# dougsouza/pytorch-sync-batchnorm-example

Measured on AMD Instinct MI355X. Metric: images/sec (whole node) resnet50 SyncBN, higher is better.
Workload: dtype bf16; 1 GPU; model=resnet50, global_batch=512, per_gpu_batch=512, image=3x224x224, memory_format=channels_last, parallelism=dp1, impl=msbn, hip_graph=False, conv_autotune=False, fused_bn_act=True

## Files before the change

msbn/models/resnet.py:

```python

from typing import List, Type, Union

import torch
import torch.nn as nn

from msbn.nn import BatchNorm2d, SyncBatchNorm
from msbn.nn.fused import SyncBatchNormAct2d, bn_act_maxpool


def conv3x3(cin, cout, stride=1):
    return nn.Conv2d(cin, cout, 3, stride=stride, padding=1, bias=False)


def conv1x1(cin, cout, stride=1):
    return nn.Conv2d(cin, cout, 1, stride=stride, bias=False)


def _norm(planes, fused):
    return SyncBatchNorm(planes) if fused else BatchNorm2d(planes)


def _split(x):
    return x if isinstance(x, tuple) else (x, x)


def _last_bn(bn, x, identity, fork):
    if not fork:
        return bn(x, residual=identity)
    if isinstance(bn, SyncBatchNormAct2d):
        return bn(x, residual=identity, fork=True)
    y = bn(x, residual=identity)
    return y, y


class BasicBlock(nn.Module):
    expansion = 1

    def __init__(self, cin, planes, stride=1, downsample=None, fused=False,
                 fork=False):
        super().__init__()
        self.fused = fused
        self.fork = fork and fused
        self.conv1 = conv3x3(cin, planes, stride)
        self.conv2 = conv3x3(planes, planes)
        self.downsample = downsample
        if fused:
            self.bn1 = SyncBatchNormAct2d(planes, relu=True)
            self.bn2 = SyncBatchNormAct2d(planes, relu=True)
        else:
            self.bn1 = BatchNorm2d(planes)
            self.bn2 = BatchNorm2d(planes)
            self.relu = nn.ReLU(inplace=True)

    def forward(self, x):
        x, skip = _split(x)
        identity = (self.downsample(skip) if self.downsample is not None
                    else skip)
        if self.fused:
            out = self.bn1(self.conv1(x))
            return _last_bn(self.bn2, self.conv2(out), identity,
                            getattr(self, "fork", False))
        out = self.relu(self.bn1(self.conv1(x)))
        out = self.bn2(self.conv2(out))
        return self.relu(out + identity)


class Bottleneck(nn.Module):
    expansion = 4

    def __init__(self, cin, planes, stride=1, downsample=None, fused=False,
                 fork=False):
        super().__init__()
        self.fused = fused
        self.fork = fork and fused
        self.conv1 = conv1x1(cin, planes)
        self.conv2 = conv3x3(planes, planes, stride)
        self.conv3 = conv1x1(planes, planes * self.expansion)
        self.downsample = downsample
        if fused:
            self.bn1 = SyncBatchNormAct2d(planes, relu=True)
            self.bn2 = SyncBatchNormAct2d(planes, relu=True)
            self.bn3 = SyncBatchNormAct2d(planes * self.expansion, relu=True)
        else:
            self.bn1 = BatchNorm2d(planes)
            self.bn2 = BatchNorm2d(planes)
            self.bn3 = BatchNorm2d(planes * self.expansion)
            self.relu = nn.ReLU(inplace=True)

    def forward(self, x):
        x, skip = _split(x)
        identity = (self.downsample(skip) if self.downsample is not None
                    else skip)
        if self.fused:
            out = self.bn1(self.conv1(x))
            out = self.bn2(self.conv2(out))
            return _last_bn(self.bn3, self.conv3(out), identity,
                            getattr(self, "fork", False))
        out = self.relu(self.bn1(self.conv1(x)))
        out = self.relu(self.bn2(self.conv2(out)))
        out = self.bn3(self.conv3(out))
        return self.relu(out + identity)


class ResNet(nn.Module):
    def __init__(
        self,
        block: Type[Union[BasicBlock, Bottleneck]],
        layers: List[int],
        num_classes: int = 1000,
        in_chans: int = 3,
        fused: bool = False,
        fork_grads: bool = True,
    ):
        super().__init__()
        self.fused = fused
        self.fork_grads = fork_grads and fused
        self.stem_pool = fused
        self.inplanes = 64
        self.conv1 = nn.Conv2d(in_chans, 64, 7, stride=2, padding=3, bias=False)
        if fused:
            self.bn1 = SyncBatchNormAct2d(64, relu=True)
        else:
            self.bn1 = BatchNorm2d(64)
        self.relu = nn.ReLU(inplace=True)
        self.maxpool = nn.MaxPool2d(3, stride=2, padding=1)
        self.layer1 = self._make_layer(block, 64, layers[0])
        self.layer2 = self._make_layer(block, 128, layers[1], stride=2)
        self.layer3 = self._make_layer(block, 256, layers[2], stride=2)
        self.layer4 = self._make_layer(block, 512, layers[3], stride=2,
                                       fork_last=False)
        self.avgpool = nn.AdaptiveAvgPool2d(1)
        self.fc = nn.Linear(512 * block.expansion, num_classes)
        for m in self.modules():
            if isinstance(m, nn.Conv2d):
                nn.init.kaiming_normal_(m.weight, mode="fan_out",
                                        nonlinearity="relu")

    def _make_layer(self, block, planes, blocks, stride=1, fork_last=True):
        fork = [self.fork_grads] * (blocks - 1) + [self.fork_grads
                                                   and fork_last]
        downsample = None
        if stride != 1 or self.inplanes != planes * block.expansion:
            downsample = nn.Sequential(
                conv1x1(self.inplanes, planes * block.expansion, stride),
                _norm(planes * block.expansion, self.fused),
            )
        layers = [block(self.inplanes, planes, stride, downsample,
                        fused=self.fused, fork=fork[0])]
        self.inplanes = planes * block.expansion
        for i in range(1, blocks):
            layers.append(block(self.inplanes, planes, fused=self.fused,
                                fork=fork[i]))
        return nn.Sequential(*layers)

    def _stem(self, x):
        x = self.conv1(x)
        if self.fused:
            if (getattr(self, "stem_pool", True)
                    and isinstance(self.bn1, SyncBatchNormAct2d)):
                return bn_act_maxpool(self.bn1, self.maxpool, x,
                                      fork=getattr(self, "fork_grads", False))
            return self.maxpool(self.bn1(x))
        return self.maxpool(self.relu(self.bn1(x)))

    def forward_features(self, x):
        x = self._stem(x)
        c2 = self.layer1(x)
        c3 = self.layer2(c2)
        c4 = self.layer3(c3)
        c5 = self.layer4(c4)
        return _split(c2)[0], _split(c3)[0], _split(c4)[0], _split(c5)[0]

    def forward(self, x):
        _, _, _, c5 = self.forward_features(x)
        out = self.avgpool(c5).flatten(1)
        return self.fc(out)


def resnet18(num_classes: int = 1000, fused: bool = False,
             fork_grads: bool = True) -> ResNet:
    return ResNet(BasicBlock, [2, 2, 2, 2], num_classes, fused=fused,
                  fork_grads=fork_grads)


def resnet50(num_classes: int = 1000, fused: bool = False,
             fork_grads: bool = True) -> ResNet:
    return ResNet(Bottleneck, [3, 4, 6, 3], num_classes, fused=fused,
                  fork_grads=fork_grads)
```

msbn/nn/fused.py:

```python

from typing import Optional

import torch
import torch.distributed as dist

from msbn import ops
from msbn.nn.batchnorm import (SyncBatchNorm, _check_negative_slope,
                               _momentum_factor, _running_stats_forward)
from msbn.nn.functions import (_combined_view, _contig, _force_sync,
                               _match_layout, compute_sync_stats)


class SyncBatchNormActFunction(torch.autograd.Function):
    @staticmethod
    def forward(
        ctx,
        input: torch.Tensor,
        residual: Optional[torch.Tensor],
        weight: Optional[torch.Tensor],
        bias: Optional[torch.Tensor],
        running_mean: Optional[torch.Tensor],
        running_var: Optional[torch.Tensor],
        eps: float,
        momentum: float,
        process_group,
        world_size: int,
        relu: bool,
        negative_slope: float = 0.0,
        fork: bool = False,
    ):
        ctx.fork = fork
        y = SyncBatchNormActFunction._forward(
            ctx, input, residual, weight, bias, running_mean, running_var,
            eps, momentum, process_group, world_size, relu, negative_slope,
        )
        if not fork:
            return y
        ctx.set_materialize_grads(False)
        return y, y.detach()

    @staticmethod
    def _forward(ctx, input, residual, weight, bias, running_mean,
                 running_var, eps, momentum, process_group, world_size, relu,
                 negative_slope):
        ctx.negative_slope = negative_slope
        input = _contig(input)
        if residual is not None:
            residual = _match_layout(residual, input)
        if weight is not None:
            weight = weight.contiguous()
        if bias is not None:
            bias = bias.contiguous()

        use_sync = world_size > 1 or (
            process_group is not None and _force_sync()
        )
        if (
            not use_sync
            and input.numel() > 0
            and (residual is None or residual.is_contiguous())
            and ops.bn_fused_local_eligible(
                input, weight, bias, running_mean, running_var
            )
        ):
            y, mean, invstd, count_sum, coefs = ops.batch_norm_fwd_fused_local(
                input, residual, weight, bias, eps, momentum,
                running_mean, running_var, relu, negative_slope,
            )
            ctx.save_for_backward(input, residual, weight, bias, mean,
                                  invstd, count_sum, coefs)
            ctx.has_coefs = True
            ctx.local_fused = True
            ctx.relu = relu
            ctx.process_group = process_group
            ctx.world_size = world_size
            return y
        ctx.local_fused = False

        mean, invstd, count_sum, coefs = compute_sync_stats(
            input, eps, momentum, running_mean, running_var,
            process_group, world_size, weight, bias, want_coefs=True,
        )
        if coefs is None:
            ctx.save_for_backward(input, residual, weight, bias, mean, invstd,
                                  count_sum)
            ctx.has_coefs = False
        else:
            ctx.save_for_backward(input, residual, weight, bias, mean, invstd,
                                  count_sum, coefs)
            ctx.has_coefs = True
        ctx.relu = relu
        ctx.process_group = process_group
        ctx.world_size = world_size
        ctx.use_sync = use_sync
        if input.numel() == 0:
            return torch.empty_like(input)
        return ops.batch_norm_elemt_act(
            input, residual, weight, bias, mean, invstd, relu, coefs,
            negative_slope,
        )

    @staticmethod
    def backward(ctx, grad_output, grad_skip=None):
        if grad_output is None:
            grad_output, grad_skip = grad_skip, None
        if grad_output is None:
            return (None,) * 13
        if ctx.has_coefs:
            (input, residual, weight, bias, mean, invstd, count_sum,
             coefs) = ctx.saved_tensors
        else:
            input, residual, weight, bias, mean, invstd, count_sum = (
                ctx.saved_tensors
            )
            coefs = None
        fold = (
            grad_skip is not None and input.is_cuda and input.numel() > 0
            and not getattr(ctx, "local_fused", False)
        )
        if fold and ctx.relu and ctx.negative_slope != 0.0 and not (
            residual is not None and ctx.needs_input_grad[1]
        ):
            fold = False
        if grad_skip is not None and not fold:
            grad_output = grad_output + grad_skip
            grad_skip = None
        grad_output = _match_layout(grad_output, input)
        if fold:
            grad_skip = _match_layout(grad_skip, input)
        relu = ctx.relu
        slope = ctx.negative_slope
        process_group = ctx.process_group
        world_size = ctx.world_size
        need_input_g = ctx.needs_input_grad[0]
        need_res_g = residual is not None and ctx.needs_input_grad[1]
        need_weight_g = weight is not None and ctx.needs_input_grad[2]
        need_bias_g = bias is not None and ctx.needs_input_grad[3]

        C = int(input.shape[1])

        if getattr(ctx, "local_fused", False) and input.numel() > 0:
            grad_input, grad_weight, grad_bias, grad_res = (
                ops.batch_norm_bwd_fused_local(
                    grad_output, input, residual, mean, invstd, weight,
                    coefs, relu, need_res_g, need_weight_g, need_bias_g,
                    slope,
                )
            )
            return (
                grad_input if need_input_g else None,
                grad_res if need_res_g else None,
                grad_weight if need_weight_g else None,
                grad_bias if need_bias_g else None,
                None, None, None, None, None, None, None, None, None,
            )

        use_gm = fold or (
            relu and residual is not None and need_res_g and input.is_cuda
            and input.numel() > 0
        )
        use_sync = getattr(ctx, "use_sync", world_size > 1)
        if input.numel() == 0:
            if use_sync and (need_input_g or need_res_g):
                combined = torch.zeros(2 * C, dtype=torch.float32,
                                       device=grad_output.device)
                from msbn.utils import debug as _dbg
                if _dbg.enabled():
                    _dbg.verify_collective("syncbn.bwd.all_reduce", combined,
                                           process_group)
                dist.all_reduce(combined, dist.ReduceOp.SUM,
                                group=process_group)
            zg = torch.empty_like(grad_output)
            return (
                zg if need_input_g else None,
                torch.empty_like(grad_output) if need_res_g else None,
                torch.zeros_like(weight) if need_weight_g else None,
                torch.zeros_like(bias) if need_bias_g else None,
                None, None, None, None, None, None, None, None, None,
            )
        gm = torch.empty_like(grad_output) if use_gm else None
        sum_dy, sum_dy_xmu, grad_weight, grad_bias = (
            ops.batch_norm_backward_reduce_act(
                grad_output, input, residual, mean, invstd, weight, bias,
                relu, need_input_g, need_weight_g, need_bias_g, coefs, gm,
                slope, grad_skip,
            )
        )
        grad_input = grad_res = None
        if need_input_g or need_res_g:
            if use_sync:
                combined, copied = _combined_view(sum_dy, sum_dy_xmu, C)
                from msbn.utils import debug as _dbg
                if _dbg.enabled():
                    _dbg.verify_collective("syncbn.bwd.all_reduce",
                                           combined, process_group)
                dist.all_reduce(combined, dist.ReduceOp.SUM, group=process_group)
                from msbn.utils.logging import comm_log
                comm_log.record("all_reduce", combined.numel() * 4,
                                f"syncbn bwd C={C}")
                if copied:
                    sum_dy, sum_dy_xmu = combined[:C], combined[C:]
            if use_gm:
                grad_input, _ = ops.batch_norm_backward_elemt_act(
                    gm, input, None, mean, invstd, weight, bias,
                    sum_dy, sum_dy_xmu, count_sum, False, False, coefs,
                )
                grad_res = gm if need_res_g else None
            else:
                grad_input, grad_res = ops.batch_norm_backward_elemt_act(
                    grad_output, input, residual, mean, invstd, weight, bias,
                    sum_dy, sum_dy_xmu, count_sum, relu, need_res_g, coefs,
                    slope,
                )
        return (
            grad_input if need_input_g else None,
            grad_res,
            grad_weight if need_weight_g else None,
            grad_bias if need_bias_g else None,
            None, None, None, None, None, None, None, None, None,
        )


class SyncBatchNormActPoolFunction(torch.autograd.Function):

    @staticmethod
    def forward(
        ctx,
        input: torch.Tensor,
        weight: Optional[torch.Tensor],
        bias: Optional[torch.Tensor],
        running_mean: Optional[torch.Tensor],
        running_var: Optional[torch.Tensor],
        eps: float,
        momentum: float,
        process_group,
        world_size: int,
        relu: bool,
        negative_slope: float = 0.0,
        fork: bool = False,
    ):
        if weight is not None:
            weight = weight.contiguous()
        if bias is not None:
            bias = bias.contiguous()
        use_sync = world_size > 1 or (
            process_group is not None and _force_sync()
        )
        mean, invstd, count_sum, coefs = compute_sync_stats(
            input, eps, momentum, running_mean, running_var,
            process_group, world_size, weight, bias, want_coefs=True,
        )
        pooled, codes = ops.batch_norm_elemt_act_pool(
            input, weight, bias, mean, invstd, relu, coefs, negative_slope
        )
        ctx.has_coefs = coefs is not None
        saved = (input, codes, weight, bias, mean, invstd, count_sum)
        ctx.save_for_backward(*(saved + ((coefs,) if ctx.has_coefs else ())))
        ctx.relu = relu
        ctx.negative_slope = negative_slope
        ctx.process_group = process_group
        ctx.use_sync = use_sync
        if not fork:
            return pooled
        ctx.set_materialize_grads(False)
        return pooled, pooled.detach()

    @staticmethod
    def backward(ctx, grad_output, grad_skip=None):
        if grad_output is None:
            grad_output, grad_skip = grad_skip, None
        if grad_output is None:
            return (None,) * 12
        saved = ctx.saved_tensors
        input, codes, weight, bias, mean, invstd, count_sum = saved[:7]
        coefs = saved[7] if ctx.has_coefs else None
        grad_output = _match_layout(grad_output, codes)
        if grad_skip is not None:
            grad_skip = _match_layout(grad_skip, codes)
        relu, slope = ctx.relu, ctx.negative_slope
        process_group = ctx.process_group
        need_input_g = ctx.needs_input_grad[0]
        need_weight_g = weight is not None and ctx.needs_input_grad[1]
        need_bias_g = bias is not None and ctx.needs_input_grad[2]
        C = int(input.shape[1])

        sum_dy, sum_dy_xmu, grad_weight, grad_bias = (
            ops.batch_norm_backward_reduce_act_pool(
                grad_output, grad_skip, codes, input, mean, invstd, weight,
                bias, relu, need_input_g, need_weight_g, need_bias_g, coefs,
                slope,
            )
        )
        grad_input = None
        if need_input_g:
            if ctx.use_sync:
                combined, copied = _combined_view(sum_dy, sum_dy_xmu, C)
                from msbn.utils import debug as _dbg
                if _dbg.enabled():
                    _dbg.verify_collective("syncbn.bwd.all_reduce",
                                           combined, process_group)
                dist.all_reduce(combined, dist.ReduceOp.SUM,
                                group=process_group)
                from msbn.utils.logging import comm_log
                comm_log.record("all_reduce", combined.numel() * 4,
                                f"syncbn bwd C={C}")
                if copied:
                    sum_dy, sum_dy_xmu = combined[:C], combined[C:]
            grad_input = ops.batch_norm_backward_elemt_act_pool(
                grad_output, grad_skip, codes, input, mean, invstd, weight,
                bias, sum_dy, sum_dy_xmu, count_sum, relu, coefs, slope,
            )
        return (
            grad_input,
            grad_weight if need_weight_g else None,
            grad_bias if need_bias_g else None,
            None, None, None, None, None, None, None, None, None,
        )


def stem_pool_eligible(bn, pool, input: torch.Tensor) -> bool:
    def _pair(v):
        return tuple(v) if isinstance(v, (tuple, list)) else (v, v)

    def _hooked(m):
        return bool(m._forward_hooks or m._forward_pre_hooks
                    or m._backward_hooks or m._backward_pre_hooks)

    return (
        type(bn) is SyncBatchNormAct2d
        and not getattr(bn, "inplace", False)
        and not _hooked(bn) and not _hooked(pool)
        and (bn.training
             or (bn.running_mean is None and bn.running_var is None))
        and type(pool) is torch.nn.MaxPool2d
        and _pair(pool.kernel_size) == (3, 3)
        and _pair(pool.stride) == (2, 2)
        and _pair(pool.padding) == (1, 1)
        and _pair(pool.dilation) == (1, 1)
        and not pool.ceil_mode and not pool.return_indices
        and input.is_cuda and input.dim() == 4 and input.numel() > 0
        and input.is_contiguous(memory_format=torch.channels_last)
        and input.dtype in (torch.float32, torch.bfloat16, torch.float16)
    )


def bn_act_maxpool(bn, pool, input: torch.Tensor, fork: bool = False):
    if not stem_pool_eligible(bn, pool, input):
        y = pool(bn(input))
        return (y, y) if fork else y
    bn._check_input_dim(input)
    bn._check_non_zero_input_channels(input)
    if bn.training and bn.track_running_stats:
        if bn.num_batches_tracked is not None:
            bn.num_batches_tracked.add_(1)
    factor = _momentum_factor(bn) if bn.training else (
        bn.momentum if bn.momentum is not None else 0.0
    )
    process_group = None
    world_size = 1
    if dist.is_available() and dist.is_initialized():
        process_group = bn.process_group or dist.group.WORLD
        world_size = dist.get_world_size(process_group)
    running_mean = bn.running_mean if bn.track_running_stats else None
    running_var = bn.running_var if bn.track_running_stats else None
    return SyncBatchNormActPoolFunction.apply(
        input, bn.weight, bn.bias, running_mean, running_var, bn.eps, factor,
        process_group, world_size, bn.relu,
        getattr(bn, "negative_slope", 0.0), fork,
    )


class InPlaceSyncBatchNormActFunction(torch.autograd.Function):

    @staticmethod
    def forward(
        ctx,
        input: torch.Tensor,
        weight: torch.Tensor,
        bias: torch.Tensor,
        running_mean: Optional[torch.Tensor],
        running_var: Optional[torch.Tensor],
        eps: float,
        momentum: float,
        process_group,
        world_size: int,
        act: bool,
        negative_slope: float = 0.0,
    ):
        if act and not negative_slope > 0.0:
            raise ValueError(
                "in-place BN needs an invertible activation: identity, or "
                "LeakyReLU with negative_slope > 0"
            )
        if _contig(input) is not input:
            raise ValueError(
                "in-place BN needs a dense NCHW or channels-last input; a "
                "copy would leave the caller's tensor unwritten"
            )
        weight = weight.contiguous()
        bias = bias.contiguous()
        use_sync = world_size > 1 or (
            process_group is not None and _force_sync()
        )
        mean, invstd, count_sum, coefs = compute_sync_stats(
            input, eps, momentum, running_mean, running_var,
            process_group, world_size, weight, bias, want_coefs=True,
        )
        if input.numel() > 0:
            ops.batch_norm_elemt_act_(
                input, weight, bias, mean, invstd, act, coefs, negative_slope
            )
        ctx.mark_dirty(input)
        ctx.has_coefs = coefs is not None
        saved = (input, weight, bias, mean, invstd, count_sum)
        ctx.save_for_backward(*(saved + ((coefs,) if ctx.has_coefs else ())))
        ctx.act = act
        ctx.negative_slope = negative_slope
        ctx.process_group = process_group
        ctx.world_size = world_size
        ctx.use_sync = use_sync
        return input

    @staticmethod
    def backward(ctx, grad_output):
        saved = ctx.saved_tensors
        y, weight, bias, mean, invstd, count_sum = saved[:6]
        coefs = saved[6] if ctx.has_coefs else None
        grad_output = _match_layout(grad_output, y)
        act, slope = ctx.act, ctx.negative_slope
        process_group = ctx.process_group
        use_sync = ctx.use_sync
        need_input_g, need_weight_g, need_bias_g = ctx.needs_input_grad[:3]
        C = int(y.shape[1])

        if y.numel() == 0:
            if use_sync and need_input_g:
                combined = torch.zeros(2 * C, dtype=torch.float32,
                                       device=grad_output.device)
                from msbn.utils import debug as _dbg
                if _dbg.enabled():
                    _dbg.verify_collective("syncbn.bwd.all_reduce", combined,
                                           process_group)
                dist.all_reduce(combined, dist.ReduceOp.SUM,
                                group=process_group)
            return (
                torch.empty_like(grad_output) if need_input_g else None,
                torch.zeros_like(weight) if need_weight_g else None,
                torch.zeros_like(bias) if need_bias_g else None,
                None, None, None, None, None, None, None, None,
            )
        sum_dy, sum_dy_xmu, grad_weight, grad_bias = (
            ops.batch_norm_backward_reduce_inplace(
                grad_output, y, invstd, weight, bias, act, need_input_g,
                need_weight_g, need_bias_g, coefs, slope,
            )
        )
        grad_input = None
        if need_input_g:
            if use_sync:
                combined, copied = _combined_view(sum_dy, sum_dy_xmu, C)
                from msbn.utils import debug as _dbg
                if _dbg.enabled():
                    _dbg.verify_collective("syncbn.bwd.all_reduce",
                                           combined, process_group)
                dist.all_reduce(combined, dist.ReduceOp.SUM, group=process_group)
                from msbn.utils.logging import comm_log
                comm_log.record("all_reduce", combined.numel() * 4,
                                f"syncbn bwd C={C}")
                if copied:
                    sum_dy, sum_dy_xmu = combined[:C], combined[C:]
            grad_input = ops.batch_norm_backward_elemt_inplace(
                grad_output, y, mean, invstd, weight, bias, sum_dy,
                sum_dy_xmu, count_sum, act, coefs, slope,
            )
        return (
            grad_input,
            grad_weight if need_weight_g else None,
            grad_bias if need_bias_g else None,
            None, None, None, None, None, None, None, None,
        )


class SyncBatchNormAct2d(SyncBatchNorm):

    def __init__(self, num_features, eps=1e-5, momentum=0.1, affine=True,
                 track_running_stats=True, process_group=None, device=None,
                 dtype=None, relu: bool = True, negative_slope: float = 0.0,
                 inplace: bool = False):
        super().__init__(num_features, eps, momentum, affine,
                         track_running_stats, process_group, device, dtype)
        self.relu = relu
        self.negative_slope = _check_negative_slope(relu, negative_slope)
        if inplace:
            if not affine:
                raise ValueError("inplace=True requires affine=True")
            if relu and not self.negative_slope > 0.0:
                raise ValueError(
                    "inplace=True needs an invertible activation: "
                    "relu=False, or relu=True with negative_slope > 0 "
                    "(plain ReLU cannot be inverted)"
                )
        self.inplace = bool(inplace)

    def extra_repr(self):
        s = super().extra_repr()
        slope = getattr(self, "negative_slope", 0.0)
        if slope != 0.0:
            s += f", negative_slope={slope}"
        if getattr(self, "inplace", False):
            s += ", inplace=True"
        return s

    def forward(self, input: torch.Tensor,
                residual: Optional[torch.Tensor] = None, fork: bool = False):
        self._check_input_dim(input)
        self._check_non_zero_input_channels(input)
        slope = getattr(self, "negative_slope", 0.0)
        inplace = getattr(self, "inplace", False)
        if inplace and (residual is not None or fork):
            raise ValueError(
                "an inplace=True SyncBatchNormAct2d takes neither a residual "
                "nor fork=True"
            )

        bn_training = self.training or (
            self.running_mean is None and self.running_var is None
        )
        if self.training and self.track_running_stats:
            if self.num_batches_tracked is not None:
                self.num_batches_tracked.add_(1)
        factor = _momentum_factor(self) if self.training else (
            self.momentum if self.momentum is not None else 0.0
        )

        if not bn_training:
            y = _running_stats_forward(self, input, residual, self.relu,
                                       slope)
            return (y, y) if fork else y

        process_group = None
        world_size = 1
        if dist.is_available() and dist.is_initialized():
            process_group = self.process_group or dist.group.WORLD
            world_size = dist.get_world_size(process_group)

        running_mean = self.running_mean if self.track_running_stats else None
        running_var = self.running_var if self.track_running_stats else None
        if inplace:
            return InPlaceSyncBatchNormActFunction.apply(
                input, self.weight, self.bias, running_mean, running_var,
                self.eps, factor, process_group, world_size, self.relu, slope,
            )
        return SyncBatchNormActFunction.apply(
            input, residual, self.weight, self.bias, running_mean, running_var,
            self.eps, factor, process_group, world_size, self.relu, slope,
            fork,
        )
```

msbn/ops/__init__.py:

```python

from typing import Optional

import torch

from msbn.ops import _reference as _ref

_C = None
_C_IMPORT_ERROR: Optional[BaseException] = None
try:
    import os as _os

    if _os.environ.get("MSBN_AB_NONT", "0") == "1":
        from msbn import _C_nont as _C
    else:
        from msbn import _C as _C
except Exception as e:
    _C_IMPORT_ERROR = e


def hip_available() -> bool:
    return _C is not None


def _require_hip():
    if _C is None:
        raise RuntimeError(
            "msbn._C (the gfx950 HIP kernel extension) is not built, but a CUDA "
            "tensor reached msbn.ops. Build it with `python setup.py "
            "build_ext --inplace` (or __graft_entry__.build()). "
            f"Import error was: {_C_IMPORT_ERROR!r}"
        )
    return _C


def batch_norm_stats(input: torch.Tensor, eps: float):
    if input.is_cuda:
        return _require_hip().batch_norm_stats(input, eps)
    return _ref.batch_norm_stats(input, eps)


def batch_norm_stats_packed(input: torch.Tensor, eps: float, out: torch.Tensor):
    C = input.shape[1]
    if input.is_cuda:
        _require_hip().batch_norm_stats_packed(input, eps, out)
        return out
    mean, invstd = _ref.batch_norm_stats(input, eps)
    out[:C] = mean
    out[C : 2 * C] = invstd
    n = input.numel() // C if C > 0 else 0
    out[2 * C] = float(n)
    return out


def batch_norm_gather_stats_with_counts(
    input: torch.Tensor,
    mean_all: torch.Tensor,
    invstd_all: torch.Tensor,
    running_mean: Optional[torch.Tensor],
    running_var: Optional[torch.Tensor],
    momentum: float,
    eps: float,
    counts: torch.Tensor,
):
    if input.is_cuda:
        return _require_hip().batch_norm_gather_stats_with_counts(
            mean_all, invstd_all, running_mean, running_var, momentum, eps, counts
        )
    return _ref.batch_norm_gather_stats_with_counts(
        input, mean_all, invstd_all, running_mean, running_var, momentum, eps, counts
    )


def batch_norm_gather_stats_packed(
    input: torch.Tensor,
    packed_all: torch.Tensor,
    running_mean: Optional[torch.Tensor],
    running_var: Optional[torch.Tensor],
    momentum: float,
    eps: float,
):
    W = packed_all.shape[0]
    C = (packed_all.shape[1] - 1) // 2
    if input.is_cuda:
        return _require_hip().batch_norm_gather_stats_packed(
            packed_all, running_mean, running_var, momentum, eps
        )
    mean_all = packed_all[:, :C]
    invstd_all = packed_all[:, C : 2 * C]
    counts = packed_all[:, 2 * C]
    mean, invstd = _ref.batch_norm_gather_stats_with_counts(
        input, mean_all, invstd_all, running_mean, running_var, momentum, eps, counts
    )
    return mean, invstd, counts.sum().reshape(1)


def batch_norm_elemt(
    input: torch.Tensor,
    weight: Optional[torch.Tensor],
    bias: Optional[torch.Tensor],
    mean: torch.Tensor,
    invstd: torch.Tensor,
    eps: float,
):
    if input.is_cuda:
        return _require_hip().batch_norm_elemt(input, weight, bias, mean, invstd, eps)
    return _ref.batch_norm_elemt(input, weight, bias, mean, invstd, eps)


def batch_norm_backward_reduce(
    grad_out: torch.Tensor,
    input: torch.Tensor,
    mean: torch.Tensor,
    invstd: torch.Tensor,
    weight: Optional[torch.Tensor],
    input_g: bool,
    weight_g: bool,
    bias_g: bool,
):
    if input.is_cuda:
        return _require_hip().batch_norm_backward_reduce(
            grad_out, input, mean, invstd, weight, input_g, weight_g, bias_g
        )
    return _ref.batch_norm_backward_reduce(
        grad_out, input, mean, invstd, weight, input_g, weight_g, bias_g
    )


def batch_norm_backward_elemt(
    grad_out: torch.Tensor,
    input: torch.Tensor,
    mean: torch.Tensor,
    invstd: torch.Tensor,
    weight: Optional[torch.Tensor],
    sum_dy: torch.Tensor,
    sum_dy_xmu: torch.Tensor,
    count: torch.Tensor,
):
    if input.is_cuda:
        return _require_hip().batch_norm_backward_elemt(
            grad_out, input, mean, invstd, weight, sum_dy, sum_dy_xmu, count
        )
    return _ref.batch_norm_backward_elemt(
        grad_out, input, mean, invstd, weight, sum_dy, sum_dy_xmu, count
    )


def bn_fused_local_eligible(input, weight, bias, running_mean, running_var):
    if not input.is_cuda or _C is None:
        return False
    return _C.bn_fused_local_eligible(
        input, weight, bias, running_mean, running_var
    )


def batch_norm_fwd_fused_local(input, residual, weight, bias, eps, momentum,
                               running_mean, running_var, relu,
                               negative_slope: float = 0.0):
    return _require_hip().batch_norm_fwd_fused_local(
        input, residual, weight, bias, eps, momentum, running_mean,
        running_var, relu, negative_slope,
    )


def batch_norm_bwd_fused_local(grad_out, input, residual, mean, invstd,
                               weight, coefs, relu_mask, want_res_grad,
                               weight_g, bias_g, negative_slope: float = 0.0):
    return _require_hip().batch_norm_bwd_fused_local(
        grad_out, input, residual, mean, invstd, weight, coefs, relu_mask,
        want_res_grad, weight_g, bias_g, negative_slope,
    )


def bn_make_coefs(mean, invstd, weight, bias):
    if mean.is_cuda:
        return _require_hip().bn_make_coefs(mean, invstd, weight, bias)
    return None


def batch_norm_elemt_act(input, residual, weight, bias, mean, invstd,
                         relu: bool, coefs=None, negative_slope: float = 0.0):
    if input.is_cuda:
        return _require_hip().batch_norm_elemt_act(
            input, residual, weight, bias, mean, invstd, relu, coefs,
            negative_slope,
        )
    return _ref.batch_norm_elemt_act(
        input, residual, weight, bias, mean, invstd, relu, negative_slope
    )


def batch_norm_backward_reduce_act(grad_out, input, residual, mean, invstd,
                                   weight, bias, relu_mask, input_g, weight_g,
                                   bias_g, coefs=None, gm_out=None,
                                   negative_slope: float = 0.0,
                                   grad_out2=None):
    if input.is_cuda:
        return _require_hip().batch_norm_backward_reduce_act(
            grad_out, input, residual, mean, invstd, weight, bias, relu_mask,
            input_g, weight_g, bias_g, coefs, gm_out, negative_slope,
            grad_out2,
        )
    return _ref.batch_norm_backward_reduce_act(
        grad_out, input, residual, mean, invstd, weight, bias, relu_mask,
        input_g, weight_g, bias_g, gm_out, negative_slope, grad_out2,
    )


def batch_norm_backward_elemt_act(grad_out, input, residual, mean, invstd,
                                  weight, bias, sum_dy, sum_dy_xmu, count,
                                  relu_mask, want_res_grad, coefs=None,
                                  negative_slope: float = 0.0):
    if input.is_cuda:
        dx, dres = _require_hip().batch_norm_backward_elemt_act(
            grad_out, input, residual, mean, invstd, weight, bias, sum_dy,
            sum_dy_xmu, count, relu_mask, want_res_grad, coefs,
            negative_slope,
        )
        return dx, (dres if want_res_grad else None)
    return _ref.batch_norm_backward_elemt_act(
        grad_out, input, residual, mean, invstd, weight, bias, sum_dy,
        sum_dy_xmu, count, relu_mask, want_res_grad, negative_slope,
    )


def batch_norm_elemt_act_pool(input, weight, bias, mean, invstd, relu: bool,
                              coefs=None, negative_slope: float = 0.0):
    if input.is_cuda:
        return _require_hip().batch_norm_elemt_act_pool(
            input, weight, bias, mean, invstd, relu, coefs, negative_slope
        )
    return _ref.batch_norm_elemt_act_pool(
        input, weight, bias, mean, invstd, relu, negative_slope
    )


def batch_norm_backward_reduce_act_pool(grad_out, grad_out2, codes, input,
                                        mean, invstd, weight, bias, relu_mask,
                                        input_g, weight_g, bias_g, coefs=None,
                                        negative_slope: float = 0.0):
    if input.is_cuda:
        return _require_hip().batch_norm_backward_reduce_act_pool(
            grad_out, grad_out2, codes, input, mean, invstd, weight, bias,
            relu_mask, input_g, weight_g, bias_g, coefs, negative_slope,
        )
    return _ref.batch_norm_backward_reduce_act_pool(
        grad_out, grad_out2, codes, input, mean, invstd, weight, bias,
        relu_mask, input_g, weight_g, bias_g, negative_slope,
    )


def batch_norm_backward_elemt_act_pool(grad_out, grad_out2, codes, input,
                                       mean, invstd, weight, bias, sum_dy,
                                       sum_dy_xmu, count, relu_mask,
                                       coefs=None,
                                       negative_slope: float = 0.0):
    if input.is_cuda:
        return _require_hip().batch_norm_backward_elemt_act_pool(
            grad_out, grad_out2, codes, input, mean, invstd, weight, bias,
            sum_dy, sum_dy_xmu, count, relu_mask, coefs, negative_slope,
        )
    return _ref.batch_norm_backward_elemt_act_pool(
        grad_out, grad_out2, codes, input, mean, invstd, weight, bias,
        sum_dy, sum_dy_xmu, count, relu_mask, negative_slope,
    )


def batch_norm_elemt_act_(input, weight, bias, mean, invstd, act: bool,
                          coefs=None, negative_slope: float = 0.0):
    if input.is_cuda:
        _require_hip().batch_norm_elemt_act_(
            input, weight, bias, mean, invstd, act, coefs, negative_slope
        )
        return input
    return _ref.batch_norm_elemt_act_(
        input, weight, bias, mean, invstd, act, negative_slope
    )


def batch_norm_backward_reduce_inplace(grad_out, output, invstd, weight, bias,
                                       act: bool, input_g, weight_g, bias_g,
                                       coefs=None,
                                       negative_slope: float = 0.0):
    if output.is_cuda:
        return _require_hip().batch_norm_backward_reduce_inplace(
            grad_out, output, invstd, weight, bias, act, input_g, weight_g,
            bias_g, coefs, negative_slope,
        )
    return _ref.batch_norm_backward_reduce_inplace(
        grad_out, output, invstd, weight, bias, act, input_g, weight_g,
        bias_g, negative_slope,
    )


def batch_norm_backward_elemt_inplace(grad_out, output, mean, invstd, weight,
                                      bias, sum_dy, sum_dy_xmu, count,
                                      act: bool, coefs=None,
                                      negative_slope: float = 0.0):
    if output.is_cuda:
        return _require_hip().batch_norm_backward_elemt_inplace(
            grad_out, output, mean, invstd, weight, bias, sum_dy, sum_dy_xmu,
            count, act, coefs, negative_slope,
        )
    return _ref.batch_norm_backward_elemt_inplace(
        grad_out, output, mean, invstd, weight, bias, sum_dy, sum_dy_xmu,
        count, act, negative_slope,
    )


def bn_frozen_coefs(running_mean, running_var, eps: float, weight, bias):
    if running_mean.is_cuda:
        return _require_hip().bn_frozen_coefs(
            running_mean, running_var, eps, weight, bias
        )
    return _ref.bn_frozen_coefs(running_mean, running_var, eps, weight, bias)


def batch_norm_frozen_backward_elemt(grad_out, input, residual, coefs,
                                     relu_mask: bool, want_input_grad: bool,
                                     want_res_grad: bool,
                                     negative_slope: float = 0.0):
    if grad_out.is_cuda:
        dx, dres = _require_hip().batch_norm_frozen_backward_elemt(
            grad_out, input, residual, coefs, relu_mask, want_input_grad,
            want_res_grad, negative_slope,
        )
        return (dx if want_input_grad else None,
                dres if want_res_grad else None)
    return _ref.batch_norm_frozen_backward_elemt(
        grad_out, input, residual, coefs, relu_mask, want_input_grad,
        want_res_grad, negative_slope,
    )


def launch_plan(kind: str, input: torch.Tensor, others=(), coefs=None) -> dict:
    path, numbers = _require_hip().launch_plan(kind, input, list(others), coefs)
    plan = dict(numbers)
    plan["path"] = path
    if "multi_trip" in plan:
        plan["multi_trip"] = bool(plan["multi_trip"])
    return plan


__all__ = [
    "hip_available",
    "launch_plan",
    "bn_frozen_coefs",
    "batch_norm_frozen_backward_elemt",
    "batch_norm_elemt_act_pool",
    "batch_norm_backward_reduce_act_pool",
    "batch_norm_backward_elemt_act_pool",
    "batch_norm_elemt_act_",
    "batch_norm_backward_reduce_inplace",
    "batch_norm_backward_elemt_inplace",
    "batch_norm_elemt_act",
    "bn_make_coefs",
    "batch_norm_backward_reduce_act",
    "batch_norm_backward_elemt_act",
    "batch_norm_stats",
    "batch_norm_stats_packed",
    "batch_norm_gather_stats_with_counts",
    "batch_norm_gather_stats_packed",
    "batch_norm_elemt",
    "batch_norm_backward_reduce",
    "batch_norm_backward_elemt",
]
```

msbn/ops/csrc/bn_kernels.hip:

```cpp
#include "bn_ops.hpp"
#include "common.hpp"

#include <ATen/ATen.h>
#include <c10/hip/HIPStream.h>

#include <algorithm>
#include <map>
#include <string>
#include <vector>

namespace msbn {

namespace {

template <typename T, int V>
__global__ void bn_stats_partial_nchw(const T* __restrict__ x,
                                      double* __restrict__ ws, int64_t N,
                                      int64_t C, int64_t S, int64_t chunkN,
                                      int64_t chunkS) {
  const int64_t c = blockIdx.x;
  const int64_t n0 = blockIdx.y * chunkN;
  const int64_t n1 = i64min(n0 + chunkN, N);
  const int64_t s0 = blockIdx.z * chunkS;
  const int64_t s1 = i64min(s0 + chunkS, S);
// ... 44 lines not shown
    }
    __syncthreads();
    if (pivot_s[0] == 0.f) break;
    pivot = pivot_s[1];
  }
  if (threadIdx.x == 0) {
    const int64_t chunk = (int64_t)blockIdx.y * gridDim.z + blockIdx.z;
    double* out = ws + (c * gridDim.y * gridDim.z + chunk) * 2;
    out[0] = a;
    out[1] = b;
  }
}

template <typename T>
__global__ void bn_stats_partial_nchw_flat(const T* __restrict__ x,
                                           double* __restrict__ ws, int64_t N,
                                           int64_t C, int64_t S,
                                           int64_t chunk_len) {
  const int64_t c = blockIdx.x;
  const int64_t NS = N * S;
  const int64_t p0 = (int64_t)blockIdx.y * chunk_len;
  const int64_t p1 = i64min(p0 + chunk_len, NS);
  __shared__ double lds[2 * (MSBN_BLOCK / MSBN_WAVE)];
  __shared__ float pivot_s[2];
  float pivot = 0.f;
  double a = 0.0, b = 0.0;
  for (int pass = 0; pass < 2; ++pass) {
    AccPair acc;
    int since_flush = 0;
    for (int64_t p = p0 + threadIdx.x; p < p1; p += blockDim.x) {
      const int64_t n = p / S, s = p - n * S;
      acc.add(to_f(nt_load1(&x[(n * C + c) * S + s])) - pivot);
      if (++since_flush == MSBN_ACC_FLUSH) {
        acc.flush();
        since_flush = 0;
      }
    }
    acc.flush();
    a = acc.a;
    b = acc.b;
    if (pass) __syncthreads();
    block_reduce_pair(a, b, lds);
    const double cnt = (double)(p1 - p0);
    if (pass) {
      if (threadIdx.x == 0) unshift_pair(a, b, pivot, cnt);
      break;
    }
    if (threadIdx.x == 0) {
      const bool re = needs_recentre(a, b, cnt);
      pivot_s[0] = re ? 1.f : 0.f;
      pivot_s[1] = re ? (float)(a / cnt) : 0.f;
    }
    __syncthreads();
    if (pivot_s[0] == 0.f) break;
    pivot = pivot_s[1];
  }
  if (threadIdx.x == 0) {
    double* out = ws + (c * gridDim.y + blockIdx.y) * 2;
    out[0] = a;
    out[1] = b;
  }
}

template <typename T, int V>
__global__ void bn_stats_partial_nhwc(const T* __restrict__ x,
                                      double* __restrict__ ws, int64_t rows,
                                      int64_t C, int64_t chunk_rows, int lpr) {
  const int rpi = blockDim.x / lpr;
  const int lane = threadIdx.x % lpr;
  const int rowoff = threadIdx.x / lpr;
  const bool active = rowoff < rpi;
  const int64_t c = (int64_t)blockIdx.x * lpr * V + (int64_t)lane * V;
  const bool inb = active && (c + V <= C);
  const int64_t r0 = (int64_t)blockIdx.y * chunk_rows;
  const int64_t r1 = i64min(r0 + chunk_rows, rows);

  __shared__ double sdata[MSBN_BLOCK * V * 2];

  float pivot[V];
  bool re[V];
#pragma unroll
  for (int k = 0; k < V; ++k) {
    pivot[k] = 0.f;
    re[k] = false;
  }

  for (int pass = 0; pass < 2; ++pass) {
    AccPair acc[V];
    if (inb) {
      int since_flush = 0;
      for (int64_t r = r0 + rowoff; r < r1; r += rpi) {
        Pack<T, V> pk = nt_load<T, V>(&x[r * C + c]);
#pragma unroll
        for (int k = 0; k < V; ++k) acc[k].add(to_f(pk.v[k]) - pivot[k]);
        if (++since_flush == MSBN_ACC_FLUSH) {
#pragma unroll
          for (int k = 0; k < V; ++k) acc[k].flush();
          since_flush = 0;
        }
      }
    }
    double a[V], b[V];
#pragma unroll
    for (int k = 0; k < V; ++k) {
      acc[k].flush();
      a[k] = acc[k].a;
      b[k] = acc[k].b;
    }
    if (pass && inb && r0 + rowoff < r1) {
      const double cnt = (double)((r1 - r0 - rowoff + rpi - 1) / rpi);
#pragma unroll
      for (int k = 0; k < V; ++k) unshift_pair(a[k], b[k], pivot[k], cnt);
    }

    if (pass) __syncthreads();
#pragma unroll
    for (int k = 0; k < V; ++k) {
      sdata[k * MSBN_BLOCK + threadIdx.x] = a[k];
      sdata[(V + k) * MSBN_BLOCK + threadIdx.x] = b[k];
    }
    for (int st = 1; st < rpi; st <<= 1) {
      __syncthreads();
      if (active && (rowoff & ((st << 1) - 1)) == 0 && rowoff + st < rpi) {
        const int other = threadIdx.x + st * lpr;
#pragma unroll
        for (int k = 0; k < V; ++k) {
          sdata[k * MSBN_BLOCK + threadIdx.x] += sdata[k * MSBN_BLOCK + other];
          sdata[(V + k) * MSBN_BLOCK + threadIdx.x] +=
              sdata[(V + k) * MSBN_BLOCK + other];
        }
      }
    }
    __syncthreads();
    int any = 0;
    if (rowoff == 0 && c < C) {
      const int64_t chunk = blockIdx.y;
      const double cnt = (double)(r1 - r0);
#pragma unroll
      for (int k = 0; k < V; ++k) {
        if (c + k < C) {
          const double sa = sdata[k * MSBN_BLOCK + threadIdx.x];
          const double sb = sdata[(V + k) * MSBN_BLOCK + threadIdx.x];
          bool want = false;
          if (!pass) {
            want = needs_recentre(sa, sb, cnt);
            sdata[k * MSBN_BLOCK + threadIdx.x] = want ? 1.0 : 0.0;
            sdata[(V + k) * MSBN_BLOCK + threadIdx.x] = want ? sa / cnt : 0.0;
            any |= want ? 1 : 0;
          }
          if (pass ? re[k] : !want) {
            double* out = ws + ((c + k) * gridDim.y + chunk) * 2;
            out[0] = sa;
            out[1] = sb;
          }
        }
      }
    }
    if (pass) break;
    if (!__syncthreads_or(any)) break;
    if (inb) {
#pragma unroll
      for (int k = 0; k < V; ++k) {
        re[k] = sdata[k * MSBN_BLOCK + lane] != 0.0;
        pivot[k] = re[k] ? (float)sdata[(V + k) * MSBN_BLOCK + lane] : 0.f;
      }
    }
  }
}

template <typename RT, typename WT>
__global__ void bn_stats_finalize(const double* __restrict__ ws, int nchunks,
                                  int64_t C, double count, float eps,
                                  float* __restrict__ mean,
                                  float* __restrict__ invstd,
                                  float* __restrict__ count_out,
                                  RT* __restrict__ rmean, RT* __restrict__ rvar,
                                  float momentum, const WT* __restrict__ w,
                                  const WT* __restrict__ bws,
                                  float* __restrict__ scale_out,
                                  float* __restrict__ shift_out) {
  const int lane = threadIdx.x & (MSBN_WAVE - 1);
  const int wid = threadIdx.x >> 6;
  const int64_t c = (int64_t)blockIdx.x * (blockDim.x >> 6) + wid;
  if (c >= C) return;
  double a = 0.0, b = 0.0;
  for (int ch = lane; ch < nchunks; ch += MSBN_WAVE) {
    a += ws[(c * nchunks + ch) * 2];
    b += ws[(c * nchunks + ch) * 2 + 1];
  }
  wave_reduce_pair(a, b);
  if (lane != 0) return;
  const double m = a / count;
  double var = b / count - m * m;
  var = var > 0.0 ? var : 0.0;
  const float istd = (float)rsqrt(var + (double)eps);
  mean[c] = (float)m;
  invstd[c] = istd;
  if (c == 0 && count_out != nullptr) count_out[0] = (float)count;
  if (rmean != nullptr) {
    const double unbiased = count > 1.0 ? var * (count / (count - 1.0)) : var;
    rmean[c] = from_f<RT>((1.f - momentum) * to_f(rmean[c]) + momentum * (float)m);
    rvar[c] =
        from_f<RT>((1.f - momentum) * to_f(rvar[c]) + momentum * (float)unbiased);
  }
  if (scale_out != nullptr) {
    const float sc = istd * (w != nullptr ? to_f(w[c]) : 1.f);
    scale_out[c] = sc;
    shift_out[c] = -(float)m * sc + (bws != nullptr ? to_f(bws[c]) : 0.f);
  }
}

template <typename RT, typename WT>
__global__ void bn_gather_stats(const float* __restrict__ packed_all, int W,
                                int64_t C, float eps, float momentum,
                                float* __restrict__ mean,
                                float* __restrict__ invstd,
                                float* __restrict__ count_out,
                                RT* __restrict__ rmean, RT* __restrict__ rvar,
                                const WT* __restrict__ wpar,
                                const WT* __restrict__ bpar,
                                float* __restrict__ scale_out,
                                float* __restrict__ shift_out) {
  const int64_t c = (int64_t)blockIdx.x * blockDim.x + threadIdx.x;
  if (c >= C) return;
  const int64_t row = 2 * C + 1;
  double n_tot = 0.0, m_acc = 0.0, ex2 = 0.0;
  for (int w = 0; w < W; ++w) {
    const float cnt = packed_all[w * row + 2 * C];
    if (cnt > 0.f) {
      const double m = packed_all[w * row + c];
      const double istd = packed_all[w * row + C + c];
      const double var = 1.0 / (istd * istd) - (double)eps;
      n_tot += cnt;
      m_acc += cnt * m;
      ex2 += cnt * (var + m * m);
    }
  }
  float m_out = 0.f, istd_out = 0.f;
  if (n_tot > 0.0) {
    const double m_g = m_acc / n_tot;
    double var_g = ex2 / n_tot - m_g * m_g;
    var_g = var_g > 0.0 ? var_g : 0.0;
    m_out = (float)m_g;
    istd_out = (float)rsqrt(var_g + (double)eps);
    if (rmean != nullptr) {
      const double unbiased =
          n_tot > 1.0 ? var_g * (n_tot / (n_tot - 1.0)) : var_g;
      rmean[c] =
          from_f<RT>((1.f - momentum) * to_f(rmean[c]) + momentum * (float)m_g);
      rvar[c] = from_f<RT>((1.f - momentum) * to_f(rvar[c]) +
                           momentum * (float)unbiased);
    }
  }
  mean[c] = m_out;
  invstd[c] = istd_out;
  if (c == 0 && count_out != nullptr) count_out[0] = (float)n_tot;
  if (scale_out != nullptr) {
    const float sc = istd_out * (wpar != nullptr ? to_f(wpar[c]) : 1.f);
    scale_out[c] = sc;
    shift_out[c] = -m_out * sc + (bpar != nullptr ? to_f(bpar[c]) : 0.f);
  }
}

template <typename WT>
__global__ void bn_affine_fwd(const float* __restrict__ mean,
                              const float* __restrict__ invstd,
                              const WT* __restrict__ w,
                              const WT* __restrict__ b, int64_t C,
                              float* __restrict__ scale,
                              float* __restrict__ shift) {
  const int64_t c = (int64_t)blockIdx.x * blockDim.x + threadIdx.x;
  if (c >= C) return;
  const float sc = invstd[c] * (w != nullptr ? to_f(w[c]) : 1.f);
  scale[c] = sc;
  shift[c] = -mean[c] * sc + (b != nullptr ? to_f(b[c]) : 0.f);
}

template <typename WT>
__global__ void bn_affine_bwd(const float* __restrict__ mean,
                              const float* __restrict__ invstd,
                              const WT* __restrict__ w,
                              const float* __restrict__ sum_dy,
                              const float* __restrict__ sum_dy_xmu,
                              const float* __restrict__ count, int64_t C,
                              float* __restrict__ coef_a,
                              float* __restrict__ coef_b,
                              float* __restrict__ coef_d) {
  const int64_t c = (int64_t)blockIdx.x * blockDim.x + threadIdx.x;
  if (c >= C) return;
  const float n = count[0];
  if (n <= 0.f) {
    coef_a[c] = coef_b[c] = coef_d[c] = 0.f;
    return;
  }
  const float istd = invstd[c];
  const float f1 = istd * (w != nullptr ? to_f(w[c]) : 1.f);
  const float f2 = sum_dy[c] / n;
  const float f3 = istd * istd * sum_dy_xmu[c] / n;
  coef_a[c] = f1;
  coef_b[c] = -f1 * f3;
  coef_d[c] = f1 * (f3 * mean[c] - f2);
}

template <typename T, int V, int ACT, bool RES>
__global__ void bn_elemt_nchw(const T* __restrict__ x,
                              const T* __restrict__ res, T* __restrict__ y,
                              const float* __restrict__ scale,
                              const float* __restrict__ shift, int64_t total,
                              int64_t C, int64_t S, float slope) {
  const int64_t stride = (int64_t)gridDim.x * blockDim.x;
  for (int64_t i = (int64_t)blockIdx.x * blockDim.x + threadIdx.x;
       i * V < total; i += stride) {
    const int64_t e = i * V;
    const int64_t c = (e / S) % C;
    const float sc = scale[c], sh = shift[c];
    if (V == 1) {
      float z = to_f(nt_load1(&x[e])) * sc + sh;
      if (RES) z += to_f(nt_load1(&res[e]));
      z = act_fwd<ACT>(z, slope);
      nt_store1(&y[e], from_f<T>(z));
    } else {
      Pack<T, V> px = nt_load<T, V>(&x[e]);
      Pack<T, V> pr;
      if (RES) pr = nt_load<T, V>(&res[e]);
      Pack<T, V> py;
#pragma unroll
      for (int k = 0; k < V; ++k) {
        float z = to_f(px.v[k]) * sc + sh;
        if (RES) z += to_f(pr.v[k]);
        z = act_fwd<ACT>(z, slope);
        py.v[k] = from_f<T>(z);
      }
      nt_store<T, V>(&y[e], py);
    }
  }
}

template <typename T, int V, int ACT, bool RES>
__global__ void bn_elemt_nhwc(const T* __restrict__ x,
                              const T* __restrict__ res, T* __restrict__ y,
                              const float* __restrict__ scale,
                              const float* __restrict__ shift, int64_t total,
                              int64_t C, float slope) {
  const int64_t stride = (int64_t)gridDim.x * blockDim.x;
  for (int64_t i = (int64_t)blockIdx.x * blockDim.x + threadIdx.x;
       i * V < total; i += stride) {
    const int64_t e = i * V;
    const int64_t c = e % C;
    if (V == 1) {
      float z = to_f(nt_load1(&x[e])) * scale[c] + shift[c];
      if (RES) z += to_f(nt_load1(&res[e]));
      z = act_fwd<ACT>(z, slope);
      nt_store1(&y[e], from_f<T>(z));
    } else {
      Pack<T, V> px = nt_load<T, V>(&x[e]);
      Pack<float, V> ps = *reinterpret_cast<const Pack<float, V>*>(&scale[c]);
      Pack<float, V> pb = *reinterpret_cast<const Pack<float, V>*>(&shift[c]);
      Pack<T, V> pr;
      if (RES) pr = nt_load<T, V>(&res[e]);
      Pack<T, V> py;
#pragma unroll
      for (int k = 0; k < V; ++k) {
        float z = to_f(px.v[k]) * ps.v[k] + pb.v[k];
        if (RES) z += to_f(pr.v[k]);
        z = act_fwd<ACT>(z, slope);
        py.v[k] = from_f<T>(z);
      }
      nt_store<T, V>(&y[e], py);
    }
  }
}

template <typename T>
__device__ __forceinline__ float fork_grad(T g1, T g2) {
  return to_f(from_f<T>(to_f(g1) + to_f(g2)));
}

template <typename T, int V, int ACT, bool RES, bool GMOUT, bool DY2>
__global__ void bn_bwd_reduce_partial_nchw(const T* __restrict__ dy,
                                           const T* __restrict__ dy2,
                                           const T* __restrict__ x,
                                           const T* __restrict__ res,
                                           T* __restrict__ gm_out,
                                           const float* __restrict__ mean,
                                           const float* __restrict__ scale,
                                           const float* __restrict__ shift,
                                           double* __restrict__ ws, int64_t N,
                                           int64_t C, int64_t S, int64_t chunkN,
                                           int64_t chunkS, float slope) {
  const int64_t c = blockIdx.x;
  const float m = mean[c];
  const float sc = ACT ? scale[c] : 0.f;
  const float sh = ACT ? shift[c] : 0.f;
  const int64_t n0 = blockIdx.y * chunkN;
  const int64_t n1 = i64min(n0 + chunkN, N);
  const int64_t s0 = blockIdx.z * chunkS;
  const int64_t s1 = i64min(s0 + chunkS, S);
  AccPair acc;
  int since_flush = 0;
  for (int64_t n = n0; n < n1; ++n) {
    const int64_t base = (n * C + c) * S;
    if (V == 1) {
      for (int64_t s = s0 + threadIdx.x; s < s1; s += blockDim.x) {
        float g = DY2 ? fork_grad(nt_load1(&dy[base + s]),
                                  nt_load1(&dy2[base + s]))
                      : to_f(nt_load1(&dy[base + s]));
        const float xv = to_f(nt_load1(&x[base + s]));
        if (ACT) {
          float z = sc * xv + sh;
          if (RES) z += to_f(nt_load1(&res[base + s]));
          g = act_gate<ACT>(z, g, slope);
        }
        if (GMOUT) nt_store1(&gm_out[base + s], from_f<T>(g));
        acc.add2(g, g * (xv - m));
        if (++since_flush == MSBN_ACC_FLUSH) {
          acc.flush();
          since_flush = 0;
        }
      }
    } else {
      for (int64_t s = s0 + (int64_t)threadIdx.x * V; s < s1;
           s += (int64_t)blockDim.x * V) {
        Pack<T, V> pg = nt_load<T, V>(&dy[base + s]);
        Pack<T, V> px = nt_load<T, V>(&x[base + s]);
        Pack<T, V> pg2, pr, pm;
        if (DY2) pg2 = nt_load<T, V>(&dy2[base + s]);
        if (RES) pr = nt_load<T, V>(&res[base + s]);
#pragma unroll
        for (int k = 0; k < V; ++k) {
          float g = DY2 ? fork_grad(pg.v[k], pg2.v[k]) : to_f(pg.v[k]);
          const float xv = to_f(px.v[k]);
          if (ACT) {
            float z = sc * xv + sh;
            if (RES) z += to_f(pr.v[k]);
            g = act_gate<ACT>(z, g, slope);
          }
          if (GMOUT) pm.v[k] = from_f<T>(g);
          acc.add2(g, g * (xv - m));
        }
        if (GMOUT) nt_store<T, V>(&gm_out[base + s], pm);
        if (++since_flush == MSBN_ACC_FLUSH / V) {
          acc.flush();
          since_flush = 0;
        }
      }
    }
  }
  acc.flush();
  double a = acc.a, b = acc.b;
  __shared__ double lds[2 * (MSBN_BLOCK / MSBN_WAVE)];
  block_reduce_pair(a, b, lds);
  if (threadIdx.x == 0) {
    const int64_t chunk = (int64_t)blockIdx.y * gridDim.z + blockIdx.z;
    double* out = ws + (c * gridDim.y * gridDim.z + chunk) * 2;
    out[0] = a;
    out[1] = b;
  }
}

template <typename T, int ACT, bool RES, bool GMOUT, bool DY2>
__global__ void bn_bwd_reduce_partial_nchw_flat(
    const T* __restrict__ dy, const T* __restrict__ dy2,
    const T* __restrict__ x,
    const T* __restrict__ res, T* __restrict__ gm_out,
    const float* __restrict__ mean,
    const float* __restrict__ scale, const float* __restrict__ shift,
    double* __restrict__ ws, int64_t N, int64_t C, int64_t S,
    int64_t chunk_len, float slope) {
  const int64_t c = blockIdx.x;
  const float m = mean[c];
  const float sc = ACT ? scale[c] : 0.f;
  const float sh = ACT ? shift[c] : 0.f;
  const int64_t NS = N * S;
  const int64_t p0 = (int64_t)blockIdx.y * chunk_len;
  const int64_t p1 = i64min(p0 + chunk_len, NS);
  AccPair acc;
  int since_flush = 0;
  for (int64_t p = p0 + threadIdx.x; p < p1; p += blockDim.x) {
    const int64_t n = p / S, s = p - n * S;
    const int64_t e = (n * C + c) * S + s;
    float g = DY2 ? fork_grad(nt_load1(&dy[e]), nt_load1(&dy2[e]))
                  : to_f(nt_load1(&dy[e]));
    const float xv = to_f(nt_load1(&x[e]));
    if (ACT) {
      float z = sc * xv + sh;
      if (RES) z += to_f(nt_load1(&res[e]));
      g = act_gate<ACT>(z, g, slope);
    }
    if (GMOUT) nt_store1(&gm_out[e], from_f<T>(g));
    acc.add2(g, g * (xv - m));
    if (++since_flush == MSBN_ACC_FLUSH) {
      acc.flush();
      since_flush = 0;
    }
  }
  acc.flush();
  double a = acc.a, b = acc.b;
  __shared__ double lds[2 * (MSBN_BLOCK / MSBN_WAVE)];
  block_reduce_pair(a, b, lds);
  if (threadIdx.x == 0) {
    double* out = ws + (c * gridDim.y + blockIdx.y) * 2;
    out[0] = a;
    out[1] = b;
  }
}

template <typename T, int V, int ACT, bool RES, bool GMOUT, bool DY2>
__global__ void bn_bwd_reduce_partial_nhwc(const T* __restrict__ dy,
                                           const T* __restrict__ dy2,
                                           const T* __restrict__ x,
                                           const T* __restrict__ res,
                                           T* __restrict__ gm_out,
                                           const float* __restrict__ mean,
                                           const float* __restrict__ scale,
                                           const float* __restrict__ shift,
                                           double* __restrict__ ws,
                                           int64_t rows, int64_t C,
                                           int64_t chunk_rows, int lpr,
                                           float slope) {
  const int rpi = blockDim.x / lpr;
  const int lane = threadIdx.x % lpr;
  const int rowoff = threadIdx.x / lpr;
  const bool active = rowoff < rpi;
  const int64_t c = (int64_t)blockIdx.x * lpr * V + (int64_t)lane * V;
  const bool inb = active && (c + V <= C);

  AccPair acc[V];
  float m[V], scv[V], shv[V];
#pragma unroll
  for (int k = 0; k < V; ++k) m[k] = scv[k] = shv[k] = 0.f;
  if (inb) {
#pragma unroll
    for (int k = 0; k < V; ++k) {
      m[k] = mean[c + k];
      if (ACT) {
        scv[k] = scale[c + k];
        shv[k] = shift[c + k];
      }
    }
    const int64_t r0 = (int64_t)blockIdx.y * chunk_rows;
    const int64_t r1 = i64min(r0 + chunk_rows, rows);
    int since_flush = 0;
    for (int64_t r = r0 + rowoff; r < r1; r += rpi) {
      Pack<T, V> pg = nt_load<T, V>(&dy[r * C + c]);
      Pack<T, V> px = nt_load<T, V>(&x[r * C + c]);
      Pack<T, V> pg2, pr, pm;
      if (DY2) pg2 = nt_load<T, V>(&dy2[r * C + c]);
      if (RES) pr = nt_load<T, V>(&res[r * C + c]);
#pragma unroll
      for (int k = 0; k < V; ++k) {
        float g = DY2 ? fork_grad(pg.v[k], pg2.v[k]) : to_f(pg.v[k]);
        const float xv = to_f(px.v[k]);
        if (ACT) {
          float z = scv[k] * xv + shv[k];
          if (RES) z += to_f(pr.v[k]);
          g = act_gate<ACT>(z, g, slope);
        }
        if (GMOUT) pm.v[k] = from_f<T>(g);
        acc[k].add2(g, g * (xv - m[k]));
      }
      if (GMOUT) nt_store<T, V>(&gm_out[r * C + c], pm);
      if (++since_flush == MSBN_ACC_FLUSH) {
#pragma unroll
        for (int k = 0; k < V; ++k) acc[k].flush();
        since_flush = 0;
      }
    }
  }
  double a[V], b[V];
#pragma unroll
  for (int k = 0; k < V; ++k) {
    acc[k].flush();
    a[k] = acc[k].a;
    b[k] = acc[k].b;
  }
  __shared__ double sdata[MSBN_BLOCK * V * 2];
#pragma unroll
  for (int k = 0; k < V; ++k) {
    sdata[k * MSBN_BLOCK + threadIdx.x] = a[k];
    sdata[(V + k) * MSBN_BLOCK + threadIdx.x] = b[k];
  }
  for (int st = 1; st < rpi; st <<= 1) {
    __syncthreads();
    if (active && (rowoff & ((st << 1) - 1)) == 0 && rowoff + st < rpi) {
      const int other = threadIdx.x + st * lpr;
#pragma unroll
      for (int k = 0; k < V; ++k) {
        sdata[k * MSBN_BLOCK + threadIdx.x] += sdata[k * MSBN_BLOCK + other];
        sdata[(V + k) * MSBN_BLOCK + threadIdx.x] +=
            sdata[(V + k) * MSBN_BLOCK + other];
      }
    }
  }
  __syncthreads();
  if (rowoff == 0 && c < C) {
    const int64_t chunk = blockIdx.y;
#pragma unroll
    for (int k = 0; k < V; ++k) {
      if (c + k < C) {
        double* out = ws + ((c + k) * gridDim.y + chunk) * 2;
        out[0] = sdata[k * MSBN_BLOCK + threadIdx.x];
        out[1] = sdata[(V + k) * MSBN_BLOCK + threadIdx.x];
      }
    }
  }
}

template <typename WT>
__global__ void bn_bwd_reduce_finalize(const double* __restrict__ ws,
                                       int nchunks, int64_t C,
                                       const float* __restrict__ invstd,
                                       float* __restrict__ sum_dy,
                                       float* __restrict__ sum_dy_xmu,
                                       WT* __restrict__ grad_weight,
                                       WT* __restrict__ grad_bias) {
  const int lane = threadIdx.x & (MSBN_WAVE - 1);
  const int wid = threadIdx.x >> 6;
  const int64_t c = (int64_t)blockIdx.x * (blockDim.x >> 6) + wid;
  if (c >= C) return;
  double a = 0.0, b = 0.0;
  for (int ch = lane; ch < nchunks; ch += MSBN_WAVE) {
    a += ws[(c * nchunks + ch) * 2];
    b += ws[(c * nchunks + ch) * 2 + 1];
  }
  wave_reduce_pair(a, b);
  if (lane != 0) return;
  if (sum_dy != nullptr) sum_dy[c] = (float)a;
  if (sum_dy_xmu != nullptr) sum_dy_xmu[c] = (float)b;
  if (grad_weight != nullptr) grad_weight[c] = from_f<WT>((float)(b * invstd[c]));
  if (grad_bias != nullptr) grad_bias[c] = from_f<WT>((float)a);
}

template <typename T, int V, int ACT, bool RES, bool RESG>
__global__ void bn_bwd_elemt_nchw(const T* __restrict__ dy,
                                  const T* __restrict__ x,
                                  const T* __restrict__ res,
                                  T* __restrict__ dx, T* __restrict__ dres,
                                  const float* __restrict__ ca,
                                  const float* __restrict__ cb,
                                  const float* __restrict__ cd,
                                  const float* __restrict__ scale,
                                  const float* __restrict__ shift,
                                  int64_t total, int64_t C, int64_t S,
                                  float slope) {
  const int64_t stride = (int64_t)gridDim.x * blockDim.x;
  for (int64_t i = (int64_t)blockIdx.x * blockDim.x + threadIdx.x;
       i * V < total; i += stride) {
    const int64_t e = i * V;
    const int64_t c = (e / S) % C;
    const float A = ca[c], B = cb[c], D = cd[c];
    const float sc = ACT ? scale[c] : 0.f;
    const float sh = ACT ? shift[c] : 0.f;
    if (V == 1) {
      float g = to_f(nt_load1(&dy[e]));
      const float xv = to_f(nt_load1(&x[e]));
      if (ACT) {
        float z = sc * xv + sh;
        if (RES) z += to_f(nt_load1(&res[e]));
        g = act_gate<ACT>(z, g, slope);
      }
      nt_store1(&dx[e], from_f<T>(A * g + B * xv + D));
      if (RESG) nt_store1(&dres[e], from_f<T>(g));
    } else {
      Pack<T, V> pg = nt_load<T, V>(&dy[e]);
      Pack<T, V> px = nt_load<T, V>(&x[e]);
      Pack<T, V> pr;
      if (RES) pr = nt_load<T, V>(&res[e]);
      Pack<T, V> po, pq;
#pragma unroll
      for (int k = 0; k < V; ++k) {
        float g = to_f(pg.v[k]);
        const float xv = to_f(px.v[k]);
        if (ACT) {
          float z = sc * xv + sh;
          if (RES) z += to_f(pr.v[k]);
          g = act_gate<ACT>(z, g, slope);
        }
        po.v[k] = from_f<T>(A * g + B * xv + D);
        if (RESG) pq.v[k] = from_f<T>(g);
      }
      nt_store<T, V>(&dx[e], po);
      if (RESG) nt_store<T, V>(&dres[e], pq);
    }
  }
}

template <typename T, int V, int ACT, bool RES, bool RESG>
__global__ void bn_bwd_elemt_nhwc(const T* __restrict__ dy,
                                  const T* __restrict__ x,
                                  const T* __restrict__ res,
                                  T* __restrict__ dx, T* __restrict__ dres,
                                  const float* __restrict__ ca,
                                  const float* __restrict__ cb,
                                  const float* __restrict__ cd,
                                  const float* __restrict__ scale,
                                  const float* __restrict__ shift,
                                  int64_t total, int64_t C, float slope) {
  const int64_t stride = (int64_t)gridDim.x * blockDim.x;
  for (int64_t i = (int64_t)blockIdx.x * blockDim.x + threadIdx.x;
       i * V < total; i += stride) {
    const int64_t e = i * V;
    const int64_t c = e % C;
    if (V == 1) {
      float g = to_f(nt_load1(&dy[e]));
      const float xv = to_f(nt_load1(&x[e]));
      if (ACT) {
        float z = scale[c] * xv + shift[c];
        if (RES) z += to_f(nt_load1(&res[e]));
        g = act_gate<ACT>(z, g, slope);
      }
      nt_store1(&dx[e], from_f<T>(ca[c] * g + cb[c] * xv + cd[c]));
      if (RESG) nt_store1(&dres[e], from_f<T>(g));
    } else {
      Pack<T, V> pg = nt_load<T, V>(&dy[e]);
      Pack<T, V> px = nt_load<T, V>(&x[e]);
      Pack<float, V> pa = *reinterpret_cast<const Pack<float, V>*>(&ca[c]);
      Pack<float, V> pb = *reinterpret_cast<const Pack<float, V>*>(&cb[c]);
      Pack<float, V> pd = *reinterpret_cast<const Pack<float, V>*>(&cd[c]);
      Pack<float, V> psc, psh;
      if (ACT) {
        psc = *reinterpret_cast<const Pack<float, V>*>(&scale[c]);
        psh = *reinterpret_cast<const Pack<float, V>*>(&shift[c]);
      }
      Pack<T, V> pr;
      if (RES) pr = nt_load<T, V>(&res[e]);
      Pack<T, V> po, pq;
#pragma unroll
      for (int k = 0; k < V; ++k) {
        float g = to_f(pg.v[k]);
        const float xv = to_f(px.v[k]);
        if (ACT) {
          float z = psc.v[k] * xv + psh.v[k];
          if (RES) z += to_f(pr.v[k]);
          g = act_gate<ACT>(z, g, slope);
        }
        po.v[k] = from_f<T>(pa.v[k] * g + pb.v[k] * xv + pd.v[k]);
        if (RESG) pq.v[k] = from_f<T>(g);
      }
      nt_store<T, V>(&dx[e], po);
      if (RESG) nt_store<T, V>(&dres[e], pq);
    }
  }
}

template <typename RT, typename WT>
__global__ void bn_frozen_coefs(const RT* __restrict__ rmean,
                                const RT* __restrict__ rvar, float eps,
                                const WT* __restrict__ w,
                                const WT* __restrict__ b, int64_t C,
                                float* __restrict__ scale,
                                float* __restrict__ shift) {
  const int64_t c = (int64_t)blockIdx.x * blockDim.x + threadIdx.x;
  if (c >= C) return;
  const float istd = (float)rsqrt((double)to_f(rvar[c]) + (double)eps);
  const float sc = istd * (w != nullptr ? to_f(w[c]) : 1.f);
  scale[c] = sc;
  shift[c] = -to_f(rmean[c]) * sc + (b != nullptr ? to_f(b[c]) : 0.f);
}

template <typename T, int V, int ACT, bool RES, bool RESG>
__global__ void bn_frozen_bwd_elemt_nchw(const T* __restrict__ dy,
                                         const T* __restrict__ x,
                                         const T* __restrict__ res,
                                         T* __restrict__ dx,
                                         T* __restrict__ dres,
                                         const float* __restrict__ scale,
                                         const float* __restrict__ shift,
                                         int64_t total, int64_t C, int64_t S,
                                         float slope) {
  const int64_t stride = (int64_t)gridDim.x * blockDim.x;
  for (int64_t i = (int64_t)blockIdx.x * blockDim.x + threadIdx.x;
       i * V < total; i += stride) {
    const int64_t e = i * V;
    const int64_t c = (e / S) % C;
    const float sc = scale[c];
    const float sh = ACT ? shift[c] : 0.f;
    if (V == 1) {
      float g = to_f(nt_load1(&dy[e]));
      if (ACT) {
        float z = sc * to_f(nt_load1(&x[e])) + sh;
        if (RES) z += to_f(nt_load1(&res[e]));
        g = act_gate<ACT>(z, g, slope);
      }
      if (dx != nullptr) nt_store1(&dx[e], from_f<T>(sc * g));
      if (RESG) nt_store1(&dres[e], from_f<T>(g));
    } else {
      Pack<T, V> pg = nt_load<T, V>(&dy[e]);
      Pack<T, V> px, pr;
      if (ACT) px = nt_load<T, V>(&x[e]);
      if (ACT && RES) pr = nt_load<T, V>(&res[e]);
      Pack<T, V> po, pq;
#pragma unroll
      for (int k = 0; k < V; ++k) {
        float g = to_f(pg.v[k]);
        if (ACT) {
          float z = sc * to_f(px.v[k]) + sh;
          if (RES) z += to_f(pr.v[k]);
          g = act_gate<ACT>(z, g, slope);
        }
        po.v[k] = from_f<T>(sc * g);
        if (RESG) pq.v[k] = from_f<T>(g);
      }
      if (dx != nullptr) nt_store<T, V>(&dx[e], po);
      if (RESG) nt_store<T, V>(&dres[e], pq);
    }
  }
}

template <typename T, int V, int ACT, bool RES, bool RESG>
__global__ void bn_frozen_bwd_elemt_nhwc(const T* __restrict__ dy,
                                         const T* __restrict__ x,
                                         const T* __restrict__ res,
                                         T* __restrict__ dx,
                                         T* __restrict__ dres,
                                         const float* __restrict__ scale,
                                         const float* __restrict__ shift,
                                         int64_t total, int64_t C,
                                         float slope) {
  const int64_t stride = (int64_t)gridDim.x * blockDim.x;
  for (int64_t i = (int64_t)blockIdx.x * blockDim.x + threadIdx.x;
       i * V < total; i += stride) {
    const int64_t e = i * V;
    const int64_t c = e % C;
    if (V == 1) {
      float g = to_f(nt_load1(&dy[e]));
      const float sc = scale[c];
      if (ACT) {
        float z = sc * to_f(nt_load1(&x[e])) + shift[c];
        if (RES) z += to_f(nt_load1(&res[e]));
        g = act_gate<ACT>(z, g, slope);
      }
      if (dx != nullptr) nt_store1(&dx[e], from_f<T>(sc * g));
      if (RESG) nt_store1(&dres[e], from_f<T>(g));
    } else {
      Pack<T, V> pg = nt_load<T, V>(&dy[e]);
      Pack<float, V> psc = *reinterpret_cast<const Pack<float, V>*>(&scale[c]);
      Pack<float, V> psh;
      Pack<T, V> px, pr;
      if (ACT) {
        psh = *reinterpret_cast<const Pack<float, V>*>(&shift[c]);
        px = nt_load<T, V>(&x[e]);
      }
      if (ACT && RES) pr = nt_load<T, V>(&res[e]);
      Pack<T, V> po, pq;
#pragma unroll
      for (int k = 0; k < V; ++k) {
        float g = to_f(pg.v[k]);
        if (ACT) {
          float z = psc.v[k] * to_f(px.v[k]) + psh.v[k];
          if (RES) z += to_f(pr.v[k]);
          g = act_gate<ACT>(z, g, slope);
        }
        po.v[k] = from_f<T>(psc.v[k] * g);
        if (RESG) pq.v[k] = from_f<T>(g);
      }
      if (dx != nullptr) nt_store<T, V>(&dx[e], po);
// ... 1063 lines not shown
    switch (TYPE) {                                                         \
      case at::kFloat: {                                                    \
        using wt_t = float;                                                 \
        return __VA_ARGS__();                                               \
      }                                                                     \
      case at::kBFloat16: {                                                 \
        using wt_t = __hip_bfloat16;                                        \
        return __VA_ARGS__();                                               \
      }                                                                     \
      case at::kHalf: {                                                     \
        using wt_t = __half;                                                \
        return __VA_ARGS__();                                               \
      }                                                                     \
      default:                                                              \
        TORCH_CHECK(false, NAME, ": unsupported weight dtype ", TYPE);      \
    }                                                                       \
  }()

void stats_into(const at::Tensor& input, double eps, float* mean_p,
                float* invstd_p, float* count_p, const at::Tensor* rmean,
                const at::Tensor* rvar, double momentum,
                const at::Tensor* wpar = nullptr,
                const at::Tensor* bpar = nullptr, float* scale_p = nullptr,
                float* shift_p = nullptr) {
  const Layout L = get_layout(input);
  const int64_t count = L.rows;
  auto stream = cur_stream();
  const auto rstat_type = rmean ? rmean->scalar_type() : at::kFloat;
  const auto w_type = wpar ? wpar->scalar_type()
                     : bpar ? bpar->scalar_type()
                            : at::kFloat;

  MSBN_DISPATCH_FLOAT_TYPES(input.scalar_type(), "batch_norm_stats", [&] {
    const native_t* x =
        reinterpret_cast<const native_t*>(input.data_ptr<scalar_t>());
    constexpr int VMAX = 16 / (int)sizeof(native_t);
    const ReducePlan plan = plan_reduce(L, (int)sizeof(native_t), {x});
    const int v = plan.v;
    const int nchunks = plan.nchunks;
    at::Tensor ws = at::empty({(int64_t)nchunks * L.C * 2},
                              input.options().dtype(at::kDouble));
    if (plan.path == RedPath::NchwFlat) {
      const auto& g = plan.flat;
      hipLaunchKernelGGL((bn_stats_partial_nchw_flat<native_t>), g.grid,
                         dim3(MSBN_BLOCK), 0, stream, x,
                         ws.data_ptr<double>(), L.N, L.C, L.S, g.chunk_len);
    } else if (plan.path == RedPath::NchwVec) {
      const auto& g = plan.nchw;
      MSBN_DISPATCH_V(v, VMAX, [&] {
        hipLaunchKernelGGL((bn_stats_partial_nchw<native_t, VV>), g.grid,
                           dim3(MSBN_BLOCK), 0, stream, x,
                           ws.data_ptr<double>(), L.N, L.C, L.S, g.chunkN,
                           g.chunkS);
      });
    } else {
      const auto& g = plan.nhwc;
      MSBN_DISPATCH_V(v, VMAX, [&] {
        hipLaunchKernelGGL((bn_stats_partial_nhwc<native_t, VV>), g.grid,
                           dim3(MSBN_BLOCK), 0, stream, x,
                           ws.data_ptr<double>(), L.rows, L.C, g.chunk_rows,
                           g.lpr);
      });
    }
    const int fgrid = (int)cdiv(L.C, kFinalizeWavesPerBlock);
    MSBN_DISPATCH_RSTAT(rstat_type, "batch_norm_stats", [&] {
      MSBN_DISPATCH_WTYPE(w_type, "batch_norm_stats", [&] {
        rstat_t* rm = rmean ? reinterpret_cast<rstat_t*>(rmean->data_ptr())
                            : nullptr;
        rstat_t* rv = rvar ? reinterpret_cast<rstat_t*>(rvar->data_ptr())
                           : nullptr;
        const wt_t* wp =
            wpar ? reinterpret_cast<const wt_t*>(wpar->data_ptr()) : nullptr;
        const wt_t* bp =
            bpar ? reinterpret_cast<const wt_t*>(bpar->data_ptr()) : nullptr;
        hipLaunchKernelGGL((bn_stats_finalize<rstat_t, wt_t>), dim3(fgrid),
                           dim3(MSBN_BLOCK), 0, stream, ws.data_ptr<double>(),
                           nchunks, L.C, (double)count, (float)eps, mean_p,
                           invstd_p, count_p, rm, rv, (float)momentum, wp, bp,
                           scale_p, shift_p);
      });
    });
  });
}

}


std::tuple<at::Tensor, at::Tensor> batch_norm_stats(const at::Tensor& input,
                                                    double eps) {
  const int64_t C = input.size(1);
  auto opts = input.options().dtype(at::kFloat);
  auto mean = at::empty({C}, opts);
  auto invstd = at::empty({C}, opts);
  if (input.numel() == 0) {
    mean.zero_();
    invstd.zero_();
    return {mean, invstd};
  }
  stats_into(input, eps, mean.data_ptr<float>(), invstd.data_ptr<float>(),
             nullptr, nullptr, nullptr, 0.0);
  return {mean, invstd};
}

void batch_norm_stats_packed(const at::Tensor& input, double eps,
                             at::Tensor& out) {
  const int64_t C = input.size(1);
  TORCH_CHECK(out.is_contiguous() && out.numel() == 2 * C + 1 &&
                  out.scalar_type() == at::kFloat,
              "packed stats buffer must be contiguous fp32 of size 2C+1");
  if (input.numel() == 0) {
    out.zero_();
    return;
  }
  float* p = out.data_ptr<float>();
  stats_into(input, eps, p, p + C, p + 2 * C, nullptr, nullptr, 0.0);
}

std::tuple<at::Tensor, at::Tensor, at::Tensor, at::Tensor>
batch_norm_gather_stats_packed_coefs(
    const at::Tensor& packed_all, const c10::optional<at::Tensor>& running_mean,
    const c10::optional<at::Tensor>& running_var, double momentum, double eps,
    const c10::optional<at::Tensor>& weight,
    const c10::optional<at::Tensor>& bias, bool want_coefs) {
  TORCH_CHECK(packed_all.dim() == 2 && packed_all.is_contiguous() &&
                  packed_all.scalar_type() == at::kFloat,
              "packed_all must be contiguous fp32 [W, 2C+1]");
  const int W = (int)packed_all.size(0);
  const int64_t C = (packed_all.size(1) - 1) / 2;
  auto opts = packed_all.options();
  auto mean = at::empty({C}, opts);
  auto invstd = at::empty({C}, opts);
  auto count_sum = at::empty({1}, opts);
  at::Tensor coefs;
  float* scale_p = nullptr;
  float* shift_p = nullptr;
  if (want_coefs) {
    coefs = at::empty({2 * C}, opts);
    scale_p = coefs.data_ptr<float>();
    shift_p = scale_p + C;
  }
  auto stream = cur_stream();
  const auto rstat_type =
      running_mean.has_value() ? running_mean->scalar_type() : at::kFloat;
  const auto w_type = weight.has_value() ? weight->scalar_type()
                      : bias.has_value() ? bias->scalar_type()
                                         : at::kFloat;
  const int fgrid = (int)cdiv(C, MSBN_BLOCK);
  MSBN_DISPATCH_RSTAT(rstat_type, "gather_stats", [&] {
    MSBN_DISPATCH_WTYPE(w_type, "gather_stats", [&] {
      rstat_t* rm = running_mean.has_value()
                        ? reinterpret_cast<rstat_t*>(running_mean->data_ptr())
                        : nullptr;
      rstat_t* rv = running_var.has_value()
                        ? reinterpret_cast<rstat_t*>(running_var->data_ptr())
                        : nullptr;
      const wt_t* wp =
          weight.has_value()
              ? reinterpret_cast<const wt_t*>(weight->data_ptr())
              : nullptr;
      const wt_t* bp = bias.has_value()
                           ? reinterpret_cast<const wt_t*>(bias->data_ptr())
                           : nullptr;
      hipLaunchKernelGGL((bn_gather_stats<rstat_t, wt_t>), dim3(fgrid),
                         dim3(MSBN_BLOCK), 0, stream,
                         packed_all.data_ptr<float>(), W, C, (float)eps,
                         (float)momentum, mean.data_ptr<float>(),
                         invstd.data_ptr<float>(), count_sum.data_ptr<float>(),
                         rm, rv, wp, bp, scale_p, shift_p);
    });
  });
  return {mean, invstd, count_sum, coefs};
}

std::tuple<at::Tensor, at::Tensor, at::Tensor> batch_norm_gather_stats_packed(
    const at::Tensor& packed_all, const c10::optional<at::Tensor>& running_mean,
    const c10::optional<at::Tensor>& running_var, double momentum, double eps) {
  auto r = batch_norm_gather_stats_packed_coefs(
      packed_all, running_mean, running_var, momentum, eps, c10::nullopt,
      c10::nullopt, false);
  return {std::get<0>(r), std::get<1>(r), std::get<2>(r)};
}

std::tuple<at::Tensor, at::Tensor, at::Tensor, at::Tensor>
batch_norm_stats_local(const at::Tensor& input, double eps,
                       const c10::optional<at::Tensor>& running_mean,
                       const c10::optional<at::Tensor>& running_var,
                       double momentum,
                       const c10::optional<at::Tensor>& weight,
                       const c10::optional<at::Tensor>& bias,
                       bool want_coefs) {
  const int64_t C = input.size(1);
  auto opts = input.options().dtype(at::kFloat);
  auto mean = at::empty({C}, opts);
  auto invstd = at::empty({C}, opts);
  auto count_sum = at::empty({1}, opts);
  at::Tensor coefs;
  float* scale_p = nullptr;
  float* shift_p = nullptr;
  if (want_coefs) {
    coefs = at::empty({2 * C}, opts);
    scale_p = coefs.data_ptr<float>();
    shift_p = scale_p + C;
  }
  TORCH_CHECK(input.numel() > 0, "batch_norm_stats_local: empty input");
  const at::Tensor* rm =
      running_mean.has_value() ? &running_mean.value() : nullptr;
  const at::Tensor* rv =
      running_var.has_value() ? &running_var.value() : nullptr;
  const at::Tensor* wp = weight.has_value() ? &weight.value() : nullptr;
  const at::Tensor* bp = bias.has_value() ? &bias.value() : nullptr;
  stats_into(input, eps, mean.data_ptr<float>(), invstd.data_ptr<float>(),
             count_sum.data_ptr<float>(), rm, rv, momentum, wp, bp, scale_p,
             shift_p);
  return {mean, invstd, count_sum, coefs};
}

std::tuple<at::Tensor, at::Tensor> batch_norm_gather_stats_with_counts(
    const at::Tensor& mean_all, const at::Tensor& invstd_all,
    const c10::optional<at::Tensor>& running_mean,
    const c10::optional<at::Tensor>& running_var, double momentum, double eps,
    const at::Tensor& counts) {
  const int64_t W = mean_all.size(0);
  const int64_t C = mean_all.size(1);
  auto packed = at::empty({W, 2 * C + 1}, mean_all.options().dtype(at::kFloat));
  packed.narrow(1, 0, C).copy_(mean_all);
  packed.narrow(1, C, C).copy_(invstd_all);
  packed.narrow(1, 2 * C, 1).copy_(
      counts.to(at::kFloat).reshape({W, 1}));
  auto out = batch_norm_gather_stats_packed(packed, running_mean, running_var,
                                            momentum, eps);
  return {std::get<0>(out), std::get<1>(out)};
}

namespace {
at::Tensor make_fwd_coefs(const at::Tensor& mean, const at::Tensor& invstd,
                          const c10::optional<at::Tensor>& weight,
                          const c10::optional<at::Tensor>& bias, int64_t C) {
  auto coefs = at::empty({2 * C}, mean.options().dtype(at::kFloat));
  float* scale = coefs.data_ptr<float>();
  float* shift = scale + C;
  auto stream = cur_stream();
  const int cgrid = (int)cdiv(C, MSBN_BLOCK);
  const auto wtype = weight.has_value() ? weight->scalar_type()
                     : bias.has_value() ? bias->scalar_type()
                                        : at::kFloat;
  MSBN_DISPATCH_RSTAT(wtype, "bn_affine", [&] {
    const rstat_t* w =
        weight.has_value()
            ? reinterpret_cast<const rstat_t*>(weight->data_ptr())
            : nullptr;
    const rstat_t* b = bias.has_value()
                           ? reinterpret_cast<const rstat_t*>(bias->data_ptr())
                           : nullptr;
    hipLaunchKernelGGL((bn_affine_fwd<rstat_t>), dim3(cgrid), dim3(MSBN_BLOCK),
                       0, stream, mean.data_ptr<float>(),
                       invstd.data_ptr<float>(), w, b, C, scale, shift);
  });
  return coefs;
}

#define MSBN_DISPATCH_BOOL(FLAG, NAME, ...)                                  \
  [&] {                                                                      \
    if (FLAG) {                                                              \
      constexpr bool NAME = true;                                            \
      return __VA_ARGS__();                                                  \
    } else {                                                                 \
      constexpr bool NAME = false;                                           \
      return __VA_ARGS__();                                                  \
    }                                                                        \
  }()

inline int act_mode(bool on, float slope) {
  return !on ? kActNone : (slope == 0.f ? kActRelu : kActLeaky);
}

#define MSBN_DISPATCH_ACT(MODE, NAME, ...)                                   \
  [&] {                                                                      \
    switch (MODE) {                                                          \
      case kActRelu: {                                                       \
        constexpr int NAME = kActRelu;                                       \
        return __VA_ARGS__();                                                \
      }                                                                      \
      case kActLeaky: {                                                      \
        constexpr int NAME = kActLeaky;                                      \
        return __VA_ARGS__();                                                \
      }                                                                      \
      default: {                                                             \
        constexpr int NAME = kActNone;                                       \
        return __VA_ARGS__();                                                \
      }                                                                      \
    }                                                                        \
  }()

template <int ACT>
using ActC = std::integral_constant<int, ACT>;
}

at::Tensor bn_make_coefs(const at::Tensor& mean, const at::Tensor& invstd,
                         const c10::optional<at::Tensor>& weight,
                         const c10::optional<at::Tensor>& bias) {
  return make_fwd_coefs(mean, invstd, weight, bias, mean.numel());
}

at::Tensor batch_norm_elemt_act(const at::Tensor& input,
                                const c10::optional<at::Tensor>& residual,
                                const c10::optional<at::Tensor>& weight,
                                const c10::optional<at::Tensor>& bias,
                                const at::Tensor& mean,
                                const at::Tensor& invstd, bool relu,
                                const c10::optional<at::Tensor>& coefs_in,
                                double negative_slope) {
  const Layout L = get_layout(input);
  auto out = at::empty_like(input);
  if (input.numel() == 0) return out;
  const float slope = (float)negative_slope;
  const int act = act_mode(relu, slope);
  auto stream = cur_stream();
  auto coefs = coefs_in.has_value()
                   ? *coefs_in
                   : make_fwd_coefs(mean, invstd, weight, bias, L.C);
  float* scale = coefs.data_ptr<float>();
  float* shift = scale + L.C;
  const bool has_res = residual.has_value();
  if (has_res) {
    TORCH_CHECK(residual->sizes() == input.sizes() &&
                    residual->strides() == input.strides() &&
                    residual->scalar_type() == input.scalar_type(),
                "residual must match input shape/strides/dtype");
  }

  const int64_t total = input.numel();
  MSBN_DISPATCH_FLOAT_TYPES(input.scalar_type(), "bn_elemt", [&] {
    const native_t* x =
        reinterpret_cast<const native_t*>(input.data_ptr<scalar_t>());
    const native_t* res =
        has_res ? reinterpret_cast<const native_t*>(residual->data_ptr())
                : nullptr;
    native_t* y = reinterpret_cast<native_t*>(out.data_ptr<scalar_t>());
    constexpr int VMAX = 16 / (int)sizeof(native_t);
    const ElemtPlan plan =
        plan_elemt(L, total, (int)sizeof(native_t), {x, y, res}, scale);
    const int v = plan.v;
    const int grid = plan.grid;
    MSBN_DISPATCH_V(v, VMAX, [&] {
      MSBN_DISPATCH_ACT(act, ACT_, [&] {
        MSBN_DISPATCH_BOOL(has_res, RES_, [&] {
          if (!L.nhwc) {
            hipLaunchKernelGGL((bn_elemt_nchw<native_t, VV, ACT_, RES_>),
                               dim3(grid), dim3(MSBN_BLOCK), 0, stream, x, res,
                               y, scale, shift, total, L.C, L.S, slope);
          } else {
            hipLaunchKernelGGL((bn_elemt_nhwc<native_t, VV, ACT_, RES_>),
                               dim3(grid), dim3(MSBN_BLOCK), 0, stream, x, res,
                               y, scale, shift, total, L.C, slope);
          }
        });
      });
    });
  });
  return out;
}

at::Tensor batch_norm_elemt(const at::Tensor& input,
                            const c10::optional<at::Tensor>& weight,
                            const c10::optional<at::Tensor>& bias,
                            const at::Tensor& mean, const at::Tensor& invstd,
                            double eps) {
  (void)eps;
  return batch_norm_elemt_act(input, c10::nullopt, weight, bias, mean, invstd,
                              false, c10::nullopt, 0.0);
}

std::tuple<at::Tensor, at::Tensor, at::Tensor, at::Tensor>
batch_norm_backward_reduce_act(
    const at::Tensor& grad_out, const at::Tensor& input,
    const c10::optional<at::Tensor>& residual, const at::Tensor& mean,
    const at::Tensor& invstd, const c10::optional<at::Tensor>& weight,
    const c10::optional<at::Tensor>& bias, bool relu_mask, bool input_g,
    bool weight_g, bool bias_g, const c10::optional<at::Tensor>& coefs_in,
    const c10::optional<at::Tensor>& gm_out, double negative_slope,
    const c10::optional<at::Tensor>& grad_out2) {
  const Layout L = get_layout(input);
  const float slope = (float)negative_slope;
  const int act = act_mode(relu_mask, slope);
  if (input.numel() == 0) {
    auto z32 = input.options().dtype(at::kFloat);
    auto combined0 = at::zeros({2 * L.C}, z32);
    const auto wt = weight.has_value() ? weight->scalar_type()
                                       : input.scalar_type();
    at::Tensor gw0, gb0;
    if (weight_g) gw0 = at::zeros({L.C}, input.options().dtype(wt));
    if (bias_g) gb0 = at::zeros({L.C}, input.options().dtype(wt));
    return {combined0.narrow(0, 0, L.C), combined0.narrow(0, L.C, L.C), gw0,
            gb0};
  }
  const bool want_gm = gm_out.has_value();
  if (want_gm) {
    TORCH_CHECK(gm_out->sizes() == input.sizes() &&
                    gm_out->strides() == input.strides() &&
                    gm_out->scalar_type() == input.scalar_type(),
                "gm_out must match input shape/strides/dtype");
  }
  TORCH_CHECK(grad_out.sizes() == input.sizes() &&
                  grad_out.strides() == input.strides(),
              "grad_out must match input shape and layout");
  const bool has_dy2 = grad_out2.has_value();
  if (has_dy2) {
    TORCH_CHECK(want_gm, "grad_out2 requires gm_out");
    TORCH_CHECK(grad_out2->sizes() == input.sizes() &&
                    grad_out2->strides() == input.strides() &&
                    grad_out2->scalar_type() == input.scalar_type() &&
                    grad_out2->device() == input.device(),
                "grad_out2 must match input shape/strides/dtype");
  }
  TORCH_CHECK(!residual.has_value() ||
                  (residual->sizes() == input.sizes() &&
                   residual->strides() == input.strides()),
              "residual must match input shape and layout");
  auto f32 = input.options().dtype(at::kFloat);
  auto combined = at::empty({2 * L.C}, f32);
  auto sum_dy = combined.narrow(0, 0, L.C);
  auto sum_dy_xmu = combined.narrow(0, L.C, L.C);
  const auto wtype =
      weight.has_value() ? weight->scalar_type() : input.scalar_type();
  auto wopts = input.options().dtype(wtype);
  at::Tensor grad_weight, grad_bias;
  if (weight_g) grad_weight = at::empty({L.C}, wopts);
  if (bias_g) grad_bias = at::empty({L.C}, wopts);

  const bool has_res = residual.has_value();
  float* scale = nullptr;
  float* shift = nullptr;
  at::Tensor coefs;
  if (relu_mask) {
    coefs = coefs_in.has_value()
                ? *coefs_in
                : make_fwd_coefs(mean, invstd, weight, bias, L.C);
    scale = coefs.data_ptr<float>();
    shift = scale + L.C;
  }

  auto stream = cur_stream();
  MSBN_DISPATCH_FLOAT_TYPES(input.scalar_type(), "bn_bwd_reduce", [&] {
    const native_t* x =
        reinterpret_cast<const native_t*>(input.data_ptr<scalar_t>());
    const native_t* dy =
        reinterpret_cast<const native_t*>(grad_out.data_ptr<scalar_t>());
    const native_t* res =
        has_res ? reinterpret_cast<const native_t*>(residual->data_ptr())
                : nullptr;
    native_t* gm =
        want_gm ? reinterpret_cast<native_t*>(gm_out->data_ptr()) : nullptr;
    const native_t* dy2 =
        has_dy2 ? reinterpret_cast<const native_t*>(grad_out2->data_ptr())
                : nullptr;
    constexpr int VMAX = 16 / (int)sizeof(native_t);
    const ReducePlan plan =
        plan_reduce(L, (int)sizeof(native_t), {x, dy, res, gm, dy2});
    const int v = plan.v;
    const int nchunks = plan.nchunks;
    at::Tensor ws = at::empty({(int64_t)nchunks * L.C * 2},
                              input.options().dtype(at::kDouble));
    MSBN_DISPATCH_ACT(act, ACT_, [&] {
      MSBN_DISPATCH_BOOL(has_res, RES_, [&] {
        MSBN_DISPATCH_BOOL(want_gm, GM_, [&] {
          auto launch = [&](auto dy2_c) {
            constexpr bool DY2_ = decltype(dy2_c)::value && GM_;
            if (!L.nhwc) {
              if (plan.path == RedPath::NchwFlat) {
                const auto& g = plan.flat;
                hipLaunchKernelGGL(
                    (bn_bwd_reduce_partial_nchw_flat<native_t, ACT_, RES_,
                                                     GM_, DY2_>),
                    g.grid, dim3(MSBN_BLOCK), 0, stream, dy, dy2, x, res, gm,
                    mean.data_ptr<float>(), scale, shift,
                    ws.data_ptr<double>(), L.N, L.C, L.S, g.chunk_len, slope);
              } else {
                const auto& g = plan.nchw;
                MSBN_DISPATCH_V(v, VMAX, [&] {
                  hipLaunchKernelGGL(
                      (bn_bwd_reduce_partial_nchw<native_t, VV, ACT_, RES_,
                                                  GM_, DY2_>),
                      g.grid, dim3(MSBN_BLOCK), 0, stream, dy, dy2, x, res,
                      gm, mean.data_ptr<float>(), scale, shift,
                      ws.data_ptr<double>(), L.N, L.C, L.S, g.chunkN,
                      g.chunkS, slope);
                });
              }
            } else {
              const auto& g = plan.nhwc;
              MSBN_DISPATCH_V(v, VMAX, [&] {
                hipLaunchKernelGGL(
                    (bn_bwd_reduce_partial_nhwc<native_t, VV, ACT_, RES_, GM_,
                                                DY2_>),
                    g.grid, dim3(MSBN_BLOCK), 0, stream, dy, dy2, x, res, gm,
                    mean.data_ptr<float>(), scale, shift,
                    ws.data_ptr<double>(), L.rows, L.C, g.chunk_rows, g.lpr,
                    slope);
              });
            }
          };
          if (has_dy2) {
            launch(std::true_type{});
          } else {
            launch(std::false_type{});
          }
        });
      });
    });
    const int fgrid = (int)cdiv(L.C, kFinalizeWavesPerBlock);
    MSBN_DISPATCH_RSTAT(wtype, "bn_bwd_reduce", [&] {
      rstat_t* gw = weight_g ? reinterpret_cast<rstat_t*>(grad_weight.data_ptr())
                             : nullptr;
      rstat_t* gb =
          bias_g ? reinterpret_cast<rstat_t*>(grad_bias.data_ptr()) : nullptr;
      hipLaunchKernelGGL((bn_bwd_reduce_finalize<rstat_t>), dim3(fgrid),
                         dim3(MSBN_BLOCK), 0, stream, ws.data_ptr<double>(),
                         nchunks, L.C, invstd.data_ptr<float>(),
                         sum_dy.data_ptr<float>(),
                         sum_dy_xmu.data_ptr<float>(), gw, gb);
    });
  });
  (void)input_g;
  return {sum_dy, sum_dy_xmu, grad_weight, grad_bias};
}

std::tuple<at::Tensor, at::Tensor, at::Tensor, at::Tensor>
batch_norm_backward_reduce(const at::Tensor& grad_out, const at::Tensor& input,
                           const at::Tensor& mean, const at::Tensor& invstd,
                           const c10::optional<at::Tensor>& weight, bool input_g,
                           bool weight_g, bool bias_g) {
  return batch_norm_backward_reduce_act(grad_out, input, c10::nullopt, mean,
                                        invstd, weight, c10::nullopt, false,
                                        input_g, weight_g, bias_g,
                                        c10::nullopt, c10::nullopt, 0.0,
                                        c10::nullopt);
}

std::tuple<at::Tensor, at::Tensor> batch_norm_backward_elemt_act(
    const at::Tensor& grad_out, const at::Tensor& input,
    const c10::optional<at::Tensor>& residual, const at::Tensor& mean,
    const at::Tensor& invstd, const c10::optional<at::Tensor>& weight,
    const c10::optional<at::Tensor>& bias, const at::Tensor& sum_dy,
    const at::Tensor& sum_dy_xmu, const at::Tensor& count, bool relu_mask,
    bool want_res_grad, const c10::optional<at::Tensor>& coefs_in,
    double negative_slope) {
  const Layout L = get_layout(input);
  const float slope = (float)negative_slope;
  const int act = act_mode(relu_mask, slope);
  auto dx = at::empty_like(grad_out);
  at::Tensor dres;
  if (want_res_grad) dres = at::empty_like(grad_out);
  if (input.numel() == 0) return {dx, dres};
  at::Tensor count_sum;
  if (count.numel() == 1 && count.scalar_type() == at::kFloat) {
    count_sum = count;
  } else {
    count_sum = count.to(at::kFloat).sum().reshape({1});
  }
  auto stream = cur_stream();
  auto f32 = input.options().dtype(at::kFloat);
  auto coefs = at::empty({3 * L.C}, f32);
  float* ca = coefs.data_ptr<float>();
  float* cb = ca + L.C;
  float* cd = cb + L.C;
  const int cgrid = (int)cdiv(L.C, MSBN_BLOCK);
  const auto wtype =
      weight.has_value() ? weight->scalar_type() : at::kFloat;
  MSBN_DISPATCH_RSTAT(wtype, "bn_bwd_elemt", [&] {
    const rstat_t* w =
        weight.has_value()
            ? reinterpret_cast<const rstat_t*>(weight->data_ptr())
            : nullptr;
    hipLaunchKernelGGL((bn_affine_bwd<rstat_t>), dim3(cgrid), dim3(MSBN_BLOCK),
                       0, stream, mean.data_ptr<float>(),
                       invstd.data_ptr<float>(), w, sum_dy.data_ptr<float>(),
                       sum_dy_xmu.data_ptr<float>(),
                       count_sum.data_ptr<float>(), L.C, ca, cb, cd);
  });
  const bool has_res = residual.has_value();
  float* scale = nullptr;
  float* shift = nullptr;
  at::Tensor fcoefs;
  if (relu_mask) {
    fcoefs = coefs_in.has_value()
                 ? *coefs_in
                 : make_fwd_coefs(mean, invstd, weight, bias, L.C);
    scale = fcoefs.data_ptr<float>();
    shift = scale + L.C;
  }

  const int64_t total = input.numel();
  MSBN_DISPATCH_FLOAT_TYPES(input.scalar_type(), "bn_bwd_elemt", [&] {
    const native_t* x =
        reinterpret_cast<const native_t*>(input.data_ptr<scalar_t>());
    const native_t* dy =
        reinterpret_cast<const native_t*>(grad_out.data_ptr<scalar_t>());
    const native_t* res =
        has_res ? reinterpret_cast<const native_t*>(residual->data_ptr())
                : nullptr;
    native_t* o = reinterpret_cast<native_t*>(dx.data_ptr<scalar_t>());
    native_t* dr = want_res_grad
                       ? reinterpret_cast<native_t*>(dres.data_ptr<scalar_t>())
                       : nullptr;
    constexpr int VMAX = 16 / (int)sizeof(native_t);
    const ElemtPlan plan = plan_elemt(L, total, (int)sizeof(native_t),
                                      {x, dy, res, o, dr}, scale);
    const int v = plan.v;
    const int grid = plan.grid;
    MSBN_DISPATCH_V(v, VMAX, [&] {
      MSBN_DISPATCH_ACT(act, ACT_, [&] {
        MSBN_DISPATCH_BOOL(has_res, RES_, [&] {
          MSBN_DISPATCH_BOOL(want_res_grad, RESG_, [&] {
            if (!L.nhwc) {
              hipLaunchKernelGGL(
                  (bn_bwd_elemt_nchw<native_t, VV, ACT_, RES_, RESG_>),
                  dim3(grid), dim3(MSBN_BLOCK), 0, stream, dy, x, res, o, dr,
                  ca, cb, cd, scale, shift, total, L.C, L.S, slope);
            } else {
              hipLaunchKernelGGL(
                  (bn_bwd_elemt_nhwc<native_t, VV, ACT_, RES_, RESG_>),
                  dim3(grid), dim3(MSBN_BLOCK), 0, stream, dy, x, res, o, dr,
                  ca, cb, cd, scale, shift, total, L.C, slope);
            }
          });
        });
      });
    });
  });
  return {dx, dres};
}

at::Tensor batch_norm_backward_elemt(
    const at::Tensor& grad_out, const at::Tensor& input, const at::Tensor& mean,
    const at::Tensor& invstd, const c10::optional<at::Tensor>& weight,
    const at::Tensor& sum_dy, const at::Tensor& sum_dy_xmu,
    const at::Tensor& count) {
  return std::get<0>(batch_norm_backward_elemt_act(
      grad_out, input, c10::nullopt, mean, invstd, weight, c10::nullopt,
      sum_dy, sum_dy_xmu, count, false, false, c10::nullopt, 0.0));
}

namespace {
struct PoolGeom {
  int H, W, OH, OW;
};

Layout pool_layout(const at::Tensor& x, const char* op) {
  TORCH_CHECK(x.dim() == 4 &&
                  x.is_contiguous(at::MemoryFormat::ChannelsLast),
              op, ": input must be a dense 4-D channels-last tensor");
  Layout L{};
  L.nhwc = true;
  L.N = x.size(0);
  L.C = x.size(1);
  L.S = x.size(2) * x.size(3);
  L.rows = L.N * L.S;
  return L;
}

PoolGeom pool_geom(const at::Tensor& x, const Layout& L, const char* op) {
  TORCH_CHECK(L.rows < (int64_t)INT32_MAX, op, ": N*H*W must be below 2^31");
  PoolGeom g{};
  g.H = (int)x.size(2);
  g.W = (int)x.size(3);
  g.OH = (g.H - 1) / 2 + 1;
  g.OW = (g.W - 1) / 2 + 1;
  return g;
}

void check_pooled(const at::Tensor& t, const at::Tensor& x, const PoolGeom& g,
                  at::ScalarType dtype, const char* op, const char* what) {
  TORCH_CHECK(t.dim() == 4 && t.size(0) == x.size(0) &&
                  t.size(1) == x.size(1) && t.size(2) == g.OH &&
                  t.size(3) == g.OW && t.scalar_type() == dtype &&
                  t.device() == x.device() &&
                  t.is_contiguous(at::MemoryFormat::ChannelsLast),
              op, ": ", what, " must be a channels-last [N, C, OH, OW] ",
              dtype, " tensor on the input's device");
}
}

std::tuple<at::Tensor, at::Tensor> batch_norm_elemt_act_pool(
    const at::Tensor& input, const c10::optional<at::Tensor>& weight,
    const c10::optional<at::Tensor>& bias, const at::Tensor& mean,
    const at::Tensor& invstd, bool relu,
    const c10::optional<at::Tensor>& coefs_in, double negative_slope) {
  const Layout L = pool_layout(input, "bn_elemt_pool");
  TORCH_CHECK(input.numel() > 0, "bn_elemt_pool: empty input");
  const PoolGeom g = pool_geom(input, L, "bn_elemt_pool");
  const float slope = (float)negative_slope;
  const int act = act_mode(relu, slope);
  auto out = at::empty({input.size(0), L.C, g.OH, g.OW},
                       input.options().memory_format(
                           at::MemoryFormat::ChannelsLast));
  auto codes = at::empty_like(out, out.options().dtype(at::kByte));
  auto stream = cur_stream();
  auto coefs = coefs_in.has_value()
                   ? *coefs_in
                   : make_fwd_coefs(mean, invstd, weight, bias, L.C);
  float* scale = coefs.data_ptr<float>();
  float* shift = scale + L.C;
  const int64_t total = out.numel();
  MSBN_DISPATCH_FLOAT_TYPES(input.scalar_type(), "bn_elemt_pool", [&] {
    const native_t* x =
        reinterpret_cast<const native_t*>(input.data_ptr<scalar_t>());
    native_t* y = reinterpret_cast<native_t*>(out.data_ptr<scalar_t>());
    uint8_t* cp = codes.data_ptr<uint8_t>();
    constexpr int VMAX = 16 / (int)sizeof(native_t);
    const ElemtPlan plan =
        plan_elemt(L, total, (int)sizeof(native_t), {x, y, cp}, scale);
    MSBN_DISPATCH_V(plan.v, VMAX, [&] {
      constexpr int VK = VV * (int)sizeof(native_t) <= 16 ? VV : 1;
      MSBN_DISPATCH_ACT(act, ACT_, [&] {
        hipLaunchKernelGGL((bn_elemt_pool_nhwc<native_t, VK, ACT_>),
                           dim3(plan.grid), dim3(MSBN_BLOCK), 0, stream, x, y,
                           cp, scale, shift, total, L.C, g.H, g.W, g.OH, g.OW,
                           slope);
      });
    });
  });
  return {out, codes};
}

std::tuple<at::Tensor, at::Tensor, at::Tensor, at::Tensor>
batch_norm_backward_reduce_act_pool(
    const at::Tensor& grad_out, const c10::optional<at::Tensor>& grad_out2,
    const at::Tensor& codes, const at::Tensor& input, const at::Tensor& mean,
    const at::Tensor& invstd, const c10::optional<at::Tensor>& weight,
    const c10::optional<at::Tensor>& bias, bool relu_mask, bool input_g,
    bool weight_g, bool bias_g, const c10::optional<at::Tensor>& coefs_in,
    double negative_slope) {
  const Layout L = pool_layout(input, "bn_bwd_reduce_pool");
  TORCH_CHECK(input.numel() > 0, "bn_bwd_reduce_pool: empty input");
  const PoolGeom g = pool_geom(input, L, "bn_bwd_reduce_pool");
  const float slope = (float)negative_slope;
  const int act = act_mode(relu_mask, slope);
  check_pooled(grad_out, input, g, input.scalar_type(), "bn_bwd_reduce_pool",
               "grad_out");
  const bool has_dy2 = grad_out2.has_value();
  if (has_dy2)
    check_pooled(*grad_out2, input, g, input.scalar_type(),
                 "bn_bwd_reduce_pool", "grad_out2");
  check_pooled(codes, input, g, at::kByte, "bn_bwd_reduce_pool", "codes");
  auto f32 = input.options().dtype(at::kFloat);
  auto combined = at::empty({2 * L.C}, f32);
  auto sum_dy = combined.narrow(0, 0, L.C);
  auto sum_dy_xmu = combined.narrow(0, L.C, L.C);
  const auto wtype =
      weight.has_value() ? weight->scalar_type() : input.scalar_type();
  auto wopts = input.options().dtype(wtype);
  at::Tensor grad_weight, grad_bias;
  if (weight_g) grad_weight = at::empty({L.C}, wopts);
  if (bias_g) grad_bias = at::empty({L.C}, wopts);

  float* scale = nullptr;
  float* shift = nullptr;
  at::Tensor coefs;
  if (relu_mask) {
    coefs = coefs_in.has_value()
                ? *coefs_in
                : make_fwd_coefs(mean, invstd, weight, bias, L.C);
    scale = coefs.data_ptr<float>();
    shift = scale + L.C;
  }

  auto stream = cur_stream();
  MSBN_DISPATCH_FLOAT_TYPES(input.scalar_type(), "bn_bwd_reduce_pool", [&] {
    const native_t* x =
        reinterpret_cast<const native_t*>(input.data_ptr<scalar_t>());
    const native_t* dy =
        reinterpret_cast<const native_t*>(grad_out.data_ptr<scalar_t>());
    const native_t* dy2 =
        has_dy2 ? reinterpret_cast<const native_t*>(grad_out2->data_ptr())
                : nullptr;
    const uint8_t* cp = codes.data_ptr<uint8_t>();
    constexpr int VMAX = 16 / (int)sizeof(native_t);
    const ReducePlan plan =
        plan_reduce(L, (int)sizeof(native_t), {x, dy, dy2, cp});
    const int nchunks = plan.nchunks;
    const auto& ng = plan.nhwc;
    at::Tensor ws = at::empty({(int64_t)nchunks * L.C * 2},
                              input.options().dtype(at::kDouble));
    MSBN_DISPATCH_V(plan.v, VMAX, [&] {
      constexpr int VK = VV * (int)sizeof(native_t) <= 16 ? VV : 1;
      MSBN_DISPATCH_ACT(act, ACT_, [&] {
        MSBN_DISPATCH_BOOL(has_dy2, DY2_, [&] {
          hipLaunchKernelGGL(
              (bn_bwd_reduce_pool_partial_nhwc<native_t, VK, ACT_, DY2_>),
              ng.grid, dim3(MSBN_BLOCK), 0, stream, dy, dy2, cp, x,
              mean.data_ptr<float>(), scale, shift, ws.data_ptr<double>(),
              L.rows, L.C, ng.chunk_rows, ng.lpr, g.H, g.W, g.OH, g.OW,
              slope);
        });
      });
    });
    const int fgrid = (int)cdiv(L.C, kFinalizeWavesPerBlock);
    MSBN_DISPATCH_RSTAT(wtype, "bn_bwd_reduce_pool", [&] {
      rstat_t* gw = weight_g ? reinterpret_cast<rstat_t*>(grad_weight.data_ptr())
                             : nullptr;
      rstat_t* gb =
          bias_g ? reinterpret_cast<rstat_t*>(grad_bias.data_ptr()) : nullptr;
      hipLaunchKernelGGL((bn_bwd_reduce_finalize<rstat_t>), dim3(fgrid),
                         dim3(MSBN_BLOCK), 0, stream, ws.data_ptr<double>(),
                         nchunks, L.C, invstd.data_ptr<float>(),
                         sum_dy.data_ptr<float>(),
                         sum_dy_xmu.data_ptr<float>(), gw, gb);
    });
  });
  (void)input_g;
  return {sum_dy, sum_dy_xmu, grad_weight, grad_bias};
}

at::Tensor batch_norm_backward_elemt_act_pool(
    const at::Tensor& grad_out, const c10::optional<at::Tensor>& grad_out2,
    const at::Tensor& codes, const at::Tensor& input, const at::Tensor& mean,
    const at::Tensor& invstd, const c10::optional<at::Tensor>& weight,
    const c10::optional<at::Tensor>& bias, const at::Tensor& sum_dy,
    const at::Tensor& sum_dy_xmu, const at::Tensor& count, bool relu_mask,
    const c10::optional<at::Tensor>& coefs_in, double negative_slope) {
  const Layout L = pool_layout(input, "bn_bwd_elemt_pool");
  TORCH_CHECK(input.numel() > 0, "bn_bwd_elemt_pool: empty input");
  const PoolGeom g = pool_geom(input, L, "bn_bwd_elemt_pool");
  const float slope = (float)negative_slope;
  const int act = act_mode(relu_mask, slope);
  check_pooled(grad_out, input, g, input.scalar_type(), "bn_bwd_elemt_pool",
               "grad_out");
  const bool has_dy2 = grad_out2.has_value();
  if (has_dy2)
    check_pooled(*grad_out2, input, g, input.scalar_type(),
                 "bn_bwd_elemt_pool", "grad_out2");
  check_pooled(codes, input, g, at::kByte, "bn_bwd_elemt_pool", "codes");
  auto dx = at::empty_like(input);
  at::Tensor count_sum;
  if (count.numel() == 1 && count.scalar_type() == at::kFloat) {
    count_sum = count;
  } else {
    count_sum = count.to(at::kFloat).sum().reshape({1});
  }
// ... 346 lines not shown
  float* shift = scale + C;
  auto stream = cur_stream();
  const int cgrid = (int)cdiv(C, MSBN_BLOCK);
  const auto w_type = has_w   ? weight->scalar_type()
                      : has_b ? bias->scalar_type()
                              : at::kFloat;
  MSBN_DISPATCH_RSTAT(running_mean.scalar_type(), "bn_frozen_coefs", [&] {
    MSBN_DISPATCH_WTYPE(w_type, "bn_frozen_coefs", [&] {
      const rstat_t* rm =
          reinterpret_cast<const rstat_t*>(running_mean.data_ptr());
      const rstat_t* rv =
          reinterpret_cast<const rstat_t*>(running_var.data_ptr());
      const wt_t* wp =
          has_w ? reinterpret_cast<const wt_t*>(weight->data_ptr()) : nullptr;
      const wt_t* bp =
          has_b ? reinterpret_cast<const wt_t*>(bias->data_ptr()) : nullptr;
      hipLaunchKernelGGL((bn_frozen_coefs<rstat_t, wt_t>), dim3(cgrid),
                         dim3(MSBN_BLOCK), 0, stream, rm, rv, (float)eps, wp,
                         bp, C, scale, shift);
    });
  });
  return coefs;
}

std::tuple<at::Tensor, at::Tensor> batch_norm_frozen_backward_elemt(
    const at::Tensor& grad_out, const c10::optional<at::Tensor>& input,
    const c10::optional<at::Tensor>& residual, const at::Tensor& coefs,
    bool relu_mask, bool want_input_grad, bool want_res_grad,
    double negative_slope) {
  const float slope = (float)negative_slope;
  TORCH_CHECK(grad_out.dim() >= 2,
              "batch_norm_frozen_backward_elemt: grad_out must be >= 2-D");
  const Layout L = get_layout(grad_out);
  auto same_layout = [&](const at::Tensor& t) {
    if (t.sizes() != grad_out.sizes() ||
        t.scalar_type() != grad_out.scalar_type())
      return false;
    if (t.strides() == grad_out.strides()) return true;
    if (!L.nhwc) return t.is_contiguous();
    return t.is_contiguous(grad_out.dim() == 4
                               ? at::MemoryFormat::ChannelsLast
                               : at::MemoryFormat::ChannelsLast3d);
  };
  const bool has_x = input.has_value() && input->defined();
  const bool has_res = relu_mask && residual.has_value() && residual->defined();
  TORCH_CHECK(!relu_mask || has_x,
              "batch_norm_frozen_backward_elemt: relu_mask needs the input");
  TORCH_CHECK(!relu_mask || same_layout(*input),
              "input must match grad_out shape/strides/dtype");
  TORCH_CHECK(!has_res || same_layout(*residual),
              "residual must match grad_out shape/strides/dtype");
  TORCH_CHECK(coefs.scalar_type() == at::kFloat && coefs.is_contiguous() &&
                  coefs.numel() == 2 * L.C,
              "coefs must be contiguous fp32 [2C] ([scale | shift])");

  at::Tensor dx, dres;
  const bool resg = want_res_grad && relu_mask;
  if (want_res_grad && !relu_mask) dres = grad_out;
  if (want_input_grad) dx = at::empty_like(grad_out);
  if (resg) dres = at::empty_like(grad_out);
  if (grad_out.numel() == 0 || (!want_input_grad && !resg)) return {dx, dres};

  auto stream = cur_stream();
  const float* scale = coefs.data_ptr<float>();
  const float* shift = scale + L.C;
  const int64_t total = grad_out.numel();
  MSBN_DISPATCH_FLOAT_TYPES(grad_out.scalar_type(), "bn_frozen_bwd_elemt", [&] {
    const native_t* dy =
        reinterpret_cast<const native_t*>(grad_out.data_ptr<scalar_t>());
    const native_t* x =
        relu_mask ? reinterpret_cast<const native_t*>(input->data_ptr())
                  : nullptr;
    const native_t* res =
        has_res ? reinterpret_cast<const native_t*>(residual->data_ptr())
                : nullptr;
    native_t* o = want_input_grad
                      ? reinterpret_cast<native_t*>(dx.data_ptr<scalar_t>())
                      : nullptr;
    native_t* dr =
        resg ? reinterpret_cast<native_t*>(dres.data_ptr<scalar_t>())
             : nullptr;
    constexpr int VMAX = 16 / (int)sizeof(native_t);
    const ElemtPlan plan = plan_elemt(L, total, (int)sizeof(native_t),
                                      {dy, x, res, o, dr}, scale);
    const int v = plan.v;
    const int grid = plan.grid;
    MSBN_DISPATCH_V(v, VMAX, [&] {
      auto launch = [&](auto act_c, auto res_c, auto resg_c) {
        constexpr int ACT_ = decltype(act_c)::value;
        constexpr bool RES_ = decltype(res_c)::value;
        constexpr bool RESG_ = decltype(resg_c)::value;
        if (!L.nhwc) {
          hipLaunchKernelGGL(
              (bn_frozen_bwd_elemt_nchw<native_t, VV, ACT_, RES_, RESG_>),
              dim3(grid), dim3(MSBN_BLOCK), 0, stream, dy, x, res, o, dr,
              scale, shift, total, L.C, L.S, slope);
        } else {
          hipLaunchKernelGGL(
              (bn_frozen_bwd_elemt_nhwc<native_t, VV, ACT_, RES_, RESG_>),
              dim3(grid), dim3(MSBN_BLOCK), 0, stream, dy, x, res, o, dr,
              scale, shift, total, L.C, slope);
        }
      };
      using T = std::true_type;
      using F = std::false_type;
      auto gated = [&](auto act_c) {
        if (has_res && resg) launch(act_c, T{}, T{});
        else if (has_res) launch(act_c, T{}, F{});
        else if (resg) launch(act_c, F{}, T{});
        else launch(act_c, F{}, F{});
      };
      if (!relu_mask) launch(ActC<kActNone>{}, F{}, F{});
      else if (slope == 0.f) gated(ActC<kActRelu>{});
      else gated(ActC<kActLeaky>{});
    });
  });
  return {dx, dres};
}

namespace {
constexpr int64_t kFusedSmallPlaneMax = 8192;
constexpr int64_t kFusedSmallMinC = 64;

bool fp32_or_absent(const c10::optional<at::Tensor>& t) {
  return !t.has_value() || !t->defined() || t->scalar_type() == at::kFloat;
}
}

bool bn_fused_local_eligible(const at::Tensor& input,
                             const c10::optional<at::Tensor>& weight,
                             const c10::optional<at::Tensor>& bias,
                             const c10::optional<at::Tensor>& running_mean,
                             const c10::optional<at::Tensor>& running_var) {
  if (!input.is_cuda() || input.dim() < 2 || input.numel() == 0) return false;
  const auto st = input.scalar_type();
  if (st != at::kFloat && st != at::kBFloat16 && st != at::kHalf) return false;
  if (!input.is_contiguous()) return false;
  if (input.dim() >= 4 &&
      input.suggest_memory_format() == at::MemoryFormat::ChannelsLast)
    return false;
  const int64_t C = input.size(1);
  const int64_t N = input.size(0);
  const int64_t plane = input.numel() / C;
  const int64_t S = plane / std::max<int64_t>(N, 1);
  const int vmax = 16 / (int)input.element_size();
  const bool vec = (S % vmax) == 0;
  const int64_t lim = vec ? 2 * kFusedSmallPlaneMax : kFusedSmallPlaneMax;
  if (C < kFusedSmallMinC || plane > lim) return false;
  return fp32_or_absent(weight) && fp32_or_absent(bias) &&
         fp32_or_absent(running_mean) && fp32_or_absent(running_var);
}

std::tuple<at::Tensor, at::Tensor, at::Tensor, at::Tensor, at::Tensor>
batch_norm_fwd_fused_local(const at::Tensor& input,
                           const c10::optional<at::Tensor>& residual,
                           const c10::optional<at::Tensor>& weight,
                           const c10::optional<at::Tensor>& bias, double eps,
                           double momentum,
                           const c10::optional<at::Tensor>& running_mean,
                           const c10::optional<at::Tensor>& running_var,
                           bool relu, double negative_slope) {
  const float slope = (float)negative_slope;
  const int64_t C = input.size(1);
  const int64_t N = input.size(0);
  const int64_t S = input.numel() / std::max<int64_t>(N * C, 1);
  auto opts = input.options().dtype(at::kFloat);
  auto mean = at::empty({C}, opts);
  auto invstd = at::empty({C}, opts);
  auto count = at::empty({1}, opts);
  auto coefs = at::empty({2 * C}, opts);
  auto y = at::empty_like(input);
  auto stream = cur_stream();
  const bool has_res = residual.has_value() && residual->defined();
  TORCH_CHECK(!has_res || residual->is_contiguous(),
              "fused local: residual must match NCHW layout");
  float* rm = running_mean.has_value() && running_mean->defined()
                  ? running_mean->data_ptr<float>()
                  : nullptr;
  float* rv = running_var.has_value() && running_var->defined()
                  ? running_var->data_ptr<float>()
                  : nullptr;
  const float* w = weight.has_value() && weight->defined()
                       ? weight->data_ptr<float>()
                       : nullptr;
  const float* b =
      bias.has_value() && bias->defined() ? bias->data_ptr<float>() : nullptr;
  float* scale_p = coefs.data_ptr<float>();
  float* shift_p = scale_p + C;
  MSBN_DISPATCH_FLOAT_TYPES(input.scalar_type(), "bn_fwd_fused_local", [&] {
    const native_t* x =
        reinterpret_cast<const native_t*>(input.data_ptr<scalar_t>());
    const native_t* res =
        has_res ? reinterpret_cast<const native_t*>(
                      residual->data_ptr<scalar_t>())
                : nullptr;
    native_t* yp = reinterpret_cast<native_t*>(y.data_ptr<scalar_t>());
    constexpr int VMAX = 16 / (int)sizeof(native_t);
    const int v = pick_v((int)sizeof(native_t), {x, res, yp}, S);
    MSBN_DISPATCH_V(v, VMAX, [&] {
      MSBN_DISPATCH_ACT(act_mode(relu, slope), ACT_, [&] {
        MSBN_DISPATCH_BOOL(has_res, RES_, [&] {
          hipLaunchKernelGGL(
              (bn_fwd_fused_small_nchw<native_t, VV, ACT_, RES_>),
              dim3((unsigned)C), dim3(MSBN_BLOCK), 0, stream, x, res, yp,
              (int)N, C, (int)S, (float)eps, (float)momentum,
              mean.data_ptr<float>(), invstd.data_ptr<float>(),
              count.data_ptr<float>(), rm, rv, w, b, scale_p, shift_p, slope);
        });
      });
    });
  });
  return {y, mean, invstd, count, coefs};
}

std::tuple<at::Tensor, at::Tensor, at::Tensor, at::Tensor>
batch_norm_bwd_fused_local(const at::Tensor& grad_out, const at::Tensor& input,
                           const c10::optional<at::Tensor>& residual,
                           const at::Tensor& mean, const at::Tensor& invstd,
                           const c10::optional<at::Tensor>& weight,
                           const c10::optional<at::Tensor>& coefs,
                           bool relu_mask, bool want_res_grad, bool weight_g,
                           bool bias_g, double negative_slope) {
  const float slope = (float)negative_slope;
  const int64_t C = input.size(1);
  const int64_t N = input.size(0);
  const int64_t S = input.numel() / std::max<int64_t>(N * C, 1);
  TORCH_CHECK(grad_out.is_contiguous(), "fused local bwd: grad layout");
  TORCH_CHECK(!relu_mask || (coefs.has_value() && coefs->defined()),
              "fused local bwd: relu mask needs coefs");
  auto opts = input.options().dtype(at::kFloat);
  auto dx = at::empty_like(input);
  at::Tensor gw, gb, dres;
  if (weight_g) gw = at::empty({C}, opts);
  if (bias_g) gb = at::empty({C}, opts);
  if (want_res_grad) dres = at::empty_like(grad_out);
  auto stream = cur_stream();
  const bool has_res = residual.has_value() && residual->defined();
  const float* scale_p = nullptr;
  const float* shift_p = nullptr;
  if (relu_mask) {
    scale_p = coefs->data_ptr<float>();
    shift_p = scale_p + C;
  }
  const float* w = weight.has_value() && weight->defined()
                       ? weight->data_ptr<float>()
                       : nullptr;
  MSBN_DISPATCH_FLOAT_TYPES(input.scalar_type(), "bn_bwd_fused_local", [&] {
    const native_t* dy =
        reinterpret_cast<const native_t*>(grad_out.data_ptr<scalar_t>());
    const native_t* x =
        reinterpret_cast<const native_t*>(input.data_ptr<scalar_t>());
    const native_t* res =
        (relu_mask && has_res)
            ? reinterpret_cast<const native_t*>(residual->data_ptr<scalar_t>())
            : nullptr;
    native_t* dxp = reinterpret_cast<native_t*>(dx.data_ptr<scalar_t>());
    native_t* drp = want_res_grad
                        ? reinterpret_cast<native_t*>(dres.data_ptr<scalar_t>())
                        : nullptr;
    constexpr int VMAX = 16 / (int)sizeof(native_t);
    const int v =
        pick_v((int)sizeof(native_t), {dy, x, res, dxp, drp}, S);
    MSBN_DISPATCH_V(v, VMAX, [&] {
      auto launch = [&](auto act_c, auto res_c, auto resg_c) {
        hipLaunchKernelGGL(
            (bn_bwd_fused_small_nchw<native_t, VV, decltype(act_c)::value,
                                     decltype(res_c)::value,
                                     decltype(resg_c)::value>),
            dim3((unsigned)C), dim3(MSBN_BLOCK), 0, stream, dy, x, res, dxp,
            drp, mean.data_ptr<float>(), invstd.data_ptr<float>(), scale_p,
            shift_p, w, weight_g ? gw.data_ptr<float>() : nullptr,
            bias_g ? gb.data_ptr<float>() : nullptr, (int)N, C, (int)S,
            slope);
      };
      using T = std::true_type;
      using F = std::false_type;
      auto gated = [&](auto act_c) {
        if (has_res && want_res_grad) launch(act_c, T{}, T{});
        else if (has_res) launch(act_c, T{}, F{});
        else if (want_res_grad) launch(act_c, F{}, T{});
        else launch(act_c, F{}, F{});
      };
      if (!relu_mask) {
        if (want_res_grad) launch(ActC<kActNone>{}, F{}, T{});
        else launch(ActC<kActNone>{}, F{}, F{});
      } else if (slope == 0.f) {
        gated(ActC<kActRelu>{});
      } else {
        gated(ActC<kActLeaky>{});
      }
    });
  });
  return {dx, gw, gb, dres};
}

std::tuple<std::string, std::map<std::string, int64_t>> launch_plan(
    const std::string& kind, const at::Tensor& input,
    const std::vector<c10::optional<at::Tensor>>& others,
    const c10::optional<at::Tensor>& coefs) {
  TORCH_CHECK(input.dim() >= 2 && input.numel() > 0,
              "launch_plan: input must be a non-empty >= 2-D tensor");
  const int esize = (int)input.element_size();
  TORCH_CHECK(esize == 2 || esize == 4, "launch_plan: unsupported dtype");
  std::vector<const void*> ptrs{input.data_ptr()};
  for (const auto& t : others)
    if (t.has_value() && t->defined()) ptrs.push_back(t->data_ptr());
  const float* coef = coefs.has_value() && coefs->defined()
                          ? coefs->data_ptr<float>()
                          : nullptr;
  std::map<std::string, int64_t> d;
  std::string path;

  if (kind == "fused_local") {
    if (!bn_fused_local_eligible(input, c10::nullopt, c10::nullopt,
                                 c10::nullopt, c10::nullopt))
      return {"ineligible", d};
    const int64_t C = input.size(1);
    const int64_t plane = input.numel() / C;
    const int64_t S = plane / input.size(0);
    d["V"] = pick_v(esize, ptrs, S);
    d["trips"] = cdiv(plane / d["V"], MSBN_BLOCK);
    d["blocks"] = C;
    return {"small_plane", d};
  }

  const bool pool_kind = kind == "elemt_pool" || kind == "bwd_reduce_pool" ||
                         kind == "bwd_elemt_pool";
  const Layout L =
      pool_kind ? pool_layout(input, "launch_plan") : get_layout(input);
  if (kind == "stats" || kind == "bwd_reduce" ||
      kind == "bwd_reduce_inplace" || kind == "bwd_reduce_pool") {
    const ReducePlan p = plan_reduce(L, esize, ptrs);
    path = p.path == RedPath::Nhwc       ? "nhwc"
           : p.path == RedPath::NchwFlat ? "nchw_flat"
                                         : "nchw_vec";
    d["V"] = p.v;
    d["nchunks"] = p.nchunks;
    d["trips"] = p.trips;
    d["flush_every"] = p.flush_every;
    d["finalize_trips"] = cdiv(p.nchunks, MSBN_WAVE);
    if (p.path == RedPath::NchwVec) {
      d["chunkN"] = p.nchw.chunkN;
      d["chunkS"] = p.nchw.chunkS;
      d["nchunkS"] = p.nchw.grid.z;
    } else if (p.path == RedPath::NchwFlat) {
      d["chunk_len"] = p.flat.chunk_len;
    } else {
      d["chunk_rows"] = p.nhwc.chunk_rows;
      d["lpr"] = p.nhwc.lpr;
      d["ctiles"] = p.nhwc.grid.x;
    }
    return {path, d};
  }
  TORCH_CHECK(kind == "elemt" || kind == "bwd_elemt" ||
                  kind == "frozen_bwd_elemt" || kind == "elemt_inplace" ||
                  kind == "bwd_elemt_inplace" || kind == "elemt_pool" ||
                  kind == "bwd_elemt_pool",
              "launch_plan: unknown kind '", kind, "'");
  int64_t total = input.numel();
  if (kind == "elemt_pool") {
    const PoolGeom g = pool_geom(input, L, "launch_plan");
    total = input.size(0) * L.C * g.OH * g.OW;
  }
  const ElemtPlan p = plan_elemt(L, total, esize, ptrs, coef);
  path = L.nhwc ? "nhwc" : (p.v == 1 ? "nchw_flat" : "nchw_vec");
  const int64_t threads = (int64_t)p.grid * MSBN_BLOCK;
  d["V"] = p.v;
  d["grid"] = p.grid;
  d["packs"] = p.packs;
  d["trips"] = cdiv(p.packs, threads);
  d["multi_trip"] = p.packs > threads ? 1 : 0;
  return {path, d};
}

}
```

msbn/ops/csrc/bn_ops.hpp:

```cpp
#pragma once

#include <ATen/ATen.h>

#include <map>
#include <string>
#include <tuple>
#include <vector>

namespace msbn {

std::tuple<at::Tensor, at::Tensor> batch_norm_stats(const at::Tensor& input,
                                                    double eps);

void batch_norm_stats_packed(const at::Tensor& input, double eps,
                             at::Tensor& out);

std::tuple<at::Tensor, at::Tensor> batch_norm_gather_stats_with_counts(
    const at::Tensor& mean_all, const at::Tensor& invstd_all,
    const c10::optional<at::Tensor>& running_mean,
    const c10::optional<at::Tensor>& running_var, double momentum, double eps,
    const at::Tensor& counts);

std::tuple<at::Tensor, at::Tensor, at::Tensor> batch_norm_gather_stats_packed(
    const at::Tensor& packed_all, const c10::optional<at::Tensor>& running_mean,
    const c10::optional<at::Tensor>& running_var, double momentum, double eps);

std::tuple<at::Tensor, at::Tensor, at::Tensor, at::Tensor>
batch_norm_gather_stats_packed_coefs(
    const at::Tensor& packed_all, const c10::optional<at::Tensor>& running_mean,
    const c10::optional<at::Tensor>& running_var, double momentum, double eps,
    const c10::optional<at::Tensor>& weight,
    const c10::optional<at::Tensor>& bias, bool want_coefs);

std::tuple<at::Tensor, at::Tensor, at::Tensor, at::Tensor>
batch_norm_stats_local(const at::Tensor& input, double eps,
                       const c10::optional<at::Tensor>& running_mean,
                       const c10::optional<at::Tensor>& running_var,
                       double momentum,
                       const c10::optional<at::Tensor>& weight,
                       const c10::optional<at::Tensor>& bias, bool want_coefs);

at::Tensor batch_norm_elemt(const at::Tensor& input,
                            const c10::optional<at::Tensor>& weight,
                            const c10::optional<at::Tensor>& bias,
                            const at::Tensor& mean, const at::Tensor& invstd,
                            double eps);

std::tuple<at::Tensor, at::Tensor, at::Tensor, at::Tensor>
batch_norm_backward_reduce(const at::Tensor& grad_out, const at::Tensor& input,
                           const at::Tensor& mean, const at::Tensor& invstd,
                           const c10::optional<at::Tensor>& weight, bool input_g,
                           bool weight_g, bool bias_g);

at::Tensor batch_norm_backward_elemt(
    const at::Tensor& grad_out, const at::Tensor& input, const at::Tensor& mean,
    const at::Tensor& invstd, const c10::optional<at::Tensor>& weight,
    const at::Tensor& sum_dy, const at::Tensor& sum_dy_xmu,
    const at::Tensor& count);

at::Tensor bn_make_coefs(const at::Tensor& mean, const at::Tensor& invstd,
                         const c10::optional<at::Tensor>& weight,
                         const c10::optional<at::Tensor>& bias);

at::Tensor batch_norm_elemt_act(const at::Tensor& input,
                                const c10::optional<at::Tensor>& residual,
                                const c10::optional<at::Tensor>& weight,
                                const c10::optional<at::Tensor>& bias,
                                const at::Tensor& mean,
                                const at::Tensor& invstd, bool relu,
                                const c10::optional<at::Tensor>& coefs_in,
                                double negative_slope);

std::tuple<at::Tensor, at::Tensor, at::Tensor, at::Tensor>
batch_norm_backward_reduce_act(
    const at::Tensor& grad_out, const at::Tensor& input,
    const c10::optional<at::Tensor>& residual, const at::Tensor& mean,
    const at::Tensor& invstd, const c10::optional<at::Tensor>& weight,
    const c10::optional<at::Tensor>& bias, bool relu_mask, bool input_g,
    bool weight_g, bool bias_g, const c10::optional<at::Tensor>& coefs_in,
    const c10::optional<at::Tensor>& gm_out, double negative_slope,
    const c10::optional<at::Tensor>& grad_out2);

at::Tensor bn_frozen_coefs(const at::Tensor& running_mean,
                           const at::Tensor& running_var, double eps,
                           const c10::optional<at::Tensor>& weight,
                           const c10::optional<at::Tensor>& bias);

std::tuple<at::Tensor, at::Tensor> batch_norm_frozen_backward_elemt(
    const at::Tensor& grad_out, const c10::optional<at::Tensor>& input,
    const c10::optional<at::Tensor>& residual, const at::Tensor& coefs,
    bool relu_mask, bool want_input_grad, bool want_res_grad,
    double negative_slope);

bool bn_fused_local_eligible(const at::Tensor& input,
                             const c10::optional<at::Tensor>& weight,
                             const c10::optional<at::Tensor>& bias,
                             const c10::optional<at::Tensor>& running_mean,
                             const c10::optional<at::Tensor>& running_var);

std::tuple<at::Tensor, at::Tensor, at::Tensor, at::Tensor, at::Tensor>
batch_norm_fwd_fused_local(const at::Tensor& input,
                           const c10::optional<at::Tensor>& residual,
                           const c10::optional<at::Tensor>& weight,
                           const c10::optional<at::Tensor>& bias, double eps,
                           double momentum,
                           const c10::optional<at::Tensor>& running_mean,
                           const c10::optional<at::Tensor>& running_var,
                           bool relu, double negative_slope);

std::tuple<at::Tensor, at::Tensor, at::Tensor, at::Tensor>
batch_norm_bwd_fused_local(const at::Tensor& grad_out, const at::Tensor& input,
                           const c10::optional<at::Tensor>& residual,
                           const at::Tensor& mean, const at::Tensor& invstd,
                           const c10::optional<at::Tensor>& weight,
                           const c10::optional<at::Tensor>& coefs,
                           bool relu_mask, bool want_res_grad, bool weight_g,
                           bool bias_g, double negative_slope);

std::tuple<at::Tensor, at::Tensor> batch_norm_backward_elemt_act(
    const at::Tensor& grad_out, const at::Tensor& input,
    const c10::optional<at::Tensor>& residual, const at::Tensor& mean,
    const at::Tensor& invstd, const c10::optional<at::Tensor>& weight,
    const c10::optional<at::Tensor>& bias, const at::Tensor& sum_dy,
    const at::Tensor& sum_dy_xmu, const at::Tensor& count, bool relu_mask,
    bool want_res_grad, const c10::optional<at::Tensor>& coefs_in,
    double negative_slope);

std::tuple<at::Tensor, at::Tensor> batch_norm_elemt_act_pool(
    const at::Tensor& input, const c10::optional<at::Tensor>& weight,
    const c10::optional<at::Tensor>& bias, const at::Tensor& mean,
    const at::Tensor& invstd, bool relu,
    const c10::optional<at::Tensor>& coefs_in, double negative_slope);

std::tuple<at::Tensor, at::Tensor, at::Tensor, at::Tensor>
batch_norm_backward_reduce_act_pool(
    const at::Tensor& grad_out, const c10::optional<at::Tensor>& grad_out2,
    const at::Tensor& codes, const at::Tensor& input, const at::Tensor& mean,
    const at::Tensor& invstd, const c10::optional<at::Tensor>& weight,
    const c10::optional<at::Tensor>& bias, bool relu_mask, bool input_g,
    bool weight_g, bool bias_g, const c10::optional<at::Tensor>& coefs_in,
    double negative_slope);

at::Tensor batch_norm_backward_elemt_act_pool(
    const at::Tensor& grad_out, const c10::optional<at::Tensor>& grad_out2,
    const at::Tensor& codes, const at::Tensor& input, const at::Tensor& mean,
    const at::Tensor& invstd, const c10::optional<at::Tensor>& weight,
    const c10::optional<at::Tensor>& bias, const at::Tensor& sum_dy,
    const at::Tensor& sum_dy_xmu, const at::Tensor& count, bool relu_mask,
    const c10::optional<at::Tensor>& coefs_in, double negative_slope);

at::Tensor batch_norm_elemt_act_(at::Tensor& input,
                                 const c10::optional<at::Tensor>& weight,
                                 const c10::optional<at::Tensor>& bias,
                                 const at::Tensor& mean,
                                 const at::Tensor& invstd, bool act,
                                 const c10::optional<at::Tensor>& coefs_in,
                                 double negative_slope);

std::tuple<at::Tensor, at::Tensor, at::Tensor, at::Tensor>
batch_norm_backward_reduce_inplace(
    const at::Tensor& grad_out, const at::Tensor& output,
    const at::Tensor& invstd, const c10::optional<at::Tensor>& weight,
    const c10::optional<at::Tensor>& bias, bool act, bool input_g,
    bool weight_g, bool bias_g, const c10::optional<at::Tensor>& coefs_in,
    double negative_slope);

at::Tensor batch_norm_backward_elemt_inplace(
    const at::Tensor& grad_out, const at::Tensor& output,
    const at::Tensor& mean, const at::Tensor& invstd,
    const c10::optional<at::Tensor>& weight,
    const c10::optional<at::Tensor>& bias, const at::Tensor& sum_dy,
    const at::Tensor& sum_dy_xmu, const at::Tensor& count, bool act,
    const c10::optional<at::Tensor>& coefs_in, double negative_slope);

std::tuple<std::string, std::map<std::string, int64_t>> launch_plan(
    const std::string& kind, const at::Tensor& input,
    const std::vector<c10::optional<at::Tensor>>& others,
    const c10::optional<at::Tensor>& coefs);

}
```

msbn/ops/csrc/common.hpp:

```cpp
#pragma once

#include <hip/hip_runtime.h>
#include <hip/hip_bf16.h>
#include <hip/hip_fp16.h>

#define MSBN_WAVE 64
#define MSBN_BLOCK 256

namespace msbn {

template <typename T, int V>
struct alignas(sizeof(T) * V) Pack {
  T v[V];
};

__device__ __forceinline__ float to_f(float x) { return x; }
__device__ __forceinline__ float to_f(__hip_bfloat16 x) {
  return __bfloat162float(x);
}
__device__ __forceinline__ float to_f(__half x) { return __half2float(x); }

template <typename T>
__device__ __forceinline__ T from_f(float x);
template <>
__device__ __forceinline__ float from_f<float>(float x) {
  return x;
}
template <>
__device__ __forceinline__ __hip_bfloat16 from_f<__hip_bfloat16>(float x) {
  return __float2bfloat16(x);
}
template <>
__device__ __forceinline__ __half from_f<__half>(float x) {
  return __float2half(x);
}

constexpr int kActNone = 0;
constexpr int kActRelu = 1;
constexpr int kActLeaky = 2;

template <int ACT>
__device__ __forceinline__ float act_fwd(float z, float slope) {
  if (ACT == kActRelu) return fmaxf(z, 0.f);
  if (ACT == kActLeaky) return z > 0.f ? z : slope * z;
  return z;
}

template <int ACT>
__device__ __forceinline__ float act_gate(float z, float g, float slope) {
  if (ACT == kActRelu) {
    if (z <= 0.f) g = 0.f;
  }
  if (ACT == kActLeaky) g = z > 0.f ? g : slope * g;
  return g;
}

template <int BYTES>
struct NTVec;
template <>
struct NTVec<32> {
  using type = int __attribute__((vector_size(32)));
};
template <>
struct NTVec<16> {
  using type = int __attribute__((vector_size(16)));
};
template <>
struct NTVec<8> {
  using type = int __attribute__((vector_size(8)));
};
template <>
struct NTVec<4> {
  using type = int;
};
template <>
struct NTVec<2> {
  using type = short;
};
template <>
struct NTVec<1> {
  using type = char;
};

template <typename T, int V>
__device__ __forceinline__ Pack<T, V> nt_load(const T* p) {
#ifdef MSBN_DISABLE_NT
  return *reinterpret_cast<const Pack<T, V>*>(p);
#else
  using VT = typename NTVec<(int)sizeof(T) * V>::type;
  union {
    VT v;
    Pack<T, V> pk;
  } u;
  u.v = __builtin_nontemporal_load(reinterpret_cast<const VT*>(p));
  return u.pk;
#endif
}

template <typename T, int V>
__device__ __forceinline__ void nt_store(T* p, const Pack<T, V>& val) {
#ifdef MSBN_DISABLE_NT
  *reinterpret_cast<Pack<T, V>*>(p) = val;
#else
  using VT = typename NTVec<(int)sizeof(T) * V>::type;
  union {
    VT v;
    Pack<T, V> pk;
  } u;
  u.pk = val;
  __builtin_nontemporal_store(u.v, reinterpret_cast<VT*>(p));
#endif
}

template <typename T>
__device__ __forceinline__ T nt_load1(const T* p) {
  return nt_load<T, 1>(p).v[0];
}

template <typename T>
__device__ __forceinline__ void nt_store1(T* p, T val) {
  Pack<T, 1> pk;
  pk.v[0] = val;
  nt_store<T, 1>(p, pk);
}

__device__ __forceinline__ void wave_reduce_pair(double& a, double& b) {
#pragma unroll
  for (int off = MSBN_WAVE / 2; off > 0; off >>= 1) {
    a += __shfl_down(a, off, MSBN_WAVE);
    b += __shfl_down(b, off, MSBN_WAVE);
  }
}

__device__ __forceinline__ void block_reduce_pair(double& a, double& b,
                                                  double* lds) {
  wave_reduce_pair(a, b);
  const int lane = threadIdx.x & (MSBN_WAVE - 1);
  const int wid = threadIdx.x >> 6;
  const int nw = blockDim.x >> 6;
  if (lane == 0) {
    lds[2 * wid] = a;
    lds[2 * wid + 1] = b;
  }
  __syncthreads();
  if (wid == 0) {
    a = (lane < nw) ? lds[2 * lane] : 0.0;
    b = (lane < nw) ? lds[2 * lane + 1] : 0.0;
    wave_reduce_pair(a, b);
  }
}

__device__ __forceinline__ int64_t i64min(int64_t a, int64_t b) {
  return a < b ? a : b;
}

#define MSBN_ACC_FLUSH 64

struct AccPair {
  double a = 0.0, b = 0.0;
  float fa = 0.f, fb = 0.f;

  __device__ __forceinline__ void add(float v) {
    fa += v;
    fb += v * v;
  }
  __device__ __forceinline__ void add2(float s, float sq) {
    fa += s;
    fb += sq;
  }
  __device__ __forceinline__ void flush() {
    a += (double)fa;
    b += (double)fb;
    fa = fb = 0.f;
  }
};

#define MSBN_RAW_COND_MAX 64.0

__device__ __forceinline__ bool needs_recentre(double sum, double sumsq,
                                               double cnt) {
  return !((MSBN_RAW_COND_MAX + 1.0) * sum * sum <=
           MSBN_RAW_COND_MAX * cnt * sumsq);
}

__device__ __forceinline__ void unshift_pair(double& a, double& b,
                                             float pivot, double cnt) {
  const double p = (double)pivot;
  b += p * (2.0 * a + cnt * p);
  a += cnt * p;
}

}
```

msbn/ops/csrc/module.cpp:

```cpp
#include <torch/extension.h>

#include <torch/csrc/distributed/c10d/ProcessGroup.hpp>

#include "bn_ops.hpp"
#include "reducer.hpp"

PYBIND11_MODULE(TORCH_EXTENSION_NAME, m) {
  m.doc() = "msbn MI355X-native kernels + reducer";

  m.def("batch_norm_stats", &msbn::batch_norm_stats, py::arg("input"),
        py::arg("eps"));
  m.def("batch_norm_stats_packed", &msbn::batch_norm_stats_packed,
        py::arg("input"), py::arg("eps"), py::arg("out"));
  m.def("batch_norm_gather_stats_with_counts",
        &msbn::batch_norm_gather_stats_with_counts, py::arg("mean_all"),
        py::arg("invstd_all"), py::arg("running_mean"), py::arg("running_var"),
        py::arg("momentum"), py::arg("eps"), py::arg("counts"));
  m.def("batch_norm_gather_stats_packed",
        &msbn::batch_norm_gather_stats_packed, py::arg("packed_all"),
        py::arg("running_mean"), py::arg("running_var"), py::arg("momentum"),
        py::arg("eps"));
  m.def("batch_norm_gather_stats_packed_coefs",
        &msbn::batch_norm_gather_stats_packed_coefs, py::arg("packed_all"),
        py::arg("running_mean"), py::arg("running_var"), py::arg("momentum"),
        py::arg("eps"), py::arg("weight"), py::arg("bias"),
        py::arg("want_coefs"));
  m.def("batch_norm_stats_local", &msbn::batch_norm_stats_local,
        py::arg("input"), py::arg("eps"), py::arg("running_mean"),
        py::arg("running_var"), py::arg("momentum"), py::arg("weight"),
        py::arg("bias"), py::arg("want_coefs"));
  m.def("batch_norm_elemt", &msbn::batch_norm_elemt, py::arg("input"),
        py::arg("weight"), py::arg("bias"), py::arg("mean"), py::arg("invstd"),
        py::arg("eps"));
  m.def("batch_norm_backward_reduce", &msbn::batch_norm_backward_reduce,
        py::arg("grad_out"), py::arg("input"), py::arg("mean"),
        py::arg("invstd"), py::arg("weight"), py::arg("input_g"),
        py::arg("weight_g"), py::arg("bias_g"));
  m.def("batch_norm_backward_elemt", &msbn::batch_norm_backward_elemt,
        py::arg("grad_out"), py::arg("input"), py::arg("mean"),
        py::arg("invstd"), py::arg("weight"), py::arg("sum_dy"),
        py::arg("sum_dy_xmu"), py::arg("count"));
  m.def("bn_make_coefs", &msbn::bn_make_coefs, py::arg("mean"),
        py::arg("invstd"), py::arg("weight"), py::arg("bias"));
  m.def("batch_norm_elemt_act", &msbn::batch_norm_elemt_act, py::arg("input"),
        py::arg("residual"), py::arg("weight"), py::arg("bias"),
        py::arg("mean"), py::arg("invstd"), py::arg("relu"),
        py::arg("coefs") = py::none(), py::arg("negative_slope") = 0.0);
  m.def("batch_norm_backward_reduce_act",
        &msbn::batch_norm_backward_reduce_act, py::arg("grad_out"),
        py::arg("input"), py::arg("residual"), py::arg("mean"),
        py::arg("invstd"), py::arg("weight"), py::arg("bias"),
        py::arg("relu_mask"), py::arg("input_g"), py::arg("weight_g"),
        py::arg("bias_g"), py::arg("coefs") = py::none(),
        py::arg("gm_out") = py::none(), py::arg("negative_slope") = 0.0,
        py::arg("grad_out2") = py::none());
  m.def("batch_norm_backward_elemt_act", &msbn::batch_norm_backward_elemt_act,
        py::arg("grad_out"), py::arg("input"), py::arg("residual"),
        py::arg("mean"), py::arg("invstd"), py::arg("weight"), py::arg("bias"),
        py::arg("sum_dy"), py::arg("sum_dy_xmu"), py::arg("count"),
        py::arg("relu_mask"), py::arg("want_res_grad"),
        py::arg("coefs") = py::none(), py::arg("negative_slope") = 0.0);

  m.def("batch_norm_elemt_act_pool", &msbn::batch_norm_elemt_act_pool,
        py::arg("input"), py::arg("weight"), py::arg("bias"), py::arg("mean"),
        py::arg("invstd"), py::arg("relu"), py::arg("coefs") = py::none(),
        py::arg("negative_slope") = 0.0);
  m.def("batch_norm_backward_reduce_act_pool",
        &msbn::batch_norm_backward_reduce_act_pool, py::arg("grad_out"),
        py::arg("grad_out2"), py::arg("codes"), py::arg("input"),
        py::arg("mean"), py::arg("invstd"), py::arg("weight"), py::arg("bias"),
        py::arg("relu_mask"), py::arg("input_g"), py::arg("weight_g"),
        py::arg("bias_g"), py::arg("coefs") = py::none(),
        py::arg("negative_slope") = 0.0);
  m.def("batch_norm_backward_elemt_act_pool",
        &msbn::batch_norm_backward_elemt_act_pool, py::arg("grad_out"),
        py::arg("grad_out2"), py::arg("codes"), py::arg("input"),
        py::arg("mean"), py::arg("invstd"), py::arg("weight"), py::arg("bias"),
        py::arg("sum_dy"), py::arg("sum_dy_xmu"), py::arg("count"),
        py::arg("relu_mask"), py::arg("coefs") = py::none(),
        py::arg("negative_slope") = 0.0);

  m.def("batch_norm_elemt_act_", &msbn::batch_norm_elemt_act_,
        py::arg("input"), py::arg("weight"), py::arg("bias"), py::arg("mean"),
        py::arg("invstd"), py::arg("act"), py::arg("coefs") = py::none(),
        py::arg("negative_slope") = 0.0);
  m.def("batch_norm_backward_reduce_inplace",
        &msbn::batch_norm_backward_reduce_inplace, py::arg("grad_out"),
        py::arg("output"), py::arg("invstd"), py::arg("weight"),
        py::arg("bias"), py::arg("act"), py::arg("input_g"),
        py::arg("weight_g"), py::arg("bias_g"), py::arg("coefs") = py::none(),
        py::arg("negative_slope") = 0.0);
  m.def("batch_norm_backward_elemt_inplace",
        &msbn::batch_norm_backward_elemt_inplace, py::arg("grad_out"),
        py::arg("output"), py::arg("mean"), py::arg("invstd"),
        py::arg("weight"), py::arg("bias"), py::arg("sum_dy"),
        py::arg("sum_dy_xmu"), py::arg("count"), py::arg("act"),
        py::arg("coefs") = py::none(), py::arg("negative_slope") = 0.0);

  m.def("bn_frozen_coefs", &msbn::bn_frozen_coefs, py::arg("running_mean"),
        py::arg("running_var"), py::arg("eps"), py::arg("weight"),
        py::arg("bias"));
  m.def("batch_norm_frozen_backward_elemt",
        &msbn::batch_norm_frozen_backward_elemt, py::arg("grad_out"),
        py::arg("input"), py::arg("residual"), py::arg("coefs"),
        py::arg("relu_mask"), py::arg("want_input_grad"),
        py::arg("want_res_grad"), py::arg("negative_slope") = 0.0);

  m.def("bn_fused_local_eligible", &msbn::bn_fused_local_eligible,
        py::arg("input"), py::arg("weight"), py::arg("bias"),
        py::arg("running_mean"), py::arg("running_var"));
  m.def("batch_norm_fwd_fused_local", &msbn::batch_norm_fwd_fused_local,
        py::arg("input"), py::arg("residual"), py::arg("weight"),
        py::arg("bias"), py::arg("eps"), py::arg("momentum"),
        py::arg("running_mean"), py::arg("running_var"), py::arg("relu"),
        py::arg("negative_slope") = 0.0);
  m.def("batch_norm_bwd_fused_local", &msbn::batch_norm_bwd_fused_local,
        py::arg("grad_out"), py::arg("input"), py::arg("residual"),
        py::arg("mean"), py::arg("invstd"), py::arg("weight"),
        py::arg("coefs"), py::arg("relu_mask"), py::arg("want_res_grad"),
        py::arg("weight_g"), py::arg("bias_g"),
        py::arg("negative_slope") = 0.0);

  m.def("launch_plan", &msbn::launch_plan, py::arg("kind"), py::arg("input"),
        py::arg("others") = std::vector<c10::optional<at::Tensor>>(),
        py::arg("coefs") = py::none());

  m.def("compute_bucket_assignment_by_size",
        &msbn::compute_bucket_assignment_by_size, py::arg("tensors"),
        py::arg("bucket_size_limits"));
  m.def("broadcast_coalesced", &msbn::broadcast_coalesced,
        py::call_guard<py::gil_scoped_release>(), py::arg("process_group"),
        py::arg("tensors"), py::arg("buffer_bytes"), py::arg("src_rank") = 0);
  m.def("verify_params_across_processes",
        &msbn::verify_params_across_processes,
        py::call_guard<py::gil_scoped_release>(), py::arg("process_group"),
        py::arg("params"));

  py::class_<msbn::Reducer, std::shared_ptr<msbn::Reducer>>(
      m, "Reducer", py::module_local())
      .def(py::init<std::vector<at::Tensor>, std::vector<std::vector<int64_t>>,
                    c10::intrusive_ptr<c10d::ProcessGroup>, bool, size_t,
                    size_t>(),
           py::arg("params"), py::arg("bucket_indices"),
           py::arg("process_group"), py::arg("gradient_as_bucket_view") = false,
           py::arg("first_bucket_bytes") = (size_t)1024 * 1024,
           py::arg("bucket_bytes") = (size_t)25 * 1024 * 1024)
      .def("prepare_for_backward", &msbn::Reducer::prepare_for_backward,
           py::arg("unused_params") = std::vector<int64_t>())
      .def("set_grad_sync_enabled", &msbn::Reducer::set_grad_sync_enabled)
      .def("set_comm_dtype", &msbn::Reducer::set_comm_dtype)
      .def("set_nan_check", &msbn::Reducer::set_nan_check)
      .def("set_div_factor", &msbn::Reducer::set_div_factor)
      .def("set_python_comm_hook", &msbn::Reducer::set_python_comm_hook,
           py::arg("state"), py::arg("hook"), py::arg("bucket_cls"))
      .def("div_factor", &msbn::Reducer::div_factor)
      .def("find_unused", &msbn::Reducer::find_unused, py::arg("outputs"))
      .def("finalize_backward", &msbn::Reducer::finalize_backward,
           py::call_guard<py::gil_scoped_release>())
      .def("rebuild_buckets", &msbn::Reducer::rebuild_buckets,
           py::call_guard<py::gil_scoped_release>())
      .def("get_bucket_indices", &msbn::Reducer::get_bucket_indices)
      .def("get_backward_stats", &msbn::Reducer::get_backward_stats)
      .def("iterations", &msbn::Reducer::iterations)
      .def("rebuilt", &msbn::Reducer::rebuilt);
}
```

Measured before the change: 9676 images/sec.

## Save 1-bit ReLU gate masks instead of residual for bn+add+relu backward

For the last BN+residual+ReLU in each residual block, the forward kernel now writes a packed bitmask recording whether each output passed the activation. The residual tensor is no longer saved for backward, and the backward reduce kernel reads the gate bits in place of recomputing the pre-activation from the residual. This is meant to cut backward memory traffic, replacing a bf16 residual read with one bit per element, and to lower activation memory. In exchange the forward pass does an extra small byte store per 8-element pack, and the kernel dispatch gains another template dimension.

```diff
diff --git a/msbn/models/resnet.py b/msbn/models/resnet.py
--- a/msbn/models/resnet.py
+++ b/msbn/models/resnet.py
@@ -37,7 +37,7 @@
     expansion = 1
 
     def __init__(self, cin, planes, stride=1, downsample=None, fused=False,
-                 fork=False):
+                 fork=False, gate_bits=True):
         super().__init__()
         self.fused = fused
         self.fork = fork and fused
@@ -46,7 +46,8 @@
         self.downsample = downsample
         if fused:
             self.bn1 = SyncBatchNormAct2d(planes, relu=True)
-            self.bn2 = SyncBatchNormAct2d(planes, relu=True)
+            self.bn2 = SyncBatchNormAct2d(planes, relu=True,
+                                          gate_bits=gate_bits)
         else:
             self.bn1 = BatchNorm2d(planes)
             self.bn2 = BatchNorm2d(planes)
@@ -69,7 +70,7 @@
     expansion = 4
 
     def __init__(self, cin, planes, stride=1, downsample=None, fused=False,
-                 fork=False):
+                 fork=False, gate_bits=True):
         super().__init__()
         self.fused = fused
         self.fork = fork and fused
@@ -80,7 +81,8 @@
         if fused:
             self.bn1 = SyncBatchNormAct2d(planes, relu=True)
             self.bn2 = SyncBatchNormAct2d(planes, relu=True)
-            self.bn3 = SyncBatchNormAct2d(planes * self.expansion, relu=True)
+            self.bn3 = SyncBatchNormAct2d(planes * self.expansion, relu=True,
+                                          gate_bits=gate_bits)
         else:
             self.bn1 = BatchNorm2d(planes)
             self.bn2 = BatchNorm2d(planes)
@@ -111,9 +113,11 @@
         in_chans: int = 3,
         fused: bool = False,
         fork_grads: bool = True,
+        gate_bits: bool = True,
     ):
         super().__init__()
         self.fused = fused
+        self.gate_bits = gate_bits and fused
         self.fork_grads = fork_grads and fused
         self.stem_pool = fused
         self.inplanes = 64
@@ -146,11 +150,12 @@
                 _norm(planes * block.expansion, self.fused),
             )
         layers = [block(self.inplanes, planes, stride, downsample,
-                        fused=self.fused, fork=fork[0])]
+                        fused=self.fused, fork=fork[0],
+                        gate_bits=self.gate_bits)]
         self.inplanes = planes * block.expansion
         for i in range(1, blocks):
             layers.append(block(self.inplanes, planes, fused=self.fused,
-                                fork=fork[i]))
+                                fork=fork[i], gate_bits=self.gate_bits))
         return nn.Sequential(*layers)
 
     def _stem(self, x):
@@ -178,12 +183,12 @@
 
 
 def resnet18(num_classes: int = 1000, fused: bool = False,
-             fork_grads: bool = True) -> ResNet:
+             fork_grads: bool = True, gate_bits: bool = True) -> ResNet:
     return ResNet(BasicBlock, [2, 2, 2, 2], num_classes, fused=fused,
-                  fork_grads=fork_grads)
+                  fork_grads=fork_grads, gate_bits=gate_bits)
 
 
 def resnet50(num_classes: int = 1000, fused: bool = False,
-             fork_grads: bool = True) -> ResNet:
+             fork_grads: bool = True, gate_bits: bool = True) -> ResNet:
     return ResNet(Bottleneck, [3, 4, 6, 3], num_classes, fused=fused,
-                  fork_grads=fork_grads)
+                  fork_grads=fork_grads, gate_bits=gate_bits)
diff --git a/msbn/nn/fused.py b/msbn/nn/fused.py
--- a/msbn/nn/fused.py
+++ b/msbn/nn/fused.py
@@ -28,8 +28,10 @@
         relu: bool,
         negative_slope: float = 0.0,
         fork: bool = False,
+        gate_bits: bool = False,
     ):
         ctx.fork = fork
+        ctx.gate_bits = gate_bits
         y = SyncBatchNormActFunction._forward(
             ctx, input, residual, weight, bias, running_mean, running_var,
             eps, momentum, process_group, world_size, relu, negative_slope,
@@ -44,6 +46,8 @@
                  running_var, eps, momentum, process_group, world_size, relu,
                  negative_slope):
         ctx.negative_slope = negative_slope
+        ctx.has_res = residual is not None
+        ctx.has_gate = False
         input = _contig(input)
         if residual is not None:
             residual = _match_layout(residual, input)
@@ -81,45 +85,52 @@
             input, eps, momentum, running_mean, running_var,
             process_group, world_size, weight, bias, want_coefs=True,
         )
-        if coefs is None:
-            ctx.save_for_backward(input, residual, weight, bias, mean, invstd,
-                                  count_sum)
-            ctx.has_coefs = False
-        else:
-            ctx.save_for_backward(input, residual, weight, bias, mean, invstd,
-                                  count_sum, coefs)
-            ctx.has_coefs = True
+        ctx.has_coefs = coefs is not None
         ctx.relu = relu
         ctx.process_group = process_group
         ctx.world_size = world_size
         ctx.use_sync = use_sync
+        gate = None
         if input.numel() == 0:
-            return torch.empty_like(input)
-        return ops.batch_norm_elemt_act(
-            input, residual, weight, bias, mean, invstd, relu, coefs,
-            negative_slope,
-        )
+            y = torch.empty_like(input)
+        elif (ctx.gate_bits and relu and residual is not None
+                and ctx.needs_input_grad[1] and input.is_cuda):
+            y, gate = ops.batch_norm_elemt_act(
+                input, residual, weight, bias, mean, invstd, relu, coefs,
+                negative_slope, ops.gate_bits_empty(input),
+            )
+        else:
+            y = ops.batch_norm_elemt_act(
+                input, residual, weight, bias, mean, invstd, relu, coefs,
+                negative_slope,
+            )
+        ctx.has_gate = gate is not None
+        saved = (input, None if ctx.has_gate else residual, weight, bias,
+                 mean, invstd, count_sum)
+        if ctx.has_coefs:
+            saved += (coefs,)
+        if ctx.has_gate:
+            saved += (gate,)
+        ctx.save_for_backward(*saved)
+        return y
 
     @staticmethod
     def backward(ctx, grad_output, grad_skip=None):
         if grad_output is None:
             grad_output, grad_skip = grad_skip, None
         if grad_output is None:
-            return (None,) * 13
-        if ctx.has_coefs:
-            (input, residual, weight, bias, mean, invstd, count_sum,
-             coefs) = ctx.saved_tensors
-        else:
-            input, residual, weight, bias, mean, invstd, count_sum = (
-                ctx.saved_tensors
-            )
-            coefs = None
+            return (None,) * 14
+        saved = ctx.saved_tensors
+        input, residual, weight, bias, mean, invstd, count_sum = saved[:7]
+        coefs = saved[7] if ctx.has_coefs else None
+        gate = saved[-1] if ctx.has_gate else None
+        has_res = ctx.has_res
         fold = (
             grad_skip is not None and input.is_cuda and input.numel() > 0
             and not getattr(ctx, "local_fused", False)
         )
         if fold and ctx.relu and ctx.negative_slope != 0.0 and not (
-            residual is not None and ctx.needs_input_grad[1]
+            has_res and ctx.needs_input_grad[1]
         ):
             fold = False
         if grad_skip is not None and not fold:
@@ -133,7 +144,7 @@
         process_group = ctx.process_group
         world_size = ctx.world_size
         need_input_g = ctx.needs_input_grad[0]
-        need_res_g = residual is not None and ctx.needs_input_grad[1]
+        need_res_g = has_res and ctx.needs_input_grad[1]
         need_weight_g = weight is not None and ctx.needs_input_grad[2]
         need_bias_g = bias is not None and ctx.needs_input_grad[3]
 
@@ -152,11 +163,11 @@
                 grad_res if need_res_g else None,
                 grad_weight if need_weight_g else None,
                 grad_bias if need_bias_g else None,
-                None, None, None, None, None, None, None, None, None,
+                None, None, None, None, None, None, None, None, None, None,
             )
 
         use_gm = fold or (
-            relu and residual is not None and need_res_g and input.is_cuda
+            relu and has_res and need_res_g and input.is_cuda
             and input.numel() > 0
         )
         use_sync = getattr(ctx, "use_sync", world_size > 1)
@@ -176,16 +187,25 @@
                 torch.empty_like(grad_output) if need_res_g else None,
                 torch.zeros_like(weight) if need_weight_g else None,
                 torch.zeros_like(bias) if need_bias_g else None,
-                None, None, None, None, None, None, None, None, None,
+                None, None, None, None, None, None, None, None, None, None,
             )
         gm = torch.empty_like(grad_output) if use_gm else None
-        sum_dy, sum_dy_xmu, grad_weight, grad_bias = (
-            ops.batch_norm_backward_reduce_act(
-                grad_output, input, residual, mean, invstd, weight, bias,
-                relu, need_input_g, need_weight_g, need_bias_g, coefs, gm,
-                slope, grad_skip,
-            )
-        )
+        if gate is not None:
+            sum_dy, sum_dy_xmu, grad_weight, grad_bias = (
+                ops.batch_norm_backward_reduce_act(
+                    grad_output, input, None, mean, invstd, weight, bias,
+                    relu, need_input_g, need_weight_g, need_bias_g, coefs, gm,
+                    slope, grad_skip, gate=gate,
+                )
+            )
+        else:
+            sum_dy, sum_dy_xmu, grad_weight, grad_bias = (
+                ops.batch_norm_backward_reduce_act(
+                    grad_output, input, residual, mean, invstd, weight, bias,
+                    relu, need_input_g, need_weight_g, need_bias_g, coefs, gm,
+                    slope, grad_skip,
+                )
+            )
         grad_input = grad_res = None
         if need_input_g or need_res_g:
             if use_sync:
@@ -217,7 +237,7 @@
             grad_res,
             grad_weight if need_weight_g else None,
             grad_bias if need_bias_g else None,
-            None, None, None, None, None, None, None, None, None,
+            None, None, None, None, None, None, None, None, None, None,
         )
 
 
@@ -486,9 +506,10 @@
     def __init__(self, num_features, eps=1e-5, momentum=0.1, affine=True,
                  track_running_stats=True, process_group=None, device=None,
                  dtype=None, relu: bool = True, negative_slope: float = 0.0,
-                 inplace: bool = False):
+                 inplace: bool = False, gate_bits: bool = True):
         super().__init__(num_features, eps, momentum, affine,
                          track_running_stats, process_group, device, dtype)
+        self.gate_bits = bool(gate_bits)
         self.relu = relu
         self.negative_slope = _check_negative_slope(relu, negative_slope)
         if inplace:
@@ -555,4 +576,5 @@
             input, residual, self.weight, self.bias, running_mean, running_var,
             self.eps, factor, process_group, world_size, self.relu, slope,
             fork,
-        )
+            getattr(self, "gate_bits", False),
+        )
diff --git a/msbn/ops/__init__.py b/msbn/ops/__init__.py
--- a/msbn/ops/__init__.py
+++ b/msbn/ops/__init__.py
@@ -177,29 +177,39 @@
     return None
 
 
+def gate_bits_empty(input: torch.Tensor) -> torch.Tensor:
+    return torch.empty((input.numel() + 7) // 8, dtype=torch.uint8,
+                       device=input.device)
+
+
 def batch_norm_elemt_act(input, residual, weight, bias, mean, invstd,
-                         relu: bool, coefs=None, negative_slope: float = 0.0):
-    if input.is_cuda:
-        return _require_hip().batch_norm_elemt_act(
+                         relu: bool, coefs=None, negative_slope: float = 0.0,
+                         gate_out=None):
+    if input.is_cuda:
+        y, wrote = _require_hip().batch_norm_elemt_act(
             input, residual, weight, bias, mean, invstd, relu, coefs,
-            negative_slope,
-        )
-    return _ref.batch_norm_elemt_act(
+            negative_slope, gate_out,
+        )
+        return y if gate_out is None else (y, gate_out if wrote else None)
+    y = _ref.batch_norm_elemt_act(
         input, residual, weight, bias, mean, invstd, relu, negative_slope
     )
+    return y if gate_out is None else (y, None)
 
 
 def batch_norm_backward_reduce_act(grad_out, input, residual, mean, invstd,
                                    weight, bias, relu_mask, input_g, weight_g,
                                    bias_g, coefs=None, gm_out=None,
                                    negative_slope: float = 0.0,
-                                   grad_out2=None):
+                                   grad_out2=None, gate=None):
     if input.is_cuda:
         return _require_hip().batch_norm_backward_reduce_act(
             grad_out, input, residual, mean, invstd, weight, bias, relu_mask,
             input_g, weight_g, bias_g, coefs, gm_out, negative_slope,
-            grad_out2,
-        )
+            grad_out2, gate,
+        )
+    if gate is not None:
+        raise ValueError("gate bits exist on the GPU path only")
     return _ref.batch_norm_backward_reduce_act(
         grad_out, input, residual, mean, invstd, weight, bias, relu_mask,
         input_g, weight_g, bias_g, gm_out, negative_slope, grad_out2,
@@ -336,14 +346,16 @@
     path, numbers = _require_hip().launch_plan(kind, input, list(others), coefs)
     plan = dict(numbers)
     plan["path"] = path
-    if "multi_trip" in plan:
-        plan["multi_trip"] = bool(plan["multi_trip"])
+    for flag in ("multi_trip", "gate"):
+        if flag in plan:
+            plan[flag] = bool(plan[flag])
     return plan
 
 
 __all__ = [
     "hip_available",
     "launch_plan",
+    "gate_bits_empty",
     "bn_frozen_coefs",
     "batch_norm_frozen_backward_elemt",
     "batch_norm_elemt_act_pool",
diff --git a/msbn/ops/csrc/bn_kernels.hip b/msbn/ops/csrc/bn_kernels.hip
--- a/msbn/ops/csrc/bn_kernels.hip
+++ b/msbn/ops/csrc/bn_kernels.hip
@@ -370,12 +370,15 @@
   coef_d[c] = f1 * (f3 * mean[c] - f2);
 }
 
-template <typename T, int V, int ACT, bool RES>
+template <typename T, int V, int ACT, bool RES, bool GATE>
 __global__ void bn_elemt_nchw(const T* __restrict__ x,
                               const T* __restrict__ res, T* __restrict__ y,
                               const float* __restrict__ scale,
                               const float* __restrict__ shift, int64_t total,
-                              int64_t C, int64_t S, float slope) {
+                              int64_t C, int64_t S, float slope,
+                              unsigned char* __restrict__ gate_out) {
+  static_assert(!GATE || (V == 8 && RES && ACT != kActNone),
+                "gate bits: one byte per 8-pack of a bn+add+act layer");
   const int64_t stride = (int64_t)gridDim.x * blockDim.x;
   for (int64_t i = (int64_t)blockIdx.x * blockDim.x + threadIdx.x;
        i * V < total; i += stride) {
@@ -392,24 +395,30 @@
       Pack<T, V> pr;
       if (RES) pr = nt_load<T, V>(&res[e]);
       Pack<T, V> py;
+      unsigned bits = 0;
 #pragma unroll
       for (int k = 0; k < V; ++k) {
         float z = to_f(px.v[k]) * sc + sh;
         if (RES) z += to_f(pr.v[k]);
+        if (GATE) bits |= (unsigned)act_pass<ACT>(z) << k;
         z = act_fwd<ACT>(z, slope);
         py.v[k] = from_f<T>(z);
       }
       nt_store<T, V>(&y[e], py);
-    }
-  }
-}
-
-template <typename T, int V, int ACT, bool RES>
+      if (GATE) gate_store(gate_out, e, bits);
+    }
+  }
+}
+
+template <typename T, int V, int ACT, bool RES, bool GATE>
 __global__ void bn_elemt_nhwc(const T* __restrict__ x,
                               const T* __restrict__ res, T* __restrict__ y,
                               const float* __restrict__ scale,
                               const float* __restrict__ shift, int64_t total,
-                              int64_t C, float slope) {
+                              int64_t C, float slope,
+                              unsigned char* __restrict__ gate_out) {
+  static_assert(!GATE || (V == 8 && RES && ACT != kActNone),
+                "gate bits: one byte per 8-pack of a bn+add+act layer");
   const int64_t stride = (int64_t)gridDim.x * blockDim.x;
   for (int64_t i = (int64_t)blockIdx.x * blockDim.x + threadIdx.x;
        i * V < total; i += stride) {
@@ -427,14 +436,17 @@
       Pack<T, V> pr;
       if (RES) pr = nt_load<T, V>(&res[e]);
       Pack<T, V> py;
+      unsigned bits = 0;
 #pragma unroll
       for (int k = 0; k < V; ++k) {
         float z = to_f(px.v[k]) * ps.v[k] + pb.v[k];
         if (RES) z += to_f(pr.v[k]);
+        if (GATE) bits |= (unsigned)act_pass<ACT>(z) << k;
         z = act_fwd<ACT>(z, slope);
         py.v[k] = from_f<T>(z);
       }
       nt_store<T, V>(&y[e], py);
+      if (GATE) gate_store(gate_out, e, bits);
     }
   }
 }
@@ -444,7 +456,8 @@
   return to_f(from_f<T>(to_f(g1) + to_f(g2)));
 }
 
-template <typename T, int V, int ACT, bool RES, bool GMOUT, bool DY2>
+template <typename T, int V, int ACT, bool RES, bool GMOUT, bool DY2,
+          bool GATE>
 __global__ void bn_bwd_reduce_partial_nchw(const T* __restrict__ dy,
                                            const T* __restrict__ dy2,
                                            const T* __restrict__ x,
@@ -455,11 +468,14 @@
                                            const float* __restrict__ shift,
                                            double* __restrict__ ws, int64_t N,
                                            int64_t C, int64_t S, int64_t chunkN,
-                                           int64_t chunkS, float slope) {
+                                           int64_t chunkS, float slope,
+                                           const unsigned char* __restrict__ gate) {
+  static_assert(!GATE || (ACT != kActNone && !RES && GMOUT && V <= 8),
+                "gate bits replace the res read of a gm-writing reduce");
   const int64_t c = blockIdx.x;
   const float m = mean[c];
-  const float sc = ACT ? scale[c] : 0.f;
-  const float sh = ACT ? shift[c] : 0.f;
+  const float sc = (ACT && !GATE) ? scale[c] : 0.f;
+  const float sh = (ACT && !GATE) ? shift[c] : 0.f;
   const int64_t n0 = blockIdx.y * chunkN;
   const int64_t n1 = i64min(n0 + chunkN, N);
   const int64_t s0 = blockIdx.z * chunkS;
@@ -474,7 +490,9 @@
                                   nt_load1(&dy2[base + s]))
                       : to_f(nt_load1(&dy[base + s]));
         const float xv = to_f(nt_load1(&x[base + s]));
-        if (ACT) {
+        if (GATE) {
+          g = act_gate_bit<ACT>(gate_load(gate, base + s) & 1u, g, slope);
+        } else if (ACT) {
           float z = sc * xv + sh;
           if (RES) z += to_f(nt_load1(&res[base + s]));
           g = act_gate<ACT>(z, g, slope);
@@ -494,11 +512,15 @@
         Pack<T, V> pg2, pr, pm;
         if (DY2) pg2 = nt_load<T, V>(&dy2[base + s]);
         if (RES) pr = nt_load<T, V>(&res[base + s]);
+        unsigned bits = 0;
+        if (GATE) bits = gate_load(gate, base + s);
 #pragma unroll
         for (int k = 0; k < V; ++k) {
           float g = DY2 ? fork_grad(pg.v[k], pg2.v[k]) : to_f(pg.v[k]);
           const float xv = to_f(px.v[k]);
-          if (ACT) {
+          if (GATE) {
+            g = act_gate_bit<ACT>((bits >> k) & 1u, g, slope);
+          } else if (ACT) {
             float z = sc * xv + sh;
             if (RES) z += to_f(pr.v[k]);
             g = act_gate<ACT>(z, g, slope);
@@ -526,7 +548,7 @@
   }
 }
 
-template <typename T, int ACT, bool RES, bool GMOUT, bool DY2>
+template <typename T, int ACT, bool RES, bool GMOUT, bool DY2, bool GATE>
 __global__ void bn_bwd_reduce_partial_nchw_flat(
     const T* __restrict__ dy, const T* __restrict__ dy2,
     const T* __restrict__ x,
@@ -534,11 +556,13 @@
     const float* __restrict__ mean,
     const float* __restrict__ scale, const float* __restrict__ shift,
     double* __restrict__ ws, int64_t N, int64_t C, int64_t S,
-    int64_t chunk_len, float slope) {
+    int64_t chunk_len, float slope, const unsigned char* __restrict__ gate) {
+  static_assert(!GATE || (ACT != kActNone && !RES && GMOUT),
+                "gate bits replace the res read of a gm-writing reduce");
   const int64_t c = blockIdx.x;
   const float m = mean[c];
-  const float sc = ACT ? scale[c] : 0.f;
-  const float sh = ACT ? shift[c] : 0.f;
+  const float sc = (ACT && !GATE) ? scale[c] : 0.f;
+  const float sh = (ACT && !GATE) ? shift[c] : 0.f;
   const int64_t NS = N * S;
   const int64_t p0 = (int64_t)blockIdx.y * chunk_len;
   const int64_t p1 = i64min(p0 + chunk_len, NS);
@@ -550,7 +574,9 @@
     float g = DY2 ? fork_grad(nt_load1(&dy[e]), nt_load1(&dy2[e]))
                   : to_f(nt_load1(&dy[e]));
     const float xv = to_f(nt_load1(&x[e]));
-    if (ACT) {
+    if (GATE) {
+      g = act_gate_bit<ACT>(gate_load(gate, e) & 1u, g, slope);
+    } else if (ACT) {
       float z = sc * xv + sh;
       if (RES) z += to_f(nt_load1(&res[e]));
       g = act_gate<ACT>(z, g, slope);
@@ -573,7 +599,8 @@
   }
 }
 
-template <typename T, int V, int ACT, bool RES, bool GMOUT, bool DY2>
+template <typename T, int V, int ACT, bool RES, bool GMOUT, bool DY2,
+          bool GATE>
 __global__ void bn_bwd_reduce_partial_nhwc(const T* __restrict__ dy,
                                            const T* __restrict__ dy2,
                                            const T* __restrict__ x,
@@ -585,7 +612,10 @@
                                            double* __restrict__ ws,
                                            int64_t rows, int64_t C,
                                            int64_t chunk_rows, int lpr,
-                                           float slope) {
+                                           float slope,
+                                           const unsigned char* __restrict__ gate) {
+  static_assert(!GATE || (ACT != kActNone && !RES && GMOUT && V <= 8),
+                "gate bits replace the res read of a gm-writing reduce");
   const int rpi = blockDim.x / lpr;
   const int lane = threadIdx.x % lpr;
   const int rowoff = threadIdx.x / lpr;
@@ -601,7 +631,7 @@
 #pragma unroll
     for (int k = 0; k < V; ++k) {
       m[k] = mean[c + k];
-      if (ACT) {
+      if (ACT && !GATE) {
         scv[k] = scale[c + k];
         shv[k] = shift[c + k];
       }
@@ -615,11 +645,15 @@
       Pack<T, V> pg2, pr, pm;
       if (DY2) pg2 = nt_load<T, V>(&dy2[r * C + c]);
       if (RES) pr = nt_load<T, V>(&res[r * C + c]);
+      unsigned bits = 0;
+      if (GATE) bits = gate_load(gate, r * C + c);
 #pragma unroll
       for (int k = 0; k < V; ++k) {
         float g = DY2 ? fork_grad(pg.v[k], pg2.v[k]) : to_f(pg.v[k]);
         const float xv = to_f(px.v[k]);
-        if (ACT) {
+        if (GATE) {
+          g = act_gate_bit<ACT>((bits >> k) & 1u, g, slope);
+        } else if (ACT) {
           float z = scv[k] * xv + shv[k];
           if (RES) z += to_f(pr.v[k]);
           g = act_gate<ACT>(z, g, slope);
@@ -2289,17 +2323,34 @@
   return make_fwd_coefs(mean, invstd, weight, bias, mean.numel());
 }
 
-at::Tensor batch_norm_elemt_act(const at::Tensor& input,
-                                const c10::optional<at::Tensor>& residual,
-                                const c10::optional<at::Tensor>& weight,
-                                const c10::optional<at::Tensor>& bias,
-                                const at::Tensor& mean,
-                                const at::Tensor& invstd, bool relu,
-                                const c10::optional<at::Tensor>& coefs_in,
-                                double negative_slope) {
+namespace {
+void check_gate_tensor(const at::Tensor& gate, const at::Tensor& input,
+                       const char* name) {
+  TORCH_CHECK(gate.scalar_type() == at::kByte && gate.is_contiguous() &&
+                  gate.device() == input.device() &&
+                  gate.numel() == (input.numel() + 7) / 8,
+              name, " must be a contiguous uint8 tensor of ceil(numel/8) "
+              "bytes on the input's device");
+}
+
+inline bool elemt_writes_gate(int act, bool has_res, int v) {
+  return act != kActNone && has_res && v == 8;
+}
+}
+
+std::tuple<at::Tensor, bool> batch_norm_elemt_act(
+    const at::Tensor& input, const c10::optional<at::Tensor>& residual,
+    const c10::optional<at::Tensor>& weight,
+    const c10::optional<at::Tensor>& bias, const at::Tensor& mean,
+    const at::Tensor& invstd, bool relu,
+    const c10::optional<at::Tensor>& coefs_in, double negative_slope,
+    const c10::optional<at::Tensor>& gate_out) {
   const Layout L = get_layout(input);
   auto out = at::empty_like(input);
-  if (input.numel() == 0) return out;
+  if (gate_out.has_value())
+    check_gate_tensor(*gate_out, input, "gate_out");
+  bool wrote_gate = false;
+  if (input.numel() == 0) return {out, wrote_gate};
   const float slope = (float)negative_slope;
   const int act = act_mode(relu, slope);
   auto stream = cur_stream();
@@ -2329,23 +2380,38 @@
         plan_elemt(L, total, (int)sizeof(native_t), {x, y, res}, scale);
     const int v = plan.v;
     const int grid = plan.grid;
+    wrote_gate = gate_out.has_value() && elemt_writes_gate(act, has_res, v);
+    unsigned char* gate =
+        wrote_gate ? gate_out->data_ptr<unsigned char>() : nullptr;
     MSBN_DISPATCH_V(v, VMAX, [&] {
       MSBN_DISPATCH_ACT(act, ACT_, [&] {
         MSBN_DISPATCH_BOOL(has_res, RES_, [&] {
-          if (!L.nhwc) {
-            hipLaunchKernelGGL((bn_elemt_nchw<native_t, VV, ACT_, RES_>),
-                               dim3(grid), dim3(MSBN_BLOCK), 0, stream, x, res,
-                               y, scale, shift, total, L.C, L.S, slope);
+          auto launch = [&](auto gate_c) {
+            constexpr bool GATE_ = decltype(gate_c)::value;
+            if (!L.nhwc) {
+              hipLaunchKernelGGL(
+                  (bn_elemt_nchw<native_t, VV, ACT_, RES_, GATE_>), dim3(grid),
+                  dim3(MSBN_BLOCK), 0, stream, x, res, y, scale, shift, total,
+                  L.C, L.S, slope, gate);
+            } else {
+              hipLaunchKernelGGL(
+                  (bn_elemt_nhwc<native_t, VV, ACT_, RES_, GATE_>), dim3(grid),
+                  dim3(MSBN_BLOCK), 0, stream, x, res, y, scale, shift, total,
+                  L.C, slope, gate);
+            }
+          };
+          constexpr bool kCanGate = VV == 8 && sizeof(native_t) == 2 &&
+                                    ACT_ != kActNone && RES_;
+          if (wrote_gate) {
+            launch(std::integral_constant<bool, kCanGate>{});
           } else {
-            hipLaunchKernelGGL((bn_elemt_nhwc<native_t, VV, ACT_, RES_>),
-                               dim3(grid), dim3(MSBN_BLOCK), 0, stream, x, res,
-                               y, scale, shift, total, L.C, slope);
+            launch(std::false_type{});
           }
         });
       });
     });
   });
-  return out;
+  return {out, wrote_gate};
 }
 
 at::Tensor batch_norm_elemt(const at::Tensor& input,
@@ -2354,8 +2420,9 @@
                             const at::Tensor& mean, const at::Tensor& invstd,
                             double eps) {
   (void)eps;
-  return batch_norm_elemt_act(input, c10::nullopt, weight, bias, mean, invstd,
-                              false, c10::nullopt, 0.0);
+  return std::get<0>(batch_norm_elemt_act(input, c10::nullopt, weight, bias,
+                                          mean, invstd, false, c10::nullopt,
+                                          0.0, c10::nullopt));
 }
 
 std::tuple<at::Tensor, at::Tensor, at::Tensor, at::Tensor>
@@ -2366,10 +2433,19 @@
     const c10::optional<at::Tensor>& bias, bool relu_mask, bool input_g,
     bool weight_g, bool bias_g, const c10::optional<at::Tensor>& coefs_in,
     const c10::optional<at::Tensor>& gm_out, double negative_slope,
-    const c10::optional<at::Tensor>& grad_out2) {
+    const c10::optional<at::Tensor>& grad_out2,
+    const c10::optional<at::Tensor>& gate) {
   const Layout L = get_layout(input);
   const float slope = (float)negative_slope;
   const int act = act_mode(relu_mask, slope);
+  const bool has_gate = gate.has_value();
+  if (has_gate) {
+    TORCH_CHECK(act != kActNone && !residual.has_value() &&
+                    gm_out.has_value() && input.element_size() == 2,
+                "gate needs relu_mask, gm_out, a bf16 / half input and no "
+                "residual");
+    check_gate_tensor(*gate, input, "gate");
+  }
   if (input.numel() == 0) {
     auto z32 = input.options().dtype(at::kFloat);
     auto combined0 = at::zeros({2 * L.C}, z32);
@@ -2419,13 +2495,15 @@
   float* scale = nullptr;
   float* shift = nullptr;
   at::Tensor coefs;
-  if (relu_mask) {
+  if (relu_mask && !has_gate) {
     coefs = coefs_in.has_value()
                 ? *coefs_in
                 : make_fwd_coefs(mean, invstd, weight, bias, L.C);
     scale = coefs.data_ptr<float>();
     shift = scale + L.C;
   }
+  const unsigned char* gate_p =
+      has_gate ? gate->data_ptr<unsigned char>() : nullptr;
 
   auto stream = cur_stream();
   MSBN_DISPATCH_FLOAT_TYPES(input.scalar_type(), "bn_bwd_reduce", [&] {
@@ -2451,27 +2529,30 @@
     MSBN_DISPATCH_ACT(act, ACT_, [&] {
       MSBN_DISPATCH_BOOL(has_res, RES_, [&] {
         MSBN_DISPATCH_BOOL(want_gm, GM_, [&] {
-          auto launch = [&](auto dy2_c) {
+          auto launch = [&](auto dy2_c, auto gate_c) {
             constexpr bool DY2_ = decltype(dy2_c)::value && GM_;
+            constexpr bool GATE_ = decltype(gate_c)::value && GM_ && !RES_ &&
+                                   ACT_ != kActNone && sizeof(native_t) == 2;
             if (!L.nhwc) {
               if (plan.path == RedPath::NchwFlat) {
                 const auto& g = plan.flat;
                 hipLaunchKernelGGL(
                     (bn_bwd_reduce_partial_nchw_flat<native_t, ACT_, RES_,
-                                                     GM_, DY2_>),
+                                                     GM_, DY2_, GATE_>),
                     g.grid, dim3(MSBN_BLOCK), 0, stream, dy, dy2, x, res, gm,
                     mean.data_ptr<float>(), scale, shift,
-                    ws.data_ptr<double>(), L.N, L.C, L.S, g.chunk_len, slope);
+                    ws.data_ptr<double>(), L.N, L.C, L.S, g.chunk_len, slope,
+                    gate_p);
               } else {
                 const auto& g = plan.nchw;
                 MSBN_DISPATCH_V(v, VMAX, [&] {
                   hipLaunchKernelGGL(
                       (bn_bwd_reduce_partial_nchw<native_t, VV, ACT_, RES_,
-                                                  GM_, DY2_>),
+                                                  GM_, DY2_, GATE_>),
                       g.grid, dim3(MSBN_BLOCK), 0, stream, dy, dy2, x, res,
                       gm, mean.data_ptr<float>(), scale, shift,
                       ws.data_ptr<double>(), L.N, L.C, L.S, g.chunkN,
-                      g.chunkS, slope);
+                      g.chunkS, slope, gate_p);
                 });
               }
             } else {
@@ -2479,18 +2560,24 @@
               MSBN_DISPATCH_V(v, VMAX, [&] {
                 hipLaunchKernelGGL(
                     (bn_bwd_reduce_partial_nhwc<native_t, VV, ACT_, RES_, GM_,
-                                                DY2_>),
+                                                DY2_, GATE_>),
                     g.grid, dim3(MSBN_BLOCK), 0, stream, dy, dy2, x, res, gm,
                     mean.data_ptr<float>(), scale, shift,
                     ws.data_ptr<double>(), L.rows, L.C, g.chunk_rows, g.lpr,
-                    slope);
+                    slope, gate_p);
               });
             }
           };
-          if (has_dy2) {
-            launch(std::true_type{});
+          if (has_gate) {
+            if (has_dy2) {
+              launch(std::true_type{}, std::true_type{});
+            } else {
+              launch(std::false_type{}, std::true_type{});
+            }
+          } else if (has_dy2) {
+            launch(std::true_type{}, std::false_type{});
           } else {
-            launch(std::false_type{});
+            launch(std::false_type{}, std::false_type{});
           }
         });
       });
@@ -2521,7 +2608,7 @@
                                         invstd, weight, c10::nullopt, false,
                                         input_g, weight_g, bias_g,
                                         c10::nullopt, c10::nullopt, 0.0,
-                                        c10::nullopt);
+                                        c10::nullopt, c10::nullopt);
 }
 
 std::tuple<at::Tensor, at::Tensor> batch_norm_backward_elemt_act(
@@ -3474,9 +3561,15 @@
               "launch_plan: input must be a non-empty >= 2-D tensor");
   const int esize = (int)input.element_size();
   TORCH_CHECK(esize == 2 || esize == 4, "launch_plan: unsupported dtype");
+  const size_t gate_at = kind == "elemt"        ? 1
+                         : kind == "bwd_reduce" ? 4
+                                                : others.size();
+  auto given = [&](size_t i) {
+    return i < others.size() && others[i].has_value() && others[i]->defined();
+  };
   std::vector<const void*> ptrs{input.data_ptr()};
-  for (const auto& t : others)
-    if (t.has_value() && t->defined()) ptrs.push_back(t->data_ptr());
+  for (size_t i = 0; i < others.size(); ++i)
+    if (i != gate_at && given(i)) ptrs.push_back(others[i]->data_ptr());
   const float* coef = coefs.has_value() && coefs->defined()
                           ? coefs->data_ptr<float>()
                           : nullptr;
@@ -3522,6 +3615,8 @@
       d["lpr"] = p.nhwc.lpr;
       d["ctiles"] = p.nhwc.grid.x;
     }
+    if (gate_at < others.size())
+      d["gate"] = given(gate_at) && !given(1) && given(2) && esize == 2;
     return {path, d};
   }
   TORCH_CHECK(kind == "elemt" || kind == "bwd_elemt" ||
@@ -3542,6 +3637,8 @@
   d["packs"] = p.packs;
   d["trips"] = cdiv(p.packs, threads);
   d["multi_trip"] = p.packs > threads ? 1 : 0;
+  if (gate_at < others.size())
+    d["gate"] = given(gate_at) && elemt_writes_gate(kActRelu, given(0), p.v);
   return {path, d};
 }
 
diff --git a/msbn/ops/csrc/bn_ops.hpp b/msbn/ops/csrc/bn_ops.hpp
--- a/msbn/ops/csrc/bn_ops.hpp
+++ b/msbn/ops/csrc/bn_ops.hpp
@@ -62,14 +62,13 @@
                          const c10::optional<at::Tensor>& weight,
                          const c10::optional<at::Tensor>& bias);
 
-at::Tensor batch_norm_elemt_act(const at::Tensor& input,
-                                const c10::optional<at::Tensor>& residual,
-                                const c10::optional<at::Tensor>& weight,
-                                const c10::optional<at::Tensor>& bias,
-                                const at::Tensor& mean,
-                                const at::Tensor& invstd, bool relu,
-                                const c10::optional<at::Tensor>& coefs_in,
-                                double negative_slope);
+std::tuple<at::Tensor, bool> batch_norm_elemt_act(
+    const at::Tensor& input, const c10::optional<at::Tensor>& residual,
+    const c10::optional<at::Tensor>& weight,
+    const c10::optional<at::Tensor>& bias, const at::Tensor& mean,
+    const at::Tensor& invstd, bool relu,
+    const c10::optional<at::Tensor>& coefs_in, double negative_slope,
+    const c10::optional<at::Tensor>& gate_out);
 
 std::tuple<at::Tensor, at::Tensor, at::Tensor, at::Tensor>
 batch_norm_backward_reduce_act(
@@ -79,7 +78,8 @@
     const c10::optional<at::Tensor>& bias, bool relu_mask, bool input_g,
     bool weight_g, bool bias_g, const c10::optional<at::Tensor>& coefs_in,
     const c10::optional<at::Tensor>& gm_out, double negative_slope,
-    const c10::optional<at::Tensor>& grad_out2);
+    const c10::optional<at::Tensor>& grad_out2,
+    const c10::optional<at::Tensor>& gate);
 
 at::Tensor bn_frozen_coefs(const at::Tensor& running_mean,
                            const at::Tensor& running_var, double eps,
diff --git a/msbn/ops/csrc/common.hpp b/msbn/ops/csrc/common.hpp
--- a/msbn/ops/csrc/common.hpp
+++ b/msbn/ops/csrc/common.hpp
@@ -47,12 +47,51 @@
 }
 
 template <int ACT>
+__device__ __forceinline__ bool act_pass(float z) {
+  if (ACT == kActRelu) return !(z <= 0.f);
+  if (ACT == kActLeaky) return z > 0.f;
+  return true;
+}
+
+template <int ACT>
+__device__ __forceinline__ float act_gate_bit(bool pass, float g,
+                                              float slope) {
+  if (ACT == kActRelu) {
+    if (!pass) g = 0.f;
+  }
+  if (ACT == kActLeaky) g = pass ? g : slope * g;
+  return g;
+}
+
+template <int ACT>
 __device__ __forceinline__ float act_gate(float z, float g, float slope) {
-  if (ACT == kActRelu) {
-    if (z <= 0.f) g = 0.f;
-  }
-  if (ACT == kActLeaky) g = z > 0.f ? g : slope * g;
-  return g;
+  return act_gate_bit<ACT>(act_pass<ACT>(z), g, slope);
+}
+
+#ifndef MSBN_GATE_STORE_NT
+#define MSBN_GATE_STORE_NT 0
+#endif
+#ifndef MSBN_GATE_LOAD_NT
+#define MSBN_GATE_LOAD_NT 0
+#endif
+
+__device__ __forceinline__ void gate_store(unsigned char* gate, int64_t e,
+                                           unsigned bits) {
+#if MSBN_GATE_STORE_NT && !defined(MSBN_DISABLE_NT)
+  __builtin_nontemporal_store((unsigned char)bits, &gate[e >> 3]);
+#else
+  gate[e >> 3] = (unsigned char)bits;
+#endif
+}
+
+__device__ __forceinline__ unsigned gate_load(const unsigned char* gate,
+                                              int64_t e) {
+#if MSBN_GATE_LOAD_NT && !defined(MSBN_DISABLE_NT)
+  const unsigned b = __builtin_nontemporal_load(&gate[e >> 3]);
+#else
+  const unsigned b = gate[e >> 3];
+#endif
+  return b >> (unsigned)(e & 7);
 }
 
 template <int BYTES>
diff --git a/msbn/ops/csrc/module.cpp b/msbn/ops/csrc/module.cpp
--- a/msbn/ops/csrc/module.cpp
+++ b/msbn/ops/csrc/module.cpp
@@ -45,7 +45,8 @@
   m.def("batch_norm_elemt_act", &msbn::batch_norm_elemt_act, py::arg("input"),
         py::arg("residual"), py::arg("weight"), py::arg("bias"),
         py::arg("mean"), py::arg("invstd"), py::arg("relu"),
-        py::arg("coefs") = py::none(), py::arg("negative_slope") = 0.0);
+        py::arg("coefs") = py::none(), py::arg("negative_slope") = 0.0,
+        py::arg("gate_out") = py::none());
   m.def("batch_norm_backward_reduce_act",
         &msbn::batch_norm_backward_reduce_act, py::arg("grad_out"),
         py::arg("input"), py::arg("residual"), py::arg("mean"),
@@ -53,7 +54,7 @@
         py::arg("relu_mask"), py::arg("input_g"), py::arg("weight_g"),
         py::arg("bias_g"), py::arg("coefs") = py::none(),
         py::arg("gm_out") = py::none(), py::arg("negative_slope") = 0.0,
-        py::arg("grad_out2") = py::none());
+        py::arg("grad_out2") = py::none(), py::arg("gate") = py::none());
   m.def("batch_norm_backward_elemt_act", &msbn::batch_norm_backward_elemt_act,
         py::arg("grad_out"), py::arg("input"), py::arg("residual"),
         py::arg("mean"), py::arg("invstd"), py::arg("weight"), py::arg("bias"),
```

Measured after the change: 9855 images/sec (median of 6 runs). 1.8% higher.
